# astooke/accel_rl

Measured on AMD Instinct MI355X. Metric: env-steps/sec (whole node), 256-env PPO Atari, higher is better.
Workload: dtype f32; 1 GPU; PPO breakout, 256 envs/GPU, horizon 5, spec-1 CNN (fp32), minibatch 512/GPU x 4 epochs, adam; synthetic fixed-frame emulator; hipGraph rollout; total_envs=256, global_minibatch=512, parallelism=single

## Files before the change

accel_rl_amd/_lib.py:

```python
import collections
import ctypes as C
import os

import torch

_PKG = os.path.dirname(os.path.abspath(__file__))
LIB_PATH = os.path.join(_PKG, "libaccel_rl_hip.so")

ARL_ABI_VERSION = 4
PROMO_NEP50, PROMO_LEGACY, PROMO_ASSOC = 0, 1, 2
PPO_TIE_THEANO, PPO_TIE_MATH, PPO_TIE_BOTH = 0, 1, 2
PPG_POLICY, PPG_AUX = 0, 1
OPT_ADAM, OPT_RMSPROP = 0, 1
VMPO_MAX_ROWS = 65536
RND_MAX_ROWS, RND_MIX_MAX_ENVS, RND_MIX_MAX_ROWS = 1 << 24, 1 << 20, 1 << 22
MAX_ACTIONS = 18
REPLAY_MAX_HORIZON = 16
RAW_H, RAW_W, OBS_H, OBS_W = 210, 160, 104, 80
OPT_PARTIALS = 1024

_vp, _i32, _i64, _f32, _f64 = C.c_void_p, C.c_int32, C.c_int64, C.c_float, C.c_double


class ArlGame(C.Structure):
# ... 100 lines not shown
NOISY_MAX_DRAWS = 16


class ArlNoisyLogitSrc(C.Structure):
    _fields_ = [("w_part", _vp), ("bias_or_null", _vp), ("s_part", _vp), ("b_sigma_or_null", _vp), ("feout", _vp),
                ("w_split_stride", _i64), ("s_split_stride", _i64), ("w_splits", _i32), ("s_splits", _i32)]


class ArlReplay(C.Structure):
    _fields_ = [("n_env", _i64), ("size", _i32), ("n_stack", _i32), ("frame_bytes", _i32),
                ("reward_horizon", _i32), ("frames", _vp), ("n_blanks", _vp), ("acts", _vp),
                ("terminals", _vp), ("rewards", _vp), ("returns", _vp)]


class ArlOptState(C.Structure):
    _fields_ = [("n_params", _i64), ("params", _vp), ("grads", _vp), ("slot0", _vp),
                ("slot1", _vp), ("step_count", _vp), ("lr_mult", _vp), ("partials", _vp),
                ("grad_norm_log", _vp), ("norm_log_len", _i32)]


_SIGNATURES = {
    "arl_abi_version": (_i32, []),
    "arl_last_error": (C.c_char_p, []),
    "arl_gae_scan": (_i32, [_vp, _vp, _vp, _vp, _f64, _f64, _i64, _i32, _i32, _vp, _vp, _vp]),
    "arl_nstep_return": (_i32, [_vp, _vp, _vp, _vp, _f64, _i64, _i32, _i32, _vp, _vp, _vp]),
    "arl_valids_mask": (_i32, [_vp, _i64, _i32, _vp, _vp, _vp, _vp, _vp]),
    "arl_standardize_workspace_bytes": (_i64, []),
    "arl_standardize": (_i32, [_vp, _vp, _i64, _f64, _vp, _vp]),
    "arl_sample_categorical": (_i32, [_vp, _vp, _i64, _i32, _vp, _vp]),
    "arl_env_act_step": (_i32, [C.POINTER(ArlGame), C.POINTER(ArlEnvState), C.POINTER(ArlRollout),
                                _vp, _vp, _vp, _vp, _i32, _i32, _f64, _f64, _vp]),
    "arl_env_frame_step": (_i32, [C.POINTER(ArlGame), C.POINTER(ArlEnvState), C.POINTER(ArlRollout),
                                  _i32, _i32, _vp]),
    "arl_env_step": (_i32, [C.POINTER(ArlGame), C.POINTER(ArlEnvState), C.POINTER(ArlRollout),
                            _vp, _vp, _vp, _vp, _i32, _i32, _f64, _f64, _i32, _i32, _vp]),
    "arl_rollout_begin": (_i32, [C.POINTER(ArlGame), C.POINTER(ArlEnvState), C.POINTER(ArlRollout), _vp]),
    "arl_env_reset": (_i32, [C.POINTER(ArlGame), C.POINTER(ArlEnvState), C.POINTER(ArlRollout),
                             _vp, _i32, _vp]),
    "arl_preprocess_frames": (_i32, [_vp, _vp, _i64, _i32, _vp, _vp]),
    "arl_copy_bytes": (_i32, [_vp, _vp, _i64, _vp]),
    "arl_ring_append": (_i32, [_vp, _i32, _vp, _i32, _vp, _vp]),
    "arl_gather_rows_many": (_i32, [C.POINTER(ArlGatherItem), _i32, _vp, _i64, C.POINTER(ArlRowMap), _vp]),
    "arl_gather_scale_obs": (_i32, [_vp, _vp, _i64, _i64, _f32, _vp, _vp]),
    "arl_gather_scale_obs_nhwc": (_i32, [_vp, _vp, _i64, _i32, _i32, _f32, _vp, _vp]),
    "arl_traj_minibatch": (_i32, [_vp, _i32, _i32, _i64, C.POINTER(_vp), _i32, _i32, _vp, _vp, C.POINTER(_vp), _vp, _vp]),
    "arl_bias_relu": (_i32, [_vp, _vp, _i64, _i32, _vp]),
    "arl_relu_bwd_workspace_bytes": (_i64, []),
    "arl_relu_bwd_bias_grad": (_i32, [_vp, _vp, _i64, _i32, _vp, _vp, _vp]),
    "arl_pg_head_workspace_bytes": (_i64, []),
    "arl_pg_head_infer": (_i32, [_vp, _vp, _vp, _i64, _i32, _i32, _vp, _vp, _vp]),
    "arl_pg_head_loss": (_i32, [_vp] * 11 + [_i64, _i32, _i32, _i32, _i32, _f32, _f32, _f32, _i32] + [_vp] * 7),
    "arl_pg_head_loss_parts": (_i32, [_vp] * 11 + [_i64, _i32, _i32, _i32, _i32, _f32, _f32, _f32, _i32] + [_vp] * 7 +
                               [_vp, _i32, _vp]),
    "arl_conv_workspace_bytes": (_i64, []),
    "arl_conv2d_fwd": (_i32, [_vp, _vp, _vp, _vp, C.POINTER(ArlConvGeom), _i32, _vp, _vp]),
    "arl_conv2d_bwd_data": (_i32, [_vp, _vp, _vp, _vp, _vp, C.POINTER(ArlConvGeom), C.POINTER(ArlCorunJob), C.POINTER(_i32), _vp]),
    "arl_conv2d_dgrad_weights": (_i32, [C.POINTER(ArlDgradWt), _i32, _vp]),
    "arl_conv2d_bwd_weight": (_i32, [_vp, _vp, _vp, C.POINTER(ArlConvGeom), _vp, _vp]),
    "arl_conv2d_bwd_weight_parts": (_i32, [_vp, _vp, _vp, C.POINTER(ArlConvGeom), _vp, _i64, C.POINTER(ArlFoldItem),
                                           _vp, C.POINTER(ArlFoldItem), _vp]),
    "arl_fold_many": (_i32, [C.POINTER(ArlFoldItem), _i32, _vp]),
    "arl_conv2d_fwd_parts": (_i32, [_vp, _vp, _vp, _vp, C.POINTER(ArlConvGeom), _i32, _vp, C.POINTER(ArlFoldItem), _vp]),
    "arl_conv2d_fwd_plan": (_i32, [C.POINTER(ArlConvGeom), C.POINTER(_i32), C.POINTER(_i32)]),
    "arl_serve_conv1_supported": (_i32, [C.POINTER(ArlGame), C.POINTER(ArlConvGeom)]),
    "arl_rollout_begin_conv1": (_i32, [C.POINTER(ArlGame), C.POINTER(ArlEnvState), C.POINTER(ArlRollout),
                                       C.POINTER(ArlServeConv1), _vp]),
    "arl_env_step_served": (_i32, [C.POINTER(ArlGame), C.POINTER(ArlEnvState), C.POINTER(ArlRollout),
                                   C.POINTER(ArlServeHead), C.POINTER(ArlServeConv1), _vp, _i32, _f64, _f64, _i32, _vp]),
    "arl_conv2d_u8_fwd": (_i32, [_vp, _i64, _vp, _f32, _vp, _vp, _vp, C.POINTER(ArlConvGeom), _i32, _vp]),
    "arl_conv2d_u8_bwd_weight_parts": (_i32, [_vp, _vp, _i64, _vp, _f32, _vp, C.POINTER(ArlConvGeom), _vp, _i64,
                                              C.POINTER(ArlFoldItem), _vp, C.POINTER(ArlFoldItem), _vp]),
    "arl_conv2d_bwd_pair": (_i32, [_vp, _vp, _vp, _vp, _vp, _vp, _vp, C.POINTER(ArlConvGeom), _vp, _i64,
                                   C.POINTER(ArlFoldItem), _vp, C.POINTER(ArlFoldItem), C.POINTER(ArlCorunJob),
                                   C.POINTER(_i32), _vp]),
    "arl_conv2d_bwd_weight_plan": (_i32, [_vp, _vp, _vp, C.POINTER(ArlConvGeom), _vp, _i64, C.POINTER(ArlFoldItem),
                                          _vp, C.POINTER(ArlFoldItem), C.POINTER(ArlWgradPlan)]),
    "arl_conv2d_u8_bwd_weight_plan": (_i32, [_vp, _vp, _i64, _vp, _f32, _vp, C.POINTER(ArlConvGeom), _vp, _i64,
                                             C.POINTER(ArlFoldItem), _vp, C.POINTER(ArlFoldItem),
                                             C.POINTER(ArlWgradPlan)]),
    "arl_conv2d_bwd_pair_plan": (_i32, [_vp, _vp, _vp, _vp, _vp, _vp, _vp, C.POINTER(ArlConvGeom), _vp, _i64,
                                        C.POINTER(ArlFoldItem), _vp, C.POINTER(ArlFoldItem), C.POINTER(ArlCorunJob),
                                        C.POINTER(_i32), C.POINTER(ArlWgradPlan), _vp]),
    "arl_conv2d_bwd_weight_group": (_i32, [C.POINTER(ArlWgradPlan), _i32, _vp]),
    "arl_relu_bwd_bias_parts": (_i32, [_vp, _vp, _i64, _i32, _vp, _vp, C.POINTER(ArlFoldItem), _vp]),
    "arl_replay_append": (_i32, [C.POINTER(ArlReplay), _vp, _vp, _vp, _vp, _i32, _i32, _f64, _i32, _vp]),
    "arl_replay_extract": (_i32, [C.POINTER(ArlReplay), _vp, _vp, _i64, _vp, _vp, _vp, _vp, _vp, _vp]),
    "arl_replay_extract_shift": (_i32, [C.POINTER(ArlReplay), _vp, _vp, _i64, _i32, _i32, _i32, _i32, _i32, _i64, _i64,
                                        _vp, _vp, _vp, _vp, _vp, _vp]),
    "arl_sumtree_find": (_i32, [_vp, _i32, _vp, _i64, _vp, _vp]),
    "arl_sumtree_add": (_i32, [_vp, _i32, _vp, _vp, _i64, _vp]),
    "arl_sumtree_gather": (_i32, [_vp, _vp, _i64, _f64, _vp, _vp]),
    "arl_sumtree_sample": (_i32, [_vp, _i32, _vp, _i32, _i32, _i32, _vp, _vp, _vp, _vp, _vp, _vp]),
    "arl_sumtree_sample_batch": (_i32, [_vp, _i32, _vp, _i32, _i32, _i32, _vp, _vp, _vp, _vp, _vp, _f64, _vp, _vp, _i32, _vp]),
    "arl_sumtree_update_pow": (_i32, [_vp, _i32, _vp, _vp, _vp, _f64, _i64, _vp]),
    "arl_is_weights": (_i32, [_vp, _i64, _f64, _vp, _vp]),
    "arl_priority_diffs": (_i32, [_vp, _vp, _i64, _f64, _vp, _vp]),
    "arl_catdqn_act": (_i32, [_vp, _vp, _vp, _i64, _i32, _i32, _i32, _i32, _vp, _vp, _vp]),
    "arl_catdqn_loss": (_i32, [_vp] * 8 + [_i64, _i32, _i32, _i32, _i32, _f32, _f32, _f32, _vp, _vp, _vp, _vp]),
    "arl_catdqn_loss_parts": (_i32, [_vp] * 8 + [_i64, _i32, _i32, _i32, _i32, _f32, _f32, _f32, _vp, _vp, _vp, _vp, _i32,
                               _vp]),
    "arl_qrdqn_act": (_i32, [_vp, _vp, _i64, _i32, _i32, _i32, _i32, _vp, _vp, _vp]),
    "arl_qrdqn_loss": (_i32, [_vp] * 7 + [_i64, _i32, _i32, _i32, _i32, _f32, _f32, _vp, _vp, _vp, _vp]),
    "arl_iqn_embed": (_i32, [_vp, _vp, _i64, _i64, _i64, _i32, _vp, _vp, _vp]),
    "arl_iqn_merge_fwd": (_i32, [_vp, _vp, _i64, _i32, _i32, _vp, _vp]),
    "arl_iqn_merge_bwd": (_i32, [_vp, _vp, _vp, _i64, _i32, _i32, _vp, _vp, _vp]),
    "arl_iqn_act": (_i32, [_vp, _vp, _i64, _i32, _i32, _i32, _vp, _vp, _vp, _i64, _vp]),
    "arl_iqn_loss": (_i32, [_vp] * 8 + [_i64, _i32, _i32, _i32, _i32, _f32, _f32, _vp, _vp, _vp, _vp, _i64, _vp]),
    "arl_miqn_loss": (_i32, [_vp] * 8 + [_i64, _i32, _i32, _i32, _i32, _f32, _f32, _f32, _f32, _f32, _vp, _vp, _vp, _vp,
                             _i64, _vp]),
    "arl_fqf_fractions": (_i32, [_vp, _i64, _i32, _i32, _vp, _vp, _vp, _vp, _vp, _vp, _vp]),
    "arl_fqf_act": (_i32, [_vp, _vp, _vp, _i64, _i32, _i32, _i32, _vp, _vp, _vp]),
    "arl_fqf_loss": (_i32, [_vp] * 13 + [_i64, _i32, _i32, _i32, _i32, _f32, _f32, _f32, _vp, _vp, _vp, _vp, _vp, _vp]),
    "arl_dqn_act": (_i32, [_vp, _vp, _i64, _i32, _i32, _i32, _vp, _vp, _vp]),
    "arl_dqn_loss": (_i32, [_vp] * 7 + [_i64, _i32, _i32, _i32, _f32, _f32, _vp, _vp, _vp, _vp]),
    "arl_drq_loss": (_i32, [_vp] * 7 + [_i64, _i32, _i32, _i32, _i32, _i32, _f32, _f32, _vp, _vp, _vp, _vp]),
    "arl_q_regress_loss": (_i32, [_vp] * 4 + [_i64, _i32, _i32, _f32, _vp, _vp, _vp, _vp]),
    "arl_qlambda_scan": (_i32, [_vp] * 4 + [_f64, _f64, _i64, _i32, _i32, _i32, _vp, _vp]),
    "arl_ppg_head_loss_parts": (_i32, [_vp] * 10 + [_i64, _i32, _i32, _i32, _i32, _f32, _f32, _f32, _f32, _i32] +
                                [_vp] * 8),
    "arl_vmpo_weights": (_i32, [_vp, _vp, _i64, _vp, _f64, _vp, _vp, _vp]),
    "arl_vmpo_head_loss_parts": (_i32, [_vp] * 10 + [_i64, _i32, _i32, _f32, _i32] + [_vp] * 8),
    "arl_vmpo_dual_step": (_i32, [_vp] * 7 + [_f32, _i32, _f32, _f32, _f32, _f32, _vp]),
    "arl_vtrace_scan": (_i32, [_vp] * 7 + [_f64] * 5 + [_i64, _i32, _i32, _vp, _vp, _vp, _vp]),
    "arl_seq_store": (_i32, [C.POINTER(_vp), _i32, _i32, _vp, _i32, _i32, _i32, _i32, _i32, C.POINTER(_vp), _vp, _vp]),
    "arl_seq_prepare": (_i32, [_vp, _vp, _i32, _i32, _i32, _i32, C.POINTER(_vp), _i32, _i32, _vp, _vp, _vp, C.POINTER(_vp),
                               _vp, _vp]),
    "arl_r2d2_loss": (_i32, [_vp] * 6 + [_i32] * 7 + [_f64] * 3 + [_vp] * 5),
    "arl_ln_bwd_workspace_bytes": (_i64, []),
    "arl_ln_relu_fwd": (_i32, [_vp, _vp, _vp, _i64, _i32, _f32, _vp, _vp, _vp]),
    "arl_ln_relu_bwd": (_i32, [_vp] * 5 + [_i64, _i32, _i32, _vp, _vp, _vp, _vp, C.POINTER(ArlFoldItem), _vp]),
    "arl_maxpool3s2_fwd": (_i32, [_vp, _i64, _i32, _i32, _i32, _vp, _vp, _vp, _vp]),
    "arl_maxpool3s2_bwd": (_i32, [_vp, _vp, _i64, _i32, _i32, _i32, _vp, _vp]),
    "arl_add_relu": (_i32, [_vp, _vp, _i64, _vp, _vp, _vp]),
    "arl_gather_scale_obs_nhwc_any": (_i32, [_vp, _vp, _i64, _i32, _i32, _f32, _vp, _vp]),
    "arl_mdqn_loss": (_i32, [_vp] * 7 + [_i64, _i32, _i32, _i32, _f32, _f32, _f32, _f32, _f32, _vp, _vp, _vp, _vp]),
    "arl_sacd_act": (_i32, [_vp, _vp, _i64, _i32, _i32, _i32, _vp, _vp, _vp]),
    "arl_sacd_loss": (_i32, [_vp] * 11 + [_i64, _i32, _i32, _f32, _f32, _vp, _vp, _vp, _vp, _vp]),
    "arl_sacd_alpha_grad": (_i32, [_vp, _i64, _vp, _f32, _vp, _vp]),
    "arl_lstm_cell_fwd": (_i32, [_vp, _i64, _vp, _vp, _i64, _i64, _i32, _vp, _i64, _vp, _i64, _vp, _i64, _vp]),
    "arl_lstm_cell_bwd": (_i32, [_vp, _i64, _vp, _vp, _vp, _i64, _vp, _i64, _vp, _i64, _i64, _i32, _vp, _i64, _vp, _vp]),
    "arl_gru_cell_fwd": (_i32, [_vp, _i64, _vp, _vp, _i64, _i64, _i32, _vp, _i64, _vp, _i64, _vp]),
    "arl_gru_cell_bwd": (_i32, [_vp, _i64, _vp, _vp, _vp, _i64, _vp, _i64, _i64, _i32, _vp, _i64, _vp, _i64, _vp, _vp]),
    "arl_rnn_cell_fwd": (_i32, [_vp, _i64, _vp, _i64, _i32, _vp, _i64, _vp]),
    "arl_rnn_cell_bwd": (_i32, [_vp, _i64, _vp, _vp, _i64, _i64, _i32, _vp, _i64, _vp]),
    "arl_seq_handover": (_i32, [_vp, _i64, _vp, _i64, _vp, _vp, _i64, _i64, _i64, _i32, _vp, _vp, _i64, _vp, _i64, _vp]),
    "arl_lstm_cell_bwd_reset": (_i32, [_vp, _i64, _vp, _vp, _vp, _i64, _vp, _i64, _vp, _i64, _i64, _i32, _vp, _i64, _vp,
                                       _vp, _vp, _i64, _i64, _vp]),
    "arl_gru_cell_bwd_reset": (_i32, [_vp, _i64, _vp, _vp, _vp, _i64, _vp, _i64, _i64, _i32, _vp, _i64, _vp, _i64, _vp,
                                      _vp, _vp, _i64, _i64, _vp]),
    "arl_rnn_cell_bwd_reset": (_i32, [_vp, _i64, _vp, _vp, _i64, _i64, _i32, _vp, _i64, _vp, _vp, _i64, _i64, _vp]),
    "arl_rnd_obs_stats_workspace_bytes": (_i64, [_i32, _i32]),
    "arl_rnd_obs_stats": (_i32, [_vp, _vp, _i64, _i32, _i32, _i32, _i32, _vp, _vp, _vp, _vp, _vp]),
    "arl_rnd_obs_prepare": (_i32, [_vp, _vp, _vp, _i64, _i64, _i32, _i32, _i32, _i32, _vp, _vp, _vp, _vp, _vp]),
    "arl_rnd_error": (_i32, [_vp, _vp, _i64, _i32, _i32, _vp, _vp, _vp, _vp]),
    "arl_rnd_reward_mix": (_i32, [_vp, _vp, _i64, _i32, _vp, _vp, _f64, _f64, _f64, _vp, _vp, _vp, _vp]),
    "arl_acer_retrace_scan": (_i32, [_vp] * 4 + [_i32, _vp, _vp, _vp, _vp, _f64, _f64, _i64, _i32, _i32, _vp, _vp, _vp, _vp]),
    "arl_acer_loss": (_i32, [_vp] * 6 + [_i64, _i32, _i32, _f64, _f64, _f64, _f64, _vp, _vp, _vp]),
    "arl_acer_avg_step": (_i32, [_vp, _vp, _i64, _f32, _vp]),
    "arl_gather_segments": (_i32, [_vp, _vp, _i64, _i64, _i64, _vp, _vp]),
    "arl_opt_step": (_i32, [C.POINTER(ArlOptState), _i32, _f32, _f32, _f32, _f32, _f32, _f32, _vp]),
    "arl_opt_step_noclip": (_i32, [C.POINTER(ArlOptState), _i32, _f32, _f32, _f32, _f32, _f32, _i32, _vp, _vp, _vp]),
    "arl_opt_finish": (_i32, [C.POINTER(ArlOptState), _i32, _f32, _vp, _vp, _vp]),
    "arl_opt_step_noclip_split": (_i32, [C.POINTER(ArlOptState), _i32, _f32, _f32, _f32, _f32, _f32, _i32, _vp, _vp,
                                         _i64, _i64, _i32, _vp]),
    "arl_opt_finish_split": (_i32, [C.POINTER(ArlOptState), _i32, _f32, _vp, _vp, _i64, _vp]),
    "arl_corun_job_init": (_i32, [C.POINTER(ArlCorunJob), C.POINTER(ArlOptState), _i32, _f32, _f32, _f32, _f32, _f32,
                                  _i32, _vp, _vp, _i64, _i64]),
    "arl_corun_job_run": (_i32, [C.POINTER(ArlCorunJob), _vp]),
    "arl_noisy_normals": (_i32, [_i64, _i64, _i32, _i32, _i64, _i32, _i32, _vp, _vp, _vp, _vp]),
    "arl_noisy_noise": (_i32, [_vp, C.POINTER(ArlNoisyLayer), _i32, _i64, _i32, _vp]),
    "arl_noisy_dense_combine": (_i32, [C.POINTER(ArlFoldItem), _vp, C.POINTER(ArlFoldItem), _vp, _vp, _i64, _i32, _i32,
                                       _vp, _vp, _vp, _vp, _vp]),
    "arl_noisy_dense_bwd_prep": (_i32, [_vp, _vp, _i64, _i32, _vp, _vp, _vp, _vp]),
    "arl_noisy_dense_bwd_dx": (_i32, [_vp, _vp, _vp, _i64, _i32, _vp, _vp]),
    "arl_noisy_draws": (_i32, [_vp, C.POINTER(ArlNoisyDraw), _i32, _i64, _i32, _vp]),
    "arl_noisy_duel_combine": (_i32, [C.POINTER(ArlFoldItem), _vp, C.POINTER(ArlFoldItem), C.POINTER(ArlFoldItem), _vp,
                                      _vp, _i64, _i32, _i32, _i32, _vp, _vp, _vp, _vp, _vp]),
    "arl_noisy_duel_bwd_prep": (_i32, [_vp, _vp, _i64, _i32, _i32, _vp, _vp, _vp, _vp, _vp]),
    "arl_noisy_duel_bwd_dx": (_i32, [_vp, _vp, _vp, _vp, _vp, _i64, _i32, _vp, _vp]),
    "arl_noisy_catdqn_loss_limits": (_i32, [C.POINTER(_i32), C.POINTER(_i32), C.POINTER(_i32)]),
    "arl_noisy_catdqn_loss_parts": (_i32, [C.POINTER(ArlNoisyLogitSrc), C.POINTER(ArlNoisyLogitSrc),
                                           C.POINTER(ArlNoisyLogitSrc), _vp, _vp, _vp, _vp, _vp, _i64, _i32, _i32, _i32,
                                           _i32, _f32, _f32, _f32, _vp, _vp, _vp, C.POINTER(ArlDgradWt), _i32, _vp]),
}

class ArlDevLaunch(C.Structure):
    _fields_ = [(n, _i32) for n in ("family", "wgm", "wgn", "tm", "tn", "bk", "minw", "flags", "split_mode", "splits")] + \
               [(n, C.c_uint32) for n in ("grid_x", "grid_y", "grid_z", "lds_bytes")]


_DEV_SIGNATURES = {
    "arl_dev_conv_trace_buffer": (None, [_vp]),
    "arl_dev_conv_force_generic": (None, [_i32]),
    "arl_dev_conv_variant": (None, [_i32]),
    "arl_dev_fwd_tile": (None, [_i32]),
    "arl_dev_dgrad_wt": (None, [_i32]),
    "arl_dev_conv_launch_log": (_i32, [C.POINTER(ArlDevLaunch), _i32]),
    "arl_dev_fold_wide_from": (None, [_i32]),
    "arl_dev_scan_force_wave": (None, [_i32]),
    "arl_dev_scan_wave_groups": (None, [_i32]),
    "arl_dev_env_variant": (None, [_i32]),
}

EXPORTED_SYMBOLS = tuple(_SIGNATURES)
DEV_SYMBOLS = tuple(_DEV_SIGNATURES)

ROUTE_SPLIT9, ROUTE_FP32, ROUTE_SPLIT6, ROUTE_BF16 = 0, 1, 6, 2
_PRECISION_TO_ROUTE = {9: ROUTE_SPLIT9, 0: ROUTE_FP32, 6: ROUTE_SPLIT6, 1: ROUTE_BF16}
default_route = _PRECISION_TO_ROUTE[int(os.environ.get("ARL_CONV_PRECISION", "9"))]


def set_conv_precision(mode):
    global default_route
    if mode not in _PRECISION_TO_ROUTE:
        raise ValueError("conv precision: 0 (fp32 MFMA), 6 or 9 (bf16-split products) or 1 (bf16 operands)")
    default_route = _PRECISION_TO_ROUTE[mode]


def conv_precision():
    return {v: k for k, v in _PRECISION_TO_ROUTE.items()}[default_route]

_lib = None


def load():
    global _lib
    if _lib is not None:
        return _lib
    if not os.path.exists(LIB_PATH):
        raise RuntimeError(
            "libaccel_rl_hip.so is not built (%s).  Run `python -c 'import __graft_entry__ as g; "
            "g.build()'` or `python accel_rl_amd/_build.py`.  There is no CPU fallback." % LIB_PATH)
    lib = C.CDLL(LIB_PATH)
    for name, (res, args) in list(_SIGNATURES.items()) + list(_DEV_SIGNATURES.items()):
        fn = getattr(lib, name)
        fn.restype = res
        fn.argtypes = args
    if lib.arl_abi_version() != ARL_ABI_VERSION:
        raise RuntimeError("libaccel_rl_hip.so ABI %d != binding %d" % (lib.arl_abi_version(), ARL_ABI_VERSION))
    _lib = lib
    return lib


def _check(rc, what):
    if rc != 0:
        msg = load().arl_last_error().decode(errors="replace")
        raise RuntimeError("%s failed (code %d): %s" % (what, rc, msg))


def ptr(t):
# ... 153 lines not shown
           "arl_env_act_step")


def env_step(game, state, rollout, prob, value, uniforms, step, mid_batch_reset, max_path_length, discount,
             max_start_noops, active=None, single_write=False, stream=None):
    _check(load().arl_env_step(C.byref(game), C.byref(state), C.byref(rollout), ptr(prob), ptr(value),
                               ptr(uniforms), ptr(active), step, int(bool(mid_batch_reset)),
                               float(max_path_length), float(discount), int(max_start_noops),
                               int(bool(single_write)), stream_ptr(stream)), "arl_env_step")


def serve_conv1_supported(game, geom):
    return bool(load().arl_serve_conv1_supported(C.byref(game), C.byref(geom)))


def rollout_begin_conv1(game, state, rollout, conv1, stream=None):
    _check(load().arl_rollout_begin_conv1(C.byref(game), C.byref(state), C.byref(rollout), C.byref(conv1),
                                          stream_ptr(stream)), "arl_rollout_begin_conv1")


def env_step_served(game, state, rollout, head, conv1, uniforms, step, max_path_length, discount, max_start_noops,
                    stream=None):
    _want(uniforms, torch.float64, "uniforms")
    _check(load().arl_env_step_served(C.byref(game), C.byref(state), C.byref(rollout), C.byref(head),
                                      None if conv1 is None else C.byref(conv1), ptr(uniforms), int(step),
                                      float(max_path_length), float(discount), int(max_start_noops),
                                      stream_ptr(stream)), "arl_env_step_served")


def env_frame_step(game, state, rollout, step, max_start_noops, stream=None):
    _check(load().arl_env_frame_step(C.byref(game), C.byref(state), C.byref(rollout), step,
                                     int(max_start_noops), stream_ptr(stream)), "arl_env_frame_step")


def rollout_begin(game, state, rollout, stream=None):
    _check(load().arl_rollout_begin(C.byref(game), C.byref(state), C.byref(rollout), stream_ptr(stream)),
           "arl_rollout_begin")


def env_reset(game, state, rollout, flags, max_start_noops, stream=None):
    _check(load().arl_env_reset(C.byref(game), C.byref(state), C.byref(rollout), ptr(flags),
                                int(max_start_noops), stream_ptr(stream)), "arl_env_reset")


def opt_step(opt, method, learning_rate, avg_factor, clip, beta1_or_rho, beta2, epsilon, stream=None):
    _check(load().arl_opt_step(C.byref(opt), method, learning_rate, avg_factor,
                               0.0 if clip is None else clip, beta1_or_rho, beta2, epsilon,
                               stream_ptr(stream)), "arl_opt_step")


OPT_NORM_SLOTS, OPT_NORM_BLOCKS = 64, 2048


def opt_step_noclip(opt, method, learning_rate, avg_factor, beta1_or_rho, beta2, epsilon, k, step_pp, norm_parts,
                    stream=None):
    _check(load().arl_opt_step_noclip(C.byref(opt), method, learning_rate, avg_factor, beta1_or_rho, beta2, epsilon,
                                      int(k), ptr(step_pp), ptr(norm_parts), stream_ptr(stream)), "arl_opt_step_noclip")


def opt_finish(opt, n_updates, avg_factor, step_pp, norm_parts, stream=None, hole_count=0):
    _check(load().arl_opt_finish_split(C.byref(opt), int(n_updates), avg_factor, ptr(step_pp), ptr(norm_parts),
                                       int(hole_count), stream_ptr(stream)), "arl_opt_finish_split")


def opt_step_noclip_split(opt, method, learning_rate, avg_factor, beta1_or_rho, beta2, epsilon, k, step_pp,
                          norm_parts, hole_first, hole_count, part, stream=None):
    _check(load().arl_opt_step_noclip_split(C.byref(opt), method, learning_rate, avg_factor, beta1_or_rho, beta2,
                                            epsilon, int(k), ptr(step_pp), ptr(norm_parts), int(hole_first),
                                            int(hole_count), int(part), stream_ptr(stream)),
           "arl_opt_step_noclip_split")


def corun_job(opt, method, learning_rate, avg_factor, beta1_or_rho, beta2, epsilon, k, step_pp, norm_parts,
              hole_first, hole_count):
    job = ArlCorunJob()
    _check(load().arl_corun_job_init(C.byref(job), C.byref(opt), method, learning_rate, avg_factor, beta1_or_rho, beta2,
                                     epsilon, int(k), ptr(step_pp), ptr(norm_parts), int(hole_first), int(hole_count)),
           "arl_corun_job_init")
    return job


def corun_job_run(job, stream=None):
    _check(load().arl_corun_job_run(C.byref(job), stream_ptr(stream)), "arl_corun_job_run")



def gather_scale_obs_nhwc(obs, idx, out, scale, stream=None):
    _want(obs, torch.uint8, "obs")
    _want(out, torch.float32, "out")
    if idx is not None:
        _want(idx, torch.int32, "idx")
    batch = out.shape[0]
    channels, plane = obs.shape[1], obs.shape[2] * obs.shape[3]
    assert out.numel() == batch * channels * plane
    _check(load().arl_gather_scale_obs_nhwc(ptr(obs), ptr(idx), batch, channels, plane, float(scale),
                                            out.data_ptr(), stream_ptr(stream)),
           "arl_gather_scale_obs_nhwc")


def traj_minibatch(seg, horizon, state_in, valids, idx, state_out, inv_count=None, stream=None):
    _want(seg, torch.int32, "seg")
    _want(idx, torch.int32, "idx")
    n_seg, n_state = seg.numel(), len(state_in)
    if len(state_out) != n_state:
        raise ValueError("traj_minibatch: %d states in, %d out" % (n_state, len(state_out)))
    if idx.numel() != n_seg * horizon:
        raise ValueError("traj_minibatch: idx holds %d rows, not %d segments x %d" % (idx.numel(), n_seg, horizon))
    hidden, total = 0, None
    for a, b in zip(state_in, state_out):
        _want(a, torch.float32, "state_in")
        _want(b, torch.float32, "state_out")
        hidden = a.shape[-1]
        if b.numel() != n_seg * hidden or a.numel() % (hidden * horizon) or total not in (None, a.numel() // hidden):
            raise ValueError("traj_minibatch: state shapes %s -> %s" % (tuple(a.shape), tuple(b.shape)))
        total = a.numel() // hidden
    if valids is not None:
        _want(valids, torch.int8, "valids")
        if valids.numel() % horizon or total not in (None, valids.numel()):
            raise ValueError("traj_minibatch: valids holds %d rows" % valids.numel())
        total = valids.numel()
    if inv_count is not None:
        _want(inv_count, torch.float32, "inv_count")
    n_traj = (total // horizon) if total is not None else 2 ** 31 // max(horizon, 1) - 1
    arr = C.c_void_p * max(n_state, 1)
    sin, sout = arr(*[ptr(a) for a in state_in]), arr(*[ptr(b) for b in state_out])
    _check(load().arl_traj_minibatch(ptr(seg), n_seg, horizon, n_traj, sin, n_state, hidden, ptr(valids), ptr(idx), sout,
                                     ptr(inv_count), stream_ptr(stream)), "arl_traj_minibatch")


def bias_relu(x, bias, rows, channels, stream=None):
    _check(load().arl_bias_relu(x.data_ptr(), bias.data_ptr(), rows, channels, stream_ptr(stream)),
           "arl_bias_relu")


def relu_bwd_workspace(device):
    return torch.empty(load().arl_relu_bwd_workspace_bytes() // 4, dtype=torch.float32, device=device)


def relu_bwd_bias_grad(dy, y, rows, channels, dbias, workspace, stream=None):
    _check(load().arl_relu_bwd_bias_grad(dy.data_ptr(), y.data_ptr(), rows, channels,
                                         dbias.data_ptr(), ptr(workspace), stream_ptr(stream)),
           "arl_relu_bwd_bias_grad")


def pg_head_workspace(device):
    return torch.zeros(load().arl_pg_head_workspace_bytes() // 4, dtype=torch.float32, device=device)


def pg_head_infer(h, w_head, b_head, prob, value, stream=None):
    batch, hid = h.shape
    n_act = prob.shape[1]
    _check(load().arl_pg_head_infer(ptr(h), w_head.data_ptr(), b_head.data_ptr(), batch, hid, n_act,
                                    ptr(prob), ptr(value), stream_ptr(stream)), "arl_pg_head_infer")


def pg_head_loss(h, w_head, b_head, actions, advantages, returns, old_prob, valids, idx, lr_mult,
                 inv_count, n_actions, kind, clip_param, v_loss_coeff, ent_loss_coeff,
                 dout, dh, dw_head, db_head, loss4, workspace, stream=None, relu_mask_dh=False,
                 tie_rule=PPO_TIE_THEANO):
    batch, hid = h.shape
    _check(load().arl_pg_head_loss(
        ptr(h), w_head.data_ptr(), b_head.data_ptr(), ptr(actions), ptr(advantages), ptr(returns),
        ptr(old_prob), ptr(valids), ptr(idx), ptr(lr_mult), ptr(inv_count), batch, hid, n_actions,
        kind, int(tie_rule), float(clip_param), float(v_loss_coeff), float(ent_loss_coeff), int(bool(relu_mask_dh)), ptr(dout), ptr(dh),
        dw_head.data_ptr(), db_head.data_ptr(), ptr(loss4), ptr(workspace), stream_ptr(stream)),
        "arl_pg_head_loss")
# ... 84 lines not shown
    if idx is not None:
        _want(idx, torch.int32, "idx")
        assert idx.numel() == geom.batch, "idx length"
    else:
        assert obs.shape[0] == geom.batch, "obs rows"


def conv2d_u8_fwd(obs, idx, scale, w, bias, y, geom, relu, stream=None):
    _u8_rows(obs, idx, geom)
    ho, wo = conv_out_hw(geom)
    assert w.numel() == geom.out_c * geom.kh * geom.kw * geom.in_c, "w size"
    assert y.numel() == geom.batch * ho * wo * geom.out_c, "y size"
    _check(load().arl_conv2d_u8_fwd(obs.data_ptr(), obs.shape[0], ptr(idx), float(scale), w.data_ptr(), ptr(bias),
                                    y.data_ptr(), C.byref(geom), int(bool(relu)), stream_ptr(stream)),
           "arl_conv2d_u8_fwd")


def conv2d_dgrad_weights(layers, stream=None):
    assert 0 < len(layers) <= DGRAD_WT_MAX
    items = (ArlDgradWt * len(layers))()
    for it, (w, wt, geom) in zip(items, layers):
        _want(w, torch.float32, "w")
        _want(wt, torch.float32, "wt")
        assert w.numel() == wt.numel() == geom.out_c * geom.kh * geom.kw * geom.in_c, "w / wt size"
        it.w, it.wt, it.geom = ptr(w), ptr(wt), C.pointer(geom)
    _check(load().arl_conv2d_dgrad_weights(items, len(layers), stream_ptr(stream)), "arl_conv2d_dgrad_weights")


def conv2d_bwd_data(dy, w, mask, dx, geom, stream=None, corun=None, wt=None):
    ho, wo = conv_out_hw(geom)
    assert dy.numel() == geom.batch * ho * wo * geom.out_c, "dy size"
    assert dx.numel() == geom.batch * geom.in_h * geom.in_w * geom.in_c, "dx size"
    assert mask is None or mask.numel() == dx.numel()
    taken = _i32(0)
    _check(load().arl_conv2d_bwd_data(dy.data_ptr(), w.data_ptr(), ptr(wt), None if mask is None else mask.data_ptr(),
                                      dx.data_ptr(), C.byref(geom), None if corun is None else C.byref(corun),
                                      C.byref(taken), stream_ptr(stream)), "arl_conv2d_bwd_data")
    return bool(taken.value)


def conv2d_bwd_weight(dy, x, dw, geom, workspace, stream=None):
    ho, wo = conv_out_hw(geom)
    assert dy.numel() == geom.batch * ho * wo * geom.out_c, "dy size"
    assert x.numel() == geom.batch * geom.in_h * geom.in_w * geom.in_c, "x size"
    assert dw.numel() == geom.out_c * geom.kh * geom.kw * geom.in_c, "dw size"
    _check(load().arl_conv2d_bwd_weight(dy.data_ptr(), x.data_ptr(), dw.data_ptr(), C.byref(geom),
                                        ptr(workspace), stream_ptr(stream)), "arl_conv2d_bwd_weight")


class FoldList(object):

    def __init__(self):
        self._items = (ArlFoldItem * FOLD_MAX_ITEMS)()
        self._n = 0
        self._plans = (ArlWgradPlan * WGRAD_GROUP_MAX)()
        self._n_plans = 0
        self.last_dw_in_place = False
        self.corun_taken = False

    def _next(self):
        assert self._n < FOLD_MAX_ITEMS, "too many pending folds"
        self._n += 1
        return C.byref(self._items[self._n - 1])

    def _bias_slot(self, dbias):
        if dbias is None:
            return None, None
        return dbias.data_ptr(), self._next()

    def _bias_done(self, dbias):
        if dbias is None:
            return True
        if self._items[self._n - 1].splits < 0:
            self._n -= 1
            return False
        return True

    def _next_plan(self, stream):
        if self._n_plans == WGRAD_GROUP_MAX:
            self.run_wgrads(stream)
        self._n_plans += 1
        return C.byref(self._plans[self._n_plans - 1])

    def run_wgrads(self, stream=None):
        n, self._n_plans = self._n_plans, 0
        if n:
            _check(load().arl_conv2d_bwd_weight_group(self._plans, n, stream_ptr(stream)), "arl_conv2d_bwd_weight_group")

    def conv2d_bwd_weight(self, dy, x, dw, geom, workspace, dbias=None, stream=None, defer=False):
        ho, wo = conv_out_hw(geom)
        assert dy.numel() == geom.batch * ho * wo * geom.out_c, "dy size"
        assert x.numel() == geom.batch * geom.in_h * geom.in_w * geom.in_c, "x size"
        assert dw.numel() == geom.out_c * geom.kh * geom.kw * geom.in_c, "dw size"
        item = self._next()
        pb, ib = self._bias_slot(dbias)
        if defer:
            _check(load().arl_conv2d_bwd_weight_plan(dy.data_ptr(), x.data_ptr(), dw.data_ptr(), C.byref(geom),
                                                     ptr(workspace), workspace.numel() * workspace.element_size(),
                                                     item, pb, ib, self._next_plan(stream)), "arl_conv2d_bwd_weight_plan")
            return self._bias_done(dbias)
        _check(load().arl_conv2d_bwd_weight_parts(dy.data_ptr(), x.data_ptr(), dw.data_ptr(), C.byref(geom),
                                                  ptr(workspace), workspace.numel() * workspace.element_size(),
                                                  item, pb, ib, stream_ptr(stream)), "arl_conv2d_bwd_weight_parts")
        return self._bias_done(dbias)

    def conv2d_u8_bwd_weight(self, dy, obs, idx, scale, dw, geom, workspace, dbias=None, stream=None, defer=False):
        _u8_rows(obs, idx, geom)
        ho, wo = conv_out_hw(geom)
        assert dy.numel() == geom.batch * ho * wo * geom.out_c, "dy size"
        assert dw.numel() == geom.out_c * geom.kh * geom.kw * geom.in_c, "dw size"
        item = self._next()
        pb, ib = self._bias_slot(dbias)
        if defer:
            _check(load().arl_conv2d_u8_bwd_weight_plan(dy.data_ptr(), obs.data_ptr(), obs.shape[0], ptr(idx),
                                                        float(scale), dw.data_ptr(), C.byref(geom), ptr(workspace),
                                                        workspace.numel() * workspace.element_size(), item, pb, ib,
                                                        self._next_plan(stream)), "arl_conv2d_u8_bwd_weight_plan")
            return self._bias_done(dbias)
        _check(load().arl_conv2d_u8_bwd_weight_parts(dy.data_ptr(), obs.data_ptr(), obs.shape[0], ptr(idx),
                                                     float(scale), dw.data_ptr(), C.byref(geom), ptr(workspace),
                                                     workspace.numel() * workspace.element_size(), item, pb, ib,
                                                     stream_ptr(stream)), "arl_conv2d_u8_bwd_weight_parts")
        return self._bias_done(dbias)

    def conv2d_bwd_pair(self, dy, w, mask, dx, x, dw, geom, workspace, dbias=None, stream=None, corun=None, wt=None,
                        defer=False):
        ho, wo = conv_out_hw(geom)
        assert dy.numel() == geom.batch * ho * wo * geom.out_c, "dy size"
        assert x.numel() == dx.numel() == geom.batch * geom.in_h * geom.in_w * geom.in_c, "x / dx size"
        assert dw.numel() == w.numel() == geom.out_c * geom.kh * geom.kw * geom.in_c, "w / dw size"
        item = self._next()
        slot = self._n - 1
        pb, ib = self._bias_slot(dbias)
        taken = _i32(0)
        if defer:
            _check(load().arl_conv2d_bwd_pair_plan(dy.data_ptr(), w.data_ptr(), ptr(wt), ptr(mask), dx.data_ptr(),
                                                   x.data_ptr(), dw.data_ptr(), C.byref(geom), ptr(workspace),
                                                   workspace.numel() * workspace.element_size(), item, pb, ib,
                                                   None if corun is None else C.byref(corun), C.byref(taken),
                                                   self._next_plan(stream), stream_ptr(stream)),
                   "arl_conv2d_bwd_pair_plan")
        else:
            _check(load().arl_conv2d_bwd_pair(dy.data_ptr(), w.data_ptr(), ptr(wt), ptr(mask), dx.data_ptr(), x.data_ptr(),
                                              dw.data_ptr(), C.byref(geom), ptr(workspace),
                                              workspace.numel() * workspace.element_size(), item, pb, ib,
                                              None if corun is None else C.byref(corun), C.byref(taken),
                                              stream_ptr(stream)), "arl_conv2d_bwd_pair")
        self.corun_taken = bool(taken.value)
        self.last_dw_in_place = self._items[slot].splits == 0
        return self._bias_done(dbias)

    def relu_bwd_bias_grad(self, dy, y, rows, channels, dbias, workspace, stream=None):
        _check(load().arl_relu_bwd_bias_parts(dy.data_ptr(), y.data_ptr(), rows, channels, dbias.data_ptr(),
                                              ptr(workspace), self._next(), stream_ptr(stream)),
               "arl_relu_bwd_bias_parts")

    def pg_head_loss(self, h, w_head, b_head, actions, advantages, returns, old_prob, valids, idx, lr_mult,
                     inv_count, n_actions, kind, clip_param, v_loss_coeff, ent_loss_coeff,
                     dout, dh, dw_head, db_head, loss4, workspace, stream=None, relu_mask_dh=False,
                 tie_rule=PPO_TIE_THEANO, dgrad_weights=None):
        batch, hid = h.shape
        assert self._n + 3 <= FOLD_MAX_ITEMS, "too many pending folds"
        first = C.byref(self._items[self._n])
        self._n += 3
        wt_items, n_wt = None, 0
        if dgrad_weights:
            n_wt = len(dgrad_weights)
            assert n_wt <= DGRAD_WT_MAX
            wt_items = (ArlDgradWt * n_wt)()
            for it, (w, wt, geom) in zip(wt_items, dgrad_weights):
# ... 959 lines not shown
```

accel_rl_amd/csrc/arl_optim_dev.h:

```cpp
#pragma once

#include "arl_common.h"

namespace arl {

__device__ __forceinline__ double wave_sum_d(double x) {
#pragma unroll
    for (int off = 32; off > 0; off >>= 1) x += __shfl_down(x, off, 64);
    return x;
}

__device__ __forceinline__ double block_sum_d(double x, double* lds) {
    x = wave_sum_d(x);
    const int lane = threadIdx.x & 63, w = threadIdx.x >> 6, nw = blockDim.x >> 6;
    if (lane == 0) lds[w] = x;
    __syncthreads();
    if (threadIdx.x == 0) {
        double s = 0;
        for (int i = 0; i < nw; ++i) s += lds[i];
        lds[0] = s;
    }
    __syncthreads();
    const double r = lds[0];
    __syncthreads();
    return r;
}

template <int METHOD>
__device__ __forceinline__ void update_one(float& p, float g, float& s0, float& s1, float avg,
                                           float cscale, float lr, float a_t, float b1, float b2,
                                           float eps) {
    const float gg = (g * avg) * cscale;
    if (METHOD == ARL_OPT_ADAM) {
        const float m = b1 * s0 + (1.f - b1) * gg;
        const float v = b2 * s1 + (1.f - b2) * (gg * gg);
        const float step = a_t * m / (sqrtf(v) + eps);
        s0 = m; s1 = v;
        p = p - step;
    } else {
        const float acc = b1 * s0 + (1.f - b1) * (gg * gg);
        const float step = lr * gg / sqrtf(acc + eps);
        s0 = acc;
        p = p - step;
    }
}

template <int METHOD>
__device__ __forceinline__ float opt_step_size(float lr, float b1, float b2, float t) {
    float a_t = 0.f;
    if (METHOD == ARL_OPT_ADAM)
        a_t = lr * sqrtf(1.f - powf(b2, t)) / (1.f - powf(b1, t));
    return a_t;
}

struct OptSeg {
    arl_opt_state o;
    int method, k;
    float lr_base, avg, b1, b2, eps;
    float* step_pp;
    double* norm_parts;
    long long a0, an, b0, bn;
    int block0, finish;
    int slots;
    int co_blocks;
};

template <int METHOD>
__device__ __forceinline__ void opt_update_block(const OptSeg& c, int block, int nblocks, double* lds) {
    const arl_opt_state& o = c.o;
    const float t = c.step_pp[c.k & 1] + 1.0f;
    const float lr = c.lr_base * o.lr_mult[0];
    const float a_t = opt_step_size<METHOD>(lr, c.b1, c.b2, t);
    float4* p4 = reinterpret_cast<float4*>(o.params);
    const float4* g4 = reinterpret_cast<const float4*>(o.grads);
    float4* m4 = reinterpret_cast<float4*>(o.slot0);
    float4* v4 = reinterpret_cast<float4*>(o.slot1);
    typedef float f32x4_t __attribute__((ext_vector_type(4)));
    auto ld_nt = [](const float4* q) {
        const f32x4_t x = __builtin_nontemporal_load(reinterpret_cast<const f32x4_t*>(q));
        return make_float4(x.x, x.y, x.z, x.w);
    };
    auto st_nt = [](float4* q, const float4& x) {
        f32x4_t y = {x.x, x.y, x.z, x.w};
        __builtin_nontemporal_store(y, reinterpret_cast<f32x4_t*>(q));
    };
    double s = 0;
    const long long total = c.an + c.bn, stride = (long long)nblocks * blockDim.x;
    for (long long j = (long long)block * blockDim.x + threadIdx.x; j < total; j += stride) {
        const long long i = j < c.an ? c.a0 + j : c.b0 + (j - c.an);
        float4 p = p4[i];
        const float4 g = ld_nt(g4 + i);
        float4 m = ld_nt(m4 + i);
        float4 v = (METHOD == ARL_OPT_ADAM) ? ld_nt(v4 + i) : make_float4(0, 0, 0, 0);
        s += (double)g.x * g.x + (double)g.y * g.y + (double)g.z * g.z + (double)g.w * g.w;
        update_one<METHOD>(p.x, g.x, m.x, v.x, c.avg, 1.f, lr, a_t, c.b1, c.b2, c.eps);
        update_one<METHOD>(p.y, g.y, m.y, v.y, c.avg, 1.f, lr, a_t, c.b1, c.b2, c.eps);
        update_one<METHOD>(p.z, g.z, m.z, v.z, c.avg, 1.f, lr, a_t, c.b1, c.b2, c.eps);
        update_one<METHOD>(p.w, g.w, m.w, v.w, c.avg, 1.f, lr, a_t, c.b1, c.b2, c.eps);
        p4[i] = p;
        st_nt(m4 + i, m);
        if (METHOD == ARL_OPT_ADAM) st_nt(v4 + i, v);
    }
    const long long n = o.n_params;
    if (c.finish && block == 0 && threadIdx.x < (n & 3)) {
        const long long i = ((n >> 2) << 2) + threadIdx.x;
        const float g = o.grads[i];
        float p = o.params[i], m = o.slot0[i], v = (METHOD == ARL_OPT_ADAM) ? o.slot1[i] : 0.f;
        s += (double)g * g;
        update_one<METHOD>(p, g, m, v, c.avg, 1.f, lr, a_t, c.b1, c.b2, c.eps);
        o.params[i] = p;
        o.slot0[i] = m;
        if (METHOD == ARL_OPT_ADAM) o.slot1[i] = v;
    }
    s = block_sum_d(s, lds);
    if (threadIdx.x == 0) {
        c.norm_parts[(long long)c.k * ARL_OPT_NORM_BLOCKS + c.block0 + block] = s;
        if (c.finish && block == 0) { c.step_pp[(c.k + 1) & 1] = t; o.step_count[0] = t; }
    }
    if (block == 0)
        for (int i = nblocks + threadIdx.x; i < c.slots; i += blockDim.x)
            c.norm_parts[(long long)c.k * ARL_OPT_NORM_BLOCKS + c.block0 + i] = 0.0;
}

inline void opt_split_plan(long long n_params, long long hole_count, int* rest, int* hole) {
    const long long n4 = n_params >> 2, h4 = hole_count >> 2;
    *rest = (int)stream_grid(n4 - h4, 256);
    if (h4 > 0 && *rest > ARL_OPT_NORM_BLOCKS / 2) *rest = ARL_OPT_NORM_BLOCKS / 2;
    long long hb = (h4 + 511) / 512;
    if (hb > ARL_OPT_NORM_BLOCKS - *rest) hb = ARL_OPT_NORM_BLOCKS - *rest;
    *hole = h4 > 0 ? (int)(hb < 1 ? 1 : hb) : 0;
}

int make_opt_seg(OptSeg* c, const arl_opt_state* opt, int32_t method, float learning_rate, float avg_factor,
                 float beta1_or_rho, float beta2, float epsilon, int32_t k, float* step_pp, double* norm_parts,
                 int64_t hole_first, int64_t hole_count, int part, int* blocks);
int launch_opt_seg(const OptSeg& c, int blocks, hipStream_t s);

}
```

accel_rl_amd/csrc/mfma_conv.hip:

```cpp
#include "mfma_conv_impl.h"
#include "dgrad_wt_dev.h"

using namespace arlc;

namespace arlc {
thread_local CallCtx t_ctx = {9, nullptr, false};
thread_local LaunchLog t_launch_log = {};
thread_local int t_launch_split = 9;
unsigned long long* g_trace = nullptr;
bool g_force_generic = false;
int g_fwd_tile = -1;
}

namespace {
constexpr int FOLD_WIDE = 128, FOLD_THREADS = 1024;
int g_fold_wide = FOLD_WIDE;
bool g_dgrad_wt = true;

struct FoldSlot { int64_t i; int zg, zgn, row0, o; };
__device__ __forceinline__ FoldSlot fold_slot(int splits, int local_block, int wide_from) {
    FoldSlot f;
    const int tid = threadIdx.x;
    f.o = tid & 15;
    if (splits >= wide_from) { f.zg = tid >> 4; f.zgn = 64; f.row0 = 0; f.i = (int64_t)local_block * 16 + f.o; }
// ... 41 lines not shown
        if (relu) { s.x = fmaxf(s.x, 0.f); s.y = fmaxf(s.y, 0.f); s.z = fmaxf(s.z, 0.f); s.w = fmaxf(s.w, 0.f); }
        if (mask) {
            const float4 m = mask[i];
            if (!(m.x > 0.f)) s.x = 0.f;
            if (!(m.y > 0.f)) s.y = 0.f;
            if (!(m.z > 0.f)) s.z = 0.f;
            if (!(m.w > 0.f)) s.w = 0.f;
        }
        out[i] = s;
    }
}

struct FoldManyArgs {
    arl_fold_item items[ARL_FOLD_MAX_ITEMS];
    int block_start[ARL_FOLD_MAX_ITEMS + 1];
    int n, wide_from;
};

__global__ __launch_bounds__(FOLD_THREADS) void fold_many_kernel(const FoldManyArgs a) {
    __shared__ float4 lds[64][16];
    int it = 0;
    while (it + 1 < a.n && (int)blockIdx.x >= a.block_start[it + 1]) ++it;
    const float4* part = reinterpret_cast<const float4*>(a.items[it].part);
    float4* out = reinterpret_cast<float4*>(a.items[it].out);
    const int64_t total4 = a.items[it].total >> 2;
    const int splits = a.items[it].splits;
    const FoldSlot f = fold_slot(splits, (int)blockIdx.x - a.block_start[it], a.wide_from);
    const float4 s = fold_sum(part, splits, total4, f, lds);
    const int64_t i = f.i;
    if (f.zg == 0 && i < total4) {
        const int64_t valid = a.items[it].valid;
        if (valid <= 0 || 4 * i + 3 < valid) {
            out[i] = s;
        } else {
            float* o1 = reinterpret_cast<float*>(out + i);
            if (4 * i < valid) o1[0] = s.x;
            if (4 * i + 1 < valid) o1[1] = s.y;
            if (4 * i + 2 < valid) o1[2] = s.z;
        }
    }
}

int launch_fold(const float* part, int splits, int64_t total, const float* bias, int n_bias, int relu,
                float* out, hipStream_t s, const float* mask = nullptr) {
    const int64_t total4 = total >> 2;
    hipLaunchKernelGGL(fold_splits_kernel, dim3((unsigned)fold_blocks(splits, total4)), dim3(FOLD_THREADS), 0, s,
                       (const float4*)part, splits, total4, (const float4*)bias, n_bias >> 2, relu,
                       (const float4*)mask, (float4*)out, g_fold_wide);
    log_launch(ARL_DEV_K_FOLD, {splits >= g_fold_wide ? 64 : 16, 0, 0, 0, 0, 0}, 0, splits,
               dim3((unsigned)fold_blocks(splits, total4)), 0);
    return arl::check_launch("fold_splits_kernel");
}

}

extern "C" int64_t arl_conv_workspace_bytes(void) { return (int64_t)64 << 20; }

extern "C" void arl_dev_conv_trace_buffer(void* device_u64_or_null) { g_trace = (unsigned long long*)device_u64_or_null; }

extern "C" void arl_dev_conv_force_generic(int32_t on) { g_force_generic = on != 0; }

extern "C" void arl_dev_fold_wide_from(int32_t splits) { g_fold_wide = splits > 0 ? splits : FOLD_WIDE; }

extern "C" void arl_dev_fwd_tile(int32_t v) { g_fwd_tile = ((v >= 0 && v <= 2) || v == 6 || v == 7) ? v : -1; }

extern "C" void arl_dev_dgrad_wt(int32_t on) { g_dgrad_wt = on != 0; }

extern "C" int32_t arl_dev_conv_launch_log(arl_dev_launch* out, int32_t max) {
    const LaunchLog& l = t_launch_log;
    for (int i = 0; out && i < l.n && i < max && i < ARL_DEV_LAUNCH_LOG_MAX; ++i) out[i] = l.rec[i];
    return l.n;
}

extern "C" int arl_corun_job_init(arl_corun_job* job, const arl_opt_state* opt, int32_t method, float learning_rate,
                                  float avg_factor, float beta1_or_rho, float beta2, float epsilon, int32_t k,
                                  float* step_pp, double* norm_parts, int64_t hole_first, int64_t hole_count) {
    ARL_REQUIRE(job, ARL_E_ARG, "null pointer");
    CorunJob* j = reinterpret_cast<CorunJob*>(job);
    int rc = arl::make_opt_seg(&j->seg, opt, method, learning_rate, avg_factor, beta1_or_rho, beta2, epsilon, k,
                               step_pp, norm_parts, hole_first, hole_count, 1, &j->blocks);
    if (rc) return rc;
    j->host_blocks = 256;
    if (const char* e = getenv("ARL_CORUN_BLOCKS")) j->host_blocks = atoi(e) > 0 ? atoi(e) : 256;
    return 0;
}

extern "C" int arl_corun_job_run(const arl_corun_job* job, void* stream) {
    ARL_REQUIRE(job, ARL_E_ARG, "null pointer");
    const CorunJob* j = reinterpret_cast<const CorunJob*>(job);
    return arl::launch_opt_seg(j->seg, j->blocks, (hipStream_t)stream);
}

namespace {
bool fwd_plan(int M, int N, int K, int* splits, int* per) {
    *splits = 1; *per = round_up(K, BKT);
    const bool small = N >= 128 && (int64_t)M * N <= (int64_t)1 << 20;
    const bool small32 = small && !g_split;
    if (small) plan_split(((M + (small32 ? 31 : 63)) / (small32 ? 32 : 64)) * ((N + 63) / 64), K, splits, per, 3 * TARGET_WGS);
    const int tiles128 = ((M + 127) / 128) * ((N + 127) / 128);
    if (!small && N >= 128 && tiles128 * 4 <= TARGET_WGS * 3) plan_split(tiles128, K, splits, per, TARGET_WGS);
    return small;
}

int fwd_impl(const float* x, const float* w, const float* bias_or_null, float* y, const arl_conv_geom* geom, int32_t relu,
             void* workspace, void* stream, arl_fold_item* parts = nullptr) {
    Geom g;
    int rc = check_geom(geom, &g);
    if (rc) return rc;
    ARL_REQUIRE(x && w && y && workspace, ARL_E_ARG, "null pointer");
    ARL_REQUIRE(arl::aligned16(x) && arl::aligned16(w) && arl::aligned16(y) && arl::aligned16(workspace) &&
                    (!bias_or_null || arl::aligned16(bias_or_null)), ARL_E_ALIGN, "16-byte alignment");
    hipStream_t s = (hipStream_t)stream;
    GemmArgs a = {};
    a.g.src = x; a.g.Hs = g.H; a.g.Ws = g.W; a.g.Cs = g.C; a.g.out_h = g.Ho; a.g.out_w = g.Wo;
    a.g.mul = g.stride; a.g.add_y = -g.pad_h; a.g.add_x = -g.pad_w; a.g.taps_x = g.kw; a.g.step = 1;
    a.M = (int)(g.batch * g.Ho * g.Wo); a.N = g.K; a.K = g.kh * g.kw * g.C;
    a.g.src_bytes = (unsigned)(g.batch * g.H * g.W * g.C * 4);
    a.b.w = w; a.b.ld = a.K; a.b.w_bytes = (unsigned)((int64_t)a.N * a.K * 4);
    a.o.dense = 1; a.trace = g_trace; a.xcd = 1;
    int splits, per;
    const bool small = fwd_plan(a.M, a.N, a.K, &splits, &per);
    const bool small32 = small && !g_split;
    const int tiles128 = ((a.M + 127) / 128) * ((a.N + 127) / 128);
    auto cu_fill = [](int t) { return (double)t / (double)(((t + TARGET_WGS - 1) / TARGET_WGS) * TARGET_WGS); };
    const int tiles64 = ((a.M + 63) / 64) * ((a.N + 63) / 64);
    const bool fill64 = !small && a.N >= 128 && splits == 1 && g_split && g_fwd_tile != 7 &&
                        (g_fwd_tile == 6 || 0.85 * cu_fill(tiles64) > cu_fill(tiles128));
    a.k_per_split = per;
    if (splits > 1) {
        ARL_REQUIRE((int64_t)splits * a.M * a.N * 4 <= arl_conv_workspace_bytes(), ARL_E_RANGE, "workspace too small");
        a.o.out = (float*)workspace; a.split_stride = (int64_t)a.M * a.N;
    } else {
        a.o.out = y; a.o.bias = bias_or_null; a.o.relu = relu;
    }
    constexpr int FBK = 32;
    const bool single_tap = g.C % FBK == 0;
    const bool multi_tap = !single_tap && FBK % g.C == 0 && g.kw % (FBK / g.C) == 0;
    const bool has_pad = g.pad_h > 0 || g.pad_w > 0;
    const bool fast = !g_force_generic && a.K % FBK == 0 && per % FBK == 0 && (single_tap || multi_tap) &&
                      (!has_pad || g.kh * g.kw <= 32) && a.N % 4 == 0;
    if (fast) {
        a.o.out_bytes = (unsigned)((int64_t)a.M * a.N * 4);
        a.g.mg_w = div_magic((int64_t)a.M + 256, a.g.out_w); a.g.mg_h = div_magic((int64_t)a.M + 256, a.g.out_h);
        a.g.taps_y = g.kh; a.g.dmin = 0;
        a.g.rmin = (a.g.add_y * g.W + a.g.add_x) * g.C;
        a.g.origin = a.g.rmin + a.g.dmin;
        a.g.src_bytes = (unsigned)(g.batch * g.H * g.W * g.C * 4 - (int64_t)a.g.origin * 4);
        if (a.N <= 16 && a.K % 16 == 0 && per % 16 == 0 && (g.C % 16 == 0 || (16 % g.C == 0 && g.kw % (16 / g.C) == 0)))
            rc = launch_igemm<4, 1, 2, 1, 16, true, true>(a, splits, multi_tap, has_pad, s);
        else if (g_split && a.N <= 32) rc = launch_igemm_split<4, 1, 1, 1, FBK, true, false, 2>(a, multi_tap, has_pad, s, splits);
        else if (g_split && a.N <= 64) {
            const int v = (g_fwd_tile >= 0 && g_fwd_tile <= 2) ? g_fwd_tile : (2 * ((a.M + 127) / 128) <= TARGET_WGS ? 1 : 0);
            if (v == 1) rc = launch_igemm_split<4, 1, 1, 1, FBK, true, false, 2>(a, multi_tap, has_pad, s, splits);
            else if (v == 2) rc = launch_igemm_split<2, 2, 1, 1, FBK, true, false, 3>(a, multi_tap, has_pad, s, splits);
            else rc = launch_igemm_split<4, 1, 1, 2, FBK, true, false, 2>(a, multi_tap, has_pad, s, splits);
        }
        else if (g_split && (small || fill64)) rc = launch_igemm_split<2, 2, 1, 1, FBK, true, false, 3>(a, multi_tap, has_pad, s, splits);
        else if (g_split) rc = launch_igemm_split<2, 2, 2, 2, FBK, true, false, 1>(a, multi_tap, has_pad, s, splits);
        else if (a.N <= 32 && a.K % 16 == 0 && per % 16 == 0 && (g.C % 16 == 0 || (16 % g.C == 0 && g.kw % (16 / g.C) == 0)))
            rc = launch_igemm<4, 1, 1, 1, 16, true>(a, splits, multi_tap, has_pad, s);
        else if (a.N <= 32) rc = launch_igemm<4, 1, 1, 1, FBK, true>(a, splits, multi_tap, has_pad, s);
        else if (a.N <= 64 && splits == 1) rc = launch_n64<true>(a, multi_tap, has_pad, s);
        else if (a.N <= 64) rc = launch_igemm<2, 2, 1, 1, FBK, true>(a, splits, multi_tap, has_pad, s);
        else if (small32) rc = launch_igemm_occ<1, 4, 2, 1, 32, true, true, 5>(a, multi_tap, has_pad, s, splits);
        else if (small) rc = launch_igemm<2, 2, 1, 1, FBK, true>(a, splits, multi_tap, has_pad, s);
        else rc = launch_igemm<2, 2, 2, 2, FBK, true>(a, splits, multi_tap, has_pad, s);
    } else {
        if (a.N <= 32) rc = launch_rowgather<4, 1, 2, 1, 16, true>(a, splits, s);
        else if (a.N <= 64) rc = launch_rowgather<2, 2, 2, 1, 16, true>(a, splits, s);
        else if (small) rc = launch_rowgather<2, 2, 1, 1, 16, true>(a, splits, s);
        else rc = launch_rowgather<2, 2, 2, 2, 16, true>(a, splits, s);
    }
    if (parts) {
// ... 176 lines not shown
        if (K <= 16) return launch_wgrad_fast<1, 4, 1, 1, FBK, true>(a, splits, p.has_pad, s);
        if (g_split && K <= 32) return launch_wgrad_split<1, 4, 1, 1, FBK, false, 2>(a, splits, p.has_pad, s);
        if (g_split && K <= 64) return launch_wgrad_split<2, 2, 1, 1, FBK, false, 2>(a, splits, p.has_pad, s);
        if (g_split) return launch_wgrad_split<2, 2, 2, 2, FBK, false, 1>(a, splits, p.has_pad, s);
        if (K <= 32) return launch_wgrad_fast<1, 4, 1, 1, FBK>(a, splits, p.has_pad, s);
        if (K <= 64) return launch_wgrad_fast<2, 2, 1, 1, FBK>(a, splits, p.has_pad, s);
        return launch_wgrad_fast<2, 2, 2, 2, FBK>(a, splits, p.has_pad, s);
    }
    if (K <= 32) return launch_wgrad<1, 4, 1, 1, 16>(a, splits, s);
    if (K <= 64) return launch_wgrad<2, 2, 1, 1, 16>(a, splits, s);
    return launch_wgrad<2, 2, 2, 2, 16>(a, splits, s);
}

int group_blocks(const WgradPlan& p) {
    const int bm = p.kind == WPLAN_U8 ? 32 : 64, bn = p.kind == WPLAN_U8 ? (p.cfg == 1 ? 256 : 128) : 64;
    return ((p.a.N + bn - 1) / bn) * ((p.a.K_out + bm - 1) / bm) * p.splits;
}

int wgrad_impl(const float* dy, const float* x, float* dw, const arl_conv_geom* geom, void* workspace,
               int64_t workspace_bytes, int* splits_out, int64_t* total_out, float** bias_part_out,
               WgradPlan* plan_only, void* stream) {
    ARL_REQUIRE(dy && x && dw && workspace, ARL_E_ARG, "null pointer");
    Geom g;
    int rc = check_geom(geom, &g);
    if (rc) return rc;
    ARL_REQUIRE(arl::aligned16(dy) && arl::aligned16(x) && arl::aligned16(dw) && arl::aligned16(workspace),
                ARL_E_ALIGN, "16-byte alignment");
    hipStream_t s = (hipStream_t)stream;
    WgradArgs a = {};
    a.dy = dy;
    a.g.src = x; a.g.Hs = g.H; a.g.Ws = g.W; a.g.Cs = g.C; a.g.out_h = g.Ho; a.g.out_w = g.Wo;
    a.g.mul = g.stride; a.g.add_y = -g.pad_h; a.g.add_x = -g.pad_w; a.g.taps_x = g.kw; a.g.step = 1;
    a.K_out = g.K; a.N = g.kh * g.kw * g.C; a.Mred = (int)(g.batch * g.Ho * g.Wo);
    a.g.src_bytes = (unsigned)(g.batch * g.H * g.W * g.C * 4);
    a.dy_bytes = (unsigned)((int64_t)a.Mred * g.K * 4);
    a.trace = g_trace; a.xcd = 1;
    int bm, bn;
    if (g.K <= 16) { bm = 16; bn = 128; }
    else if (g.K <= 32) { bm = 32; bn = 128; }
    else if (g.K <= 64) { bm = 64; bn = 64; }
    else { bm = 128; bn = 128; }
    const int tiles = ((a.K_out + bm - 1) / bm) * ((a.N + bn - 1) / bn);
    int splits, per;
    plan_split(tiles, a.Mred, &splits, &per, g.K <= 32 ? 2 * TARGET_WGS : g.K <= 64 ? 3 * TARGET_WGS : TARGET_WGS);
    a.m_per_split = per;
    const int64_t total = (int64_t)a.K_out * a.N;
    if (splits > 1) {
        ARL_REQUIRE((int64_t)splits * total * 4 <= workspace_bytes, ARL_E_RANGE, "workspace too small");
        a.part = (float*)workspace;
    } else {
        a.part = dw;
    }
    constexpr int FBK = 32;
    const bool has_pad = g.pad_h > 0 || g.pad_w > 0;
    const bool fast = !g_force_generic && a.Mred % FBK == 0 && per % FBK == 0 && (!has_pad || g.kh * g.kw <= 32);
    if (bias_part_out) *bias_part_out = nullptr;
    if (fast && bias_part_out) {
        const int64_t used = splits > 1 ? (int64_t)splits * total : 0;
        ARL_REQUIRE((used + (int64_t)splits * a.K_out) * 4 <= workspace_bytes, ARL_E_RANGE, "workspace too small");
        a.bias_part = (float*)workspace + used;
        *bias_part_out = a.bias_part;
    }
    if (fast) {
        a.g.taps_y = g.kh; a.g.dmin = 0;
        a.g.rmin = (a.g.add_y * g.W + a.g.add_x) * g.C;
        a.g.origin = a.g.rmin;
        a.g.src_bytes = (unsigned)(g.batch * g.H * g.W * g.C * 4 - (int64_t)a.g.origin * 4);
        const int img = g.Ho * g.Wo;
        a.adv_b = WG_ROWS / img;
        a.adv_y = (WG_ROWS % img) / g.Wo;
        a.adv_x = (WG_ROWS % img) % g.Wo;
    }
    WgradPlan p = {};
    p.a = a; p.fast = fast; p.has_pad = has_pad; p.cfg = g.K <= 32 ? 0 : g.K <= 64 ? 1 : 2;
    p.splits = splits; p.total = total; p.kind = WPLAN_F32; p.route = g_split;
    *splits_out = splits;
    *total_out = total;
    if (plan_only) { *plan_only = p; return 0; }
    return launch_wgrad_plan(p, s);
}
}

extern "C" int arl_conv2d_bwd_data(const float* dy, const float* w, const float* wt_or_null, const float* mask_or_null,
                                   float* dx, const arl_conv_geom* geom, const arl_corun_job* job_or_null,
                                   int32_t* job_taken_or_null, void* stream) {
    ARL_ROUTE_SCOPE(geom, job_or_null);
    const int rc = dgrad_impl(dy, w, mask_or_null, dx, geom, nullptr, stream, nullptr, 0, wt_or_null);
    if (job_taken_or_null) *job_taken_or_null = t_ctx.corun_taken ? 1 : 0;
    return rc;
}

extern "C" int arl_conv2d_bwd_weight(const float* dy, const float* x, float* dw, const arl_conv_geom* geom,
                                     void* workspace, void* stream) {
    ARL_ROUTE_SCOPE(geom, nullptr);
    int splits = 1;
    int64_t total = 0;
    int rc = wgrad_impl(dy, x, dw, geom, workspace, arl_conv_workspace_bytes(), &splits, &total, nullptr, nullptr, stream);
    if (rc || splits == 1) return rc;
    return launch_fold((const float*)workspace, splits, total, nullptr, 4, 0, dw, (hipStream_t)stream);
}

namespace {
void bias_item(arl_fold_item* item, const float* bias_part, float* dbias, int splits, int channels) {
    item->part = bias_part; item->out = dbias; item->total = channels;
    item->splits = bias_part ? splits : -1;
    item->valid = 0;
}
int wgrad_parts_impl(const float* dy, const float* x, float* dw, const arl_conv_geom* geom,
                     void* workspace, int64_t workspace_bytes, arl_fold_item* item,
                     float* dbias_or_null, arl_fold_item* bias_item_or_null, void* stream,
                     WgradPlan* plan_only = nullptr) {
    ARL_REQUIRE(item && (!dbias_or_null || bias_item_or_null), ARL_E_ARG, "null pointer");
    ARL_REQUIRE(!dbias_or_null || arl::aligned16(dbias_or_null), ARL_E_ALIGN, "16-byte alignment");
    int splits = 1;
    int64_t total = 0;
    float* bias_part = nullptr;
    int rc = wgrad_impl(dy, x, dw, geom, workspace, workspace_bytes, &splits, &total,
                        dbias_or_null ? &bias_part : nullptr, plan_only, stream);
    item->part = (const float*)workspace; item->out = dw; item->total = total;
    item->splits = splits > 1 ? splits : 0;
    item->valid = 0;
    if (dbias_or_null) bias_item(bias_item_or_null, bias_part, dbias_or_null, splits, geom->out_c);
    return rc;
}
}

extern "C" int arl_conv2d_bwd_weight_parts(const float* dy, const float* x, float* dw, const arl_conv_geom* geom,
                                           void* workspace, int64_t workspace_bytes, arl_fold_item* item,
                                           float* dbias_or_null, arl_fold_item* bias_item_or_null, void* stream) {
    ARL_ROUTE_SCOPE(geom, nullptr);
    return wgrad_parts_impl(dy, x, dw, geom, workspace, workspace_bytes, item, dbias_or_null, bias_item_or_null, stream);
}

static_assert(sizeof(WgradPlan) <= sizeof(arl_wgrad_plan), "arl_wgrad_plan too small");

extern "C" int arl_conv2d_bwd_weight_plan(const float* dy, const float* x, float* dw, const arl_conv_geom* geom,
                                          void* workspace, int64_t workspace_bytes, arl_fold_item* item,
                                          float* dbias_or_null, arl_fold_item* bias_item_or_null, arl_wgrad_plan* plan) {
    ARL_REQUIRE(plan, ARL_E_ARG, "null pointer");
    *plan = arl_wgrad_plan{};
    ARL_ROUTE_SCOPE(geom, nullptr);
    return wgrad_parts_impl(dy, x, dw, geom, workspace, workspace_bytes, item, dbias_or_null, bias_item_or_null, nullptr,
                            reinterpret_cast<WgradPlan*>(plan));
}

namespace {
struct U8Geom { int H, W, C, K, kh, kw, stride, Ho, Wo; int64_t batch; };

int check_u8(const uint8_t* obs, int64_t obs_rows, const arl_conv_geom* g, U8Geom* o) {
    ARL_REQUIRE(obs && g && obs_rows > 0, ARL_E_ARG, "null pointer");
    ARL_REQUIRE(g->batch > 0 && g->in_h > 0 && g->in_w > 0 && g->in_c > 0 && g->out_c > 0 && g->kh > 0 && g->kw > 0 &&
                    g->stride > 0, ARL_E_ARG, "conv: bad geometry");
    const int cpr = g->kw / 4;
    ARL_REQUIRE(g->pad_h == 0 && g->pad_w == 0 && g->stride % 4 == 0 && g->in_w % 4 == 0 &&
                    (g->in_h * g->in_w) % 4 == 0 && (g->kw == 4 || g->kw == 8 || g->kw == 16) && g->kh % (4 / cpr) == 0 &&
                    g->out_c % 4 == 0 && g->out_c <= 32 && ((uintptr_t)obs & 3) == 0,
                ARL_E_RANGE, "u8 conv: needs pad 0, stride % 4 == 0, width % 4 == 0, kw in {4, 8, 16}, <= 32 filters");
    o->H = g->in_h; o->W = g->in_w; o->C = g->in_c; o->K = g->out_c; o->kh = g->kh; o->kw = g->kw; o->stride = g->stride;
    o->Ho = (g->in_h - g->kh) / g->stride + 1; o->Wo = (g->in_w - g->kw) / g->stride + 1; o->batch = g->batch;
    const int64_t lim = (int64_t)OOB / 4;
    ARL_REQUIRE(o->Ho > 0 && o->Wo > 0 && g->batch * (int64_t)o->Ho * o->Wo * g->out_c < lim &&
                    obs_rows * (int64_t)g->in_c * g->in_h * g->in_w < (int64_t)OOB,
                ARL_E_RANGE, "conv: tensor larger than the 32-bit buffer offsets address");
    return 0;
}

void fill_u8(GatherDesc* d, const uint8_t* obs, int64_t obs_rows, const int32_t* idx, float scale, const U8Geom& g) {
// ... 43 lines not shown
        const dim3 pgrid((a.M + PBM - 1) / PBM, 1, 1);
        const arl::OptSeg none = {};
        const size_t lds = (size_t)2 * (PBM * (PBK + 4) + 32 * (PBK + 4)) * sizeof(float);
        hipLaunchKernelGGL((igemm_occ_kernel<2, 2, 2, 1, PBK, true, false, false, true, 5, false, true>), pgrid, dim3(256),
                           lds, (hipStream_t)stream, a, none);
        log_launch(ARL_DEV_K_IGEMM_OCC, {2, 2, 2, 1, PBK, 5}, launch_flags(true, true, true, false, false), 1, pgrid, lds);
        return arl::check_launch("igemm_occ_kernel (u8)");
    } else {
        const size_t lds = (size_t)2 * (BM * (BK + 4) + 32 * (BK + 4)) * sizeof(float);
        hipLaunchKernelGGL((igemm_u8_kernel<4, 1, 1, 1, BK, false>), grid, dim3(256), lds, (hipStream_t)stream, a);
        log_launch(ARL_DEV_K_IGEMM_U8, {4, 1, 1, 1, BK, 0}, launch_flags(true, false, true, false, false), 1, grid, lds);
    }
    return arl::check_launch("igemm_u8_kernel");
}

namespace {
int wgrad_u8_impl(const float* dy, const uint8_t* obs, int64_t obs_rows, const int32_t* idx_or_null, float scale, float* dw,
                  const arl_conv_geom* geom, void* workspace, int64_t workspace_bytes, arl_fold_item* item,
                  float* dbias_or_null, arl_fold_item* bias_item_or_null, WgradPlan* plan_only, void* stream) {
    launch_log_clear();
    ARL_REQUIRE(dy && dw && workspace && item && (!dbias_or_null || bias_item_or_null), ARL_E_ARG, "null pointer");
    U8Geom g;
    int rc = check_u8(obs, obs_rows, geom, &g);
    if (rc) return rc;
    ARL_ROUTE_SCOPE(geom, nullptr);
    ARL_REQUIRE(arl::aligned16(dy) && arl::aligned16(dw) && arl::aligned16(workspace) &&
                    (!dbias_or_null || arl::aligned16(dbias_or_null)), ARL_E_ALIGN, "16-byte alignment");
    WgradArgs a = {};
    a.dy = dy;
    fill_u8(&a.g, obs, obs_rows, idx_or_null, scale, g);
    a.K_out = g.K; a.N = g.C * g.kh * g.kw; a.Mred = (int)(g.batch * g.Ho * g.Wo);
    a.dy_bytes = (unsigned)((int64_t)a.Mred * g.K * 4);
    a.trace = g_trace; a.xcd = 1;
    const bool wide = g.K > 16 && g_split && g.kw % 8 == 0 && a.N % 256 == 0;
    const int bm = g.K <= 16 ? 16 : 32, bn = wide ? 256 : 128;
    const int tiles = ((a.K_out + bm - 1) / bm) * ((a.N + bn - 1) / bn);
    int splits, per;
    plan_split(tiles, a.Mred, &splits, &per, (g.K <= 16 ? 4 : 2) * TARGET_WGS);
    a.m_per_split = per;
    const int64_t total = (int64_t)a.K_out * a.N;
    const int64_t used = splits > 1 ? (int64_t)splits * total : 0;
    ARL_REQUIRE((used + (int64_t)splits * a.K_out) * 4 <= workspace_bytes, ARL_E_RANGE, "workspace too small");
    a.part = splits > 1 ? (float*)workspace : dw;
    if (dbias_or_null) a.bias_part = (float*)workspace + used;
    const int img = g.Ho * g.Wo;
    a.adv_b = WG_ROWS / img; a.adv_y = (WG_ROWS % img) / g.Wo; a.adv_x = (WG_ROWS % img) % g.Wo;
    WgradPlan p = {};
    p.a = a; p.splits = splits; p.total = total; p.kind = WPLAN_U8; p.route = g_split;
    p.cfg = g.K > 16 && g_split && g.kw % 8 == 0 ? (wide ? 1 : 2) : g.K <= 16 ? 0 : 3;
    p.fast = p.cfg == 1 || p.cfg == 2;
    item->part = (const float*)workspace; item->out = dw; item->total = total;
    item->splits = splits > 1 ? splits : 0;
    item->valid = 0;
    if (dbias_or_null) bias_item(bias_item_or_null, a.bias_part, dbias_or_null, splits, g.K);
    if (plan_only) { *plan_only = p; return 0; }
    return launch_wgrad_plan(p, (hipStream_t)stream);
}
}

extern "C" int arl_conv2d_u8_bwd_weight_parts(const float* dy, const uint8_t* obs, int64_t obs_rows,
                                              const int32_t* idx_or_null, float scale, float* dw,
                                              const arl_conv_geom* geom, void* workspace, int64_t workspace_bytes,
                                              arl_fold_item* item, float* dbias_or_null,
                                              arl_fold_item* bias_item_or_null, void* stream) {
    return wgrad_u8_impl(dy, obs, obs_rows, idx_or_null, scale, dw, geom, workspace, workspace_bytes, item, dbias_or_null,
                         bias_item_or_null, nullptr, stream);
}

extern "C" int arl_conv2d_u8_bwd_weight_plan(const float* dy, const uint8_t* obs, int64_t obs_rows,
                                             const int32_t* idx_or_null, float scale, float* dw,
                                             const arl_conv_geom* geom, void* workspace, int64_t workspace_bytes,
                                             arl_fold_item* item, float* dbias_or_null,
                                             arl_fold_item* bias_item_or_null, arl_wgrad_plan* plan) {
    ARL_REQUIRE(plan, ARL_E_ARG, "null pointer");
    *plan = arl_wgrad_plan{};
    return wgrad_u8_impl(dy, obs, obs_rows, idx_or_null, scale, dw, geom, workspace, workspace_bytes, item, dbias_or_null,
                         bias_item_or_null, reinterpret_cast<WgradPlan*>(plan), nullptr);
}


namespace {
int pair_impl(const float* dy, const float* w, const float* wt_or_null, const float* mask_or_null, float* dx, const float* x,
              float* dw, const arl_conv_geom* geom, void* workspace, int64_t workspace_bytes, arl_fold_item* item,
              float* dbias_or_null, arl_fold_item* bias_item_or_null, const arl_corun_job* job_or_null,
              int32_t* job_taken_or_null, WgradPlan* defer, void* stream) {
    ARL_REQUIRE(item && geom && (!dbias_or_null || bias_item_or_null), ARL_E_ARG, "null pointer");
    if (job_taken_or_null) *job_taken_or_null = 0;
    ARL_ROUTE_SCOPE(geom, job_or_null);
    ARL_REQUIRE(!dbias_or_null || arl::aligned16(dbias_or_null), ARL_E_ALIGN, "16-byte alignment");
    DgradPlan dp = {};
    WgradPlan wp = {};
    int splits = 1;
    int64_t total = 0;
    float* bias_part = nullptr;
    int rc = dgrad_impl(dy, w, mask_or_null, dx, geom, &dp, stream);
    if (rc) return rc;
    rc = wgrad_impl(dy, x, dw, geom, workspace, workspace_bytes, &splits, &total,
                    dbias_or_null ? &bias_part : nullptr, &wp, stream);
    if (rc) return rc;
    const bool has_pad = dp.has_pad || wp.has_pad;
    const int64_t dgrad_tiles = (int64_t)((dp.a.M + 127) / 128) * ((dp.a.N + 127) / 128) * (dp.a.n_par ? dp.a.n_par : 1);
    const bool paired = dp.fast && wp.fast && dp.cfg == 2 && wp.cfg == 2 && dgrad_tiles <= 2 * TARGET_WGS &&
                        (!has_pad || geom->kh * geom->kw <= 32) && !g_trace;
    if (!paired) {
        const int64_t half = (workspace_bytes / 2) & ~(int64_t)15;
        rc = dgrad_impl(dy, w, mask_or_null, dx, geom, nullptr, stream, (char*)workspace + half, workspace_bytes - half,
                        wt_or_null);
        if (job_taken_or_null) *job_taken_or_null = t_ctx.corun_taken ? 1 : 0;
        if (rc) return rc;
        return wgrad_parts_impl(dy, x, dw, geom, workspace, half, item, dbias_or_null, bias_item_or_null, stream, defer);
    }
    hipStream_t s = (hipStream_t)stream;
    if (g_split) rc = launch_pair<2, 2, 2, 2, 2, 2, 2, 2, 16>(dp, wp, has_pad, s);
    else rc = launch_pair<2, 2, 2, 2, 2, 2, 2, 2>(dp, wp, has_pad, s);
    item->part = (const float*)workspace; item->out = dw; item->total = wp.total;
    item->splits = wp.splits > 1 ? wp.splits : 0;
    item->valid = 0;
    if (dbias_or_null) bias_item(bias_item_or_null, bias_part, dbias_or_null, wp.splits, geom->out_c);
    return rc;
}
}

extern "C" int arl_conv2d_bwd_pair(const float* dy, const float* w, const float* wt_or_null, const float* mask_or_null,
                                   float* dx, const float* x, float* dw, const arl_conv_geom* geom, void* workspace,
                                   int64_t workspace_bytes, arl_fold_item* item, float* dbias_or_null,
                                   arl_fold_item* bias_item_or_null, const arl_corun_job* job_or_null,
                                   int32_t* job_taken_or_null, void* stream) {
    return pair_impl(dy, w, wt_or_null, mask_or_null, dx, x, dw, geom, workspace, workspace_bytes, item, dbias_or_null,
                     bias_item_or_null, job_or_null, job_taken_or_null, nullptr, stream);
}

extern "C" int arl_conv2d_bwd_pair_plan(const float* dy, const float* w, const float* wt_or_null, const float* mask_or_null,
                                        float* dx, const float* x, float* dw, const arl_conv_geom* geom, void* workspace,
                                        int64_t workspace_bytes, arl_fold_item* item, float* dbias_or_null,
                                        arl_fold_item* bias_item_or_null, const arl_corun_job* job_or_null,
                                        int32_t* job_taken_or_null, arl_wgrad_plan* plan, void* stream) {
    ARL_REQUIRE(plan, ARL_E_ARG, "null pointer");
    *plan = arl_wgrad_plan{};
    return pair_impl(dy, w, wt_or_null, mask_or_null, dx, x, dw, geom, workspace, workspace_bytes, item, dbias_or_null,
                     bias_item_or_null, job_or_null, job_taken_or_null, reinterpret_cast<WgradPlan*>(plan), stream);
}

extern "C" int arl_conv2d_bwd_weight_group(const arl_wgrad_plan* plans, int32_t n, void* stream) {
    launch_log_clear();
    ARL_REQUIRE(plans || n == 0, ARL_E_ARG, "null pointer");
    ARL_REQUIRE(n >= 0 && n <= ARL_WGRAD_GROUP_MAX, ARL_E_RANGE, "0 .. ARL_WGRAD_GROUP_MAX plans");
    hipStream_t s = (hipStream_t)stream;
    const WgradPlan* pl[ARL_WGRAD_GROUP_MAX];
    for (int i = 0; i < n; ++i) pl[i] = reinterpret_cast<const WgradPlan*>(&plans[i]);
    auto body_of = [](const WgradPlan& p) {
        if (!p.route || g_trace) return -1;
        if (p.kind == WPLAN_U8) return p.cfg == 1 ? 2 : p.cfg == 2 ? 3 : -1;
        return p.kind == WPLAN_F32 && p.fast && p.cfg == 1 ? (p.has_pad ? 1 : 0) : -1;
    };
    int route = 0, n_el = 0, el[ARL_WGRAD_GROUP_MAX];
    for (int i = 0; i < n; ++i) {
        if (pl[i]->kind != WPLAN_F32 && pl[i]->kind != WPLAN_U8) continue;
        if (body_of(*pl[i]) >= 0 && !route) route = pl[i]->route;
        if (body_of(*pl[i]) >= 0 && pl[i]->route == route) el[n_el++] = i;
    }
    for (int i = 0; i < n; ++i) {
        if (pl[i]->kind != WPLAN_F32 && pl[i]->kind != WPLAN_U8) continue;
        bool grouped = false;
        for (int k = 0; k < n_el; ++k) grouped = grouped || el[k] == i;
        if (grouped && n_el > 1) continue;
        const CallScope scope(pl[i]->route, nullptr, true);
        const int rc = launch_wgrad_plan(*pl[i], s);
        if (rc) return rc;
    }
    if (n_el < 2) return 0;
    for (int i = 1; i < n_el; ++i)
        for (int k = i; k > 0 && group_blocks(*pl[el[k]]) > group_blocks(*pl[el[k - 1]]); --k) std::swap(el[k], el[k - 1]);
    WgradGroupArgs g = {};
    size_t lds = 0;
    int groups = 0;
    for (int k = 0; k < n_el; ++k) {
        const WgradPlan& p = *pl[el[k]];
        const int body = body_of(p);
        const int bm = body < 2 ? 64 : 32, bn = body < 2 ? 64 : body == 2 ? 256 : 128;
        const int npl = planes_of(route);
        const size_t l = (size_t)2 * (npl * bm + (body < 2 ? npl : 1) * bn) * 32 * 2;
        if (l > lds) lds = l;
        g.a[k] = p.a; g.body[k] = body;
        g.gx[k] = (p.a.N + bn - 1) / bn; g.gy[k] = (p.a.K_out + bm - 1) / bm;
        g.blocks[k] = group_blocks(p);
        g.group_start[k] = groups;
        groups += (g.blocks[k] + 7) / 8;
    }
    g.group_start[n_el] = groups; g.n = n_el;
    const CallScope scope(route, nullptr, true);
    return launch_wgrad_group(g, groups, lds, s);
}

namespace {
__global__ __launch_bounds__(256) void dgrad_weights_kernel(const arlw::DgradWtArgs a) {
    arlw::dgrad_wt_block(a, (int)blockIdx.x, (int)threadIdx.x);
}
}

namespace arlw {
int dgrad_wt_plan(const arl_dgrad_wt* items, int32_t n, DgradWtArgs* out, int* blocks_out) {
    ARL_REQUIRE(items && n > 0 && n <= ARL_DGRAD_WT_MAX, ARL_E_ARG, "1 .. ARL_DGRAD_WT_MAX items");
    DgradWtArgs& a = *out;
    a = DgradWtArgs{};
    int blocks = 0;
    for (int i = 0; i < n; ++i) {
        arlc::Geom g;
        int rc = arlc::check_geom(items[i].geom, &g);
        if (rc) return rc;
        ARL_REQUIRE(items[i].w && items[i].wt && items[i].w != items[i].wt, ARL_E_ARG, "null / aliased pointer");
        ARL_REQUIRE(arl::aligned16(items[i].w) && arl::aligned16(items[i].wt), ARL_E_ALIGN, "16-byte alignment");
        const int st = g.stride;
        ARL_REQUIRE(g.kh % st == 0 && g.kw % st == 0 && st * st <= 4 && g.H >= st && g.W >= st, ARL_E_RANGE,
                    "kernel size divisible by the stride, stride <= 2");
        DgradWtItem& q = a.it[i];
        q.w = items[i].w; q.wt = items[i].wt; q.K = g.K; q.kh = g.kh; q.kw = g.kw; q.C = g.C; q.st = st;
        q.taps_x = g.kw / st; q.kred = (g.kh / st) * (g.kw / st) * g.K; q.total = g.K * g.kh * g.kw * g.C;
        for (int ph = 0; ph < st; ++ph)
            for (int pw = 0; pw < st; ++pw) {
                q.i0[ph * st + pw] = (ph + g.pad_h) % st;
                q.j0[ph * st + pw] = (pw + g.pad_w) % st;
            }
        a.block_start[i] = blocks;
        blocks += (q.total + 255) / 256;
    }
    a.block_start[n] = blocks; a.n = n;
    *blocks_out = blocks;
    return 0;
}
}

extern "C" int arl_conv2d_dgrad_weights(const arl_dgrad_wt* items, int32_t n, void* stream) {
    launch_log_clear();
    arlw::DgradWtArgs a;
    int blocks = 0;
    int rc = arlw::dgrad_wt_plan(items, n, &a, &blocks);
    if (rc) return rc;
    hipLaunchKernelGGL(dgrad_weights_kernel, dim3((unsigned)blocks), dim3(256), 0, (hipStream_t)stream, a);
    log_launch(ARL_DEV_K_DGRAD_WEIGHTS, {0, 0, 0, 0, 0, 0}, 0, n, dim3((unsigned)blocks), 0);
    return arl::check_launch("dgrad_weights_kernel");
}

extern "C" int arl_fold_many(const arl_fold_item* items, int32_t n, void* stream) {
    launch_log_clear();
    ARL_REQUIRE(items || n == 0, ARL_E_ARG, "null pointer");
    ARL_REQUIRE(n >= 0 && n <= ARL_FOLD_MAX_ITEMS, ARL_E_RANGE, "too many fold items");
    FoldManyArgs a = {};
    int blocks = 0;
    for (int i = 0; i < n; ++i) {
        if (items[i].splits <= 0) continue;
        ARL_REQUIRE(items[i].part && items[i].out && items[i].total > 0 && (items[i].total & 3) == 0, ARL_E_ARG,
                    "fold item: null pointer or length not a multiple of 4");
        ARL_REQUIRE(arl::aligned16(items[i].part) && arl::aligned16(items[i].out), ARL_E_ALIGN, "16-byte alignment");
        a.items[a.n] = items[i];
        a.block_start[a.n++] = blocks;
        blocks += fold_blocks(items[i].splits, items[i].total >> 2);
    }
    if (a.n == 0) return 0;
    a.block_start[a.n] = blocks;
    a.wide_from = g_fold_wide;
    hipLaunchKernelGGL(fold_many_kernel, dim3((unsigned)blocks), dim3(FOLD_THREADS), 0, (hipStream_t)stream, a);
    log_launch(ARL_DEV_K_FOLD_MANY, {0, 0, 0, 0, 0, 0}, 0, a.n, dim3((unsigned)blocks), 0);
    return arl::check_launch("fold_many_kernel");
}
```

accel_rl_amd/csrc/mfma_dispatch.h:

```cpp
#pragma once
#include "mfma_generic.h"
#include "mfma_igemm.h"
#include "mfma_wgrad.h"
#include "mfma_pair.h"

namespace arlc {

struct LaunchLog { int n; arl_dev_launch rec[ARL_DEV_LAUNCH_LOG_MAX]; };
extern thread_local LaunchLog t_launch_log;
extern thread_local int t_launch_split;
inline void launch_log_clear() { t_launch_log.n = 0; }
struct Tile { int wgm, wgn, tm, tn, bk, minw; };
inline void log_launch(int family, Tile t, int flags, int splits, dim3 grid, size_t lds) {
    LaunchLog& l = t_launch_log;
    if (l.n < ARL_DEV_LAUNCH_LOG_MAX)
        l.rec[l.n] = arl_dev_launch{family, t.wgm, t.wgn, t.tm, t.tn, t.bk, t.minw, flags, t_launch_split, splits,
                                    grid.x, grid.y, grid.z, (uint32_t)lds};
    ++l.n;
}

template <int WGM, int WGN, int TM, int TN, int BK, bool B_KC, bool TAP_UNIFORM = false>
int launch_rowgather(const GemmArgs& a, int splits, hipStream_t s) {
    constexpr int BM = WGM * TM * 32, BN = WGN * TN * 32;
    constexpr int A_SZ = BM * (BK + 4), B_SZ = B_KC ? BN * (BK + 4) : BK * BN;
    const size_t lds = (size_t)2 * (A_SZ + B_SZ) * sizeof(float);
    dim3 grid((a.M + BM - 1) / BM, (a.N + BN - 1) / BN, splits);
    hipLaunchKernelGGL((rowgather_gemm_kernel<WGM, WGN, TM, TN, BK, B_KC, TAP_UNIFORM>), grid, dim3(256), lds, s, a);
    log_launch(ARL_DEV_K_ROWGATHER, {WGM, WGN, TM, TN, BK, 0},
               (B_KC ? ARL_DEV_F_B_KC : 0) | (TAP_UNIFORM ? ARL_DEV_F_TAP_UNIFORM : 0), splits, grid, lds);
    return arl::check_launch("rowgather_gemm_kernel");
}

template <int WGM, int WGN, int TM, int TN, int BK>
int launch_wgrad(const WgradArgs& a, int splits, hipStream_t s) {
    constexpr int BM = WGM * TM * 32, BN = WGN * TN * 32;
    const size_t lds = (size_t)2 * BK * (BM + BN) * sizeof(float);
    dim3 grid((a.N + BN - 1) / BN, (a.K_out + BM - 1) / BM, splits);
    hipLaunchKernelGGL((wgrad_kernel<WGM, WGN, TM, TN, BK>), grid, dim3(256), lds, s, a);
    log_launch(ARL_DEV_K_WGRAD, {WGM, WGN, TM, TN, BK, 0}, 0, splits, grid, lds);
    return arl::check_launch("wgrad_kernel");
}

inline int launch_flags(bool b_kc, bool n16, bool u8, bool multi_tap, bool has_pad, bool direct = false, bool corun = false) {
    return (b_kc ? ARL_DEV_F_B_KC : 0) | (n16 ? ARL_DEV_F_N16 : 0) | (u8 ? ARL_DEV_F_U8 : 0) |
           (multi_tap ? ARL_DEV_F_MULTI_TAP : 0) | (has_pad ? ARL_DEV_F_HAS_PAD : 0) | (direct ? ARL_DEV_F_DIRECT : 0) |
           (corun ? ARL_DEV_F_CORUN : 0);
}

constexpr bool lds_fits(int floats) { return floats * 4 <= 65536; }

template <typename K>
int allow_big_lds(K kernel, size_t lds) {
    if (lds <= 65536) return 0;
    hipError_t e = hipFuncSetAttribute(reinterpret_cast<const void*>(kernel),
                                       hipFuncAttributeMaxDynamicSharedMemorySize, (int)lds);
    if (e != hipSuccess) { arl::set_error("hipFuncSetAttribute(LDS %zu): %s", lds, hipGetErrorString(e)); return (int)e; }
    return 0;
}

template <int WGM, int WGN, int TM, int TN, int BK, bool B_KC, bool N16 = false>
int launch_igemm(const GemmArgs& a, int splits, bool multi_tap, bool has_pad, hipStream_t s) {
    constexpr int BM = WGM * TM * (N16 ? 16 : 32), BN = N16 ? WGN * 16 : WGN * TN * 32;
    constexpr int A_SZ = BM * (BK + 4), B_SZ = B_KC ? BN * (BK + 4) : BK * (N16 ? BN + 4 : BN);
    const size_t lds = (size_t)2 * (A_SZ + B_SZ) * sizeof(float);
    dim3 grid((a.M + BM - 1) / BM, (a.N + BN - 1) / BN, a.n_par ? a.n_par : splits);
    int rc = 0;
#define ARL_IGEMM(MT, HP)                                                                                  \
    do {                                                                                                   \
        auto k = igemm_kernel<WGM, WGN, TM, TN, BK, B_KC, MT, HP, N16>;                                    \
        rc = allow_big_lds(k, lds);                                                                        \
        if (!rc) hipLaunchKernelGGL(k, grid, dim3(256), lds, s, a);                                        \
    } while (0)
    if (multi_tap && has_pad) ARL_IGEMM(true, true);
    else if (multi_tap) ARL_IGEMM(true, false);
    else if (has_pad) ARL_IGEMM(false, true);
    else ARL_IGEMM(false, false);
#undef ARL_IGEMM
    if (!rc) log_launch(ARL_DEV_K_IGEMM, {WGM, WGN, TM, TN, BK, 0}, launch_flags(B_KC, N16, false, multi_tap, has_pad), splits, grid, lds);
    return rc ? rc : arl::check_launch("igemm_kernel");
}

struct CorunJob { arl::OptSeg seg; int blocks, host_blocks; };
static_assert(sizeof(CorunJob) <= sizeof(arl_corun_job), "arl_corun_job too small");
struct CallCtx { int split; const CorunJob* corun; bool corun_taken; };
extern thread_local CallCtx t_ctx;
#define g_split (t_ctx.split)
struct CallScope {
    explicit CallScope(int split, const arl_corun_job* job = nullptr, bool keep_log = false) {
        t_ctx.split = split; t_ctx.corun = reinterpret_cast<const CorunJob*>(job); t_ctx.corun_taken = false;
        t_launch_split = split;
        if (!keep_log) launch_log_clear();
    }
    ~CallScope() { t_ctx.corun = nullptr; }
};
inline int split_of(const arl_conv_geom* g) {
    if (!g) return 9;
    return g->route == ARL_CONV_ROUTE_SPLIT9 ? 9 : g->route == ARL_CONV_ROUTE_FP32 ? 0 : g->route == ARL_CONV_ROUTE_SPLIT6 ? 6
         : g->route == ARL_CONV_ROUTE_BF16 ? 1 : -1;
}
#define ARL_ROUTE_SCOPE(geom, job)                                                                         \
    ARL_REQUIRE(split_of(geom) >= 0, ARL_E_ARG, "conv route: ARL_CONV_ROUTE_SPLIT9, _FP32, _SPLIT6 or _BF16");    \
    const CallScope call_scope_(split_of(geom), job)
inline bool corun_take(arl::OptSeg* c, dim3* grid) {
    if (!t_ctx.corun || t_ctx.corun_taken) return false;
    *c = t_ctx.corun->seg;
    c->co_blocks = t_ctx.corun->blocks < t_ctx.corun->host_blocks ? t_ctx.corun->blocks : t_ctx.corun->host_blocks;
    grid->x += (unsigned)c->co_blocks;
    t_ctx.corun_taken = true;
    return true;
}

template <int WGM, int WGN, int TM, int TN, int BK, bool B_KC, bool N16, int MINW>
int launch_igemm_occ(const GemmArgs& a, bool multi_tap, bool has_pad, hipStream_t s, int splits = 1) {
    constexpr int BM = WGM * TM * (N16 ? 16 : 32), BN = N16 ? WGN * 16 : WGN * TN * 32;
    constexpr int A_SZ = BM * (BK + 4), B_SZ = B_KC ? BN * (BK + 4) : BK * (N16 ? BN + 4 : BN);
    const size_t lds = (size_t)2 * (A_SZ + B_SZ) * sizeof(float);
    static_assert(lds_fits(2 * (A_SZ + B_SZ)), "<= 64 KiB of LDS");
    dim3 grid((a.M + BM - 1) / BM, (a.N + BN - 1) / BN, a.n_par ? a.n_par : splits);
    arl::OptSeg c = {};
    if constexpr (!B_KC) {
        if (!multi_tap && corun_take(&c, &grid)) {
            if (has_pad) hipLaunchKernelGGL((igemm_occ_kernel<WGM, WGN, TM, TN, BK, B_KC, false, true, N16, MINW, true>), grid, dim3(256), lds, s, a, c);
            else hipLaunchKernelGGL((igemm_occ_kernel<WGM, WGN, TM, TN, BK, B_KC, false, false, N16, MINW, true>), grid, dim3(256), lds, s, a, c);
            log_launch(ARL_DEV_K_IGEMM_OCC, {WGM, WGN, TM, TN, BK, MINW}, launch_flags(B_KC, N16, false, false, has_pad, false, true), splits, grid, lds);
            return arl::check_launch("igemm_occ_kernel (co-run)");
        }
    }
#define ARL_IGEMM_OCC(MT, HP) \
    hipLaunchKernelGGL((igemm_occ_kernel<WGM, WGN, TM, TN, BK, B_KC, MT, HP, N16, MINW>), grid, dim3(256), lds, s, a, c)
    if (multi_tap && has_pad) ARL_IGEMM_OCC(true, true);
    else if (multi_tap) ARL_IGEMM_OCC(true, false);
    else if (has_pad) ARL_IGEMM_OCC(false, true);
    else ARL_IGEMM_OCC(false, false);
#undef ARL_IGEMM_OCC
    log_launch(ARL_DEV_K_IGEMM_OCC, {WGM, WGN, TM, TN, BK, MINW}, launch_flags(B_KC, N16, false, multi_tap, has_pad), splits, grid, lds);
    return arl::check_launch("igemm_occ_kernel");
}

#ifdef ARL_NO_SPLIT6
#define ARL_BY_MODE(X1, X6, X9) do { X9; } while (0)
#else
#define ARL_BY_MODE(X1, X6, X9) do { if (g_split == 1) { X1; } else if (g_split == 6) { X6; } else { X9; } } while (0)
#endif

template <int WGM, int WGN, int TM, int TN, int BK, bool B_KC, bool U8, int MINW>
int launch_igemm_split(const GemmArgs& a, bool multi_tap, bool has_pad, hipStream_t s, int splits = 1) {
    constexpr int BM = WGM * TM * 32, BN = WGN * TN * 32;
    const int npl = planes_of(g_split);
    const size_t lds = (size_t)2 * ((U8 ? 1 : npl) * BM + npl * BN) * BK * 2;
    const size_t lds_dir = (size_t)2 * npl * BN * BK * 2;
    (void)lds_dir;
    dim3 grid((a.M + BM - 1) / BM, (a.N + BN - 1) / BN, a.n_par ? a.n_par : splits);
    arl::OptSeg c = {};
    int rc = 0;
    auto note = [&](bool mt, bool hp, bool co) {
        const bool ad = WGN == 1 && (U8 || !mt);
        if (!rc) log_launch(ARL_DEV_K_IGEMM_SPLIT, {WGM, WGN, TM, TN, BK, MINW}, launch_flags(B_KC, false, U8, mt, hp, ad, co), splits, grid, ad ? lds_dir : lds);
    };
#define ARL_SPLIT_K(MT, HP, SPL, CO, AD)                                                                   \
    do {                                                                                                   \
        auto k = igemm_split_kernel<WGM, WGN, TM, TN, BK, B_KC, MT, HP, U8, SPL, MINW, CO, AD>;            \
        const size_t lds_k = (AD) ? lds_dir : lds;                                                         \
        rc = allow_big_lds(k, lds_k + (CO ? 64 : 0));                                                      \
        if (!rc) hipLaunchKernelGGL(k, grid, dim3(256), lds_k, s, a, c);                                   \
    } while (0)
#define ARL_SPLIT_PIN(MT, HP, SPL, CO)                                                                     \
    do {                                                                                                   \
        constexpr bool AD = WGN == 1 && (U8 || !(MT));                                                     \
        ARL_SPLIT_K(MT, HP, SPL, CO, AD);                                                                  \
    } while (0)
#define ARL_SPLIT_MODE(MT, HP, CO)                                                                         \
    do {                                                                                                   \
        ARL_BY_MODE(ARL_SPLIT_PIN(MT, HP, 1, CO), ARL_SPLIT_PIN(MT, HP, 6, CO), ARL_SPLIT_PIN(MT, HP, 9, CO));                           \
    } while (0)
    if constexpr (U8) {
        ARL_SPLIT_MODE(false, false, false);
        note(false, false, false);
    } else {
        if constexpr (!B_KC || (WGM == 4 && WGN == 1 && TM == 1)) {
            if (!multi_tap && corun_take(&c, &grid)) {
                if (has_pad) ARL_SPLIT_MODE(false, true, true); else ARL_SPLIT_MODE(false, false, true);
                note(false, has_pad, true);
                return rc ? rc : arl::check_launch("igemm_split_kernel (co-run)");
            }
        }
        if (multi_tap && has_pad) ARL_SPLIT_MODE(true, true, false);
        else if (multi_tap) ARL_SPLIT_MODE(true, false, false);
        else if (has_pad) ARL_SPLIT_MODE(false, true, false);
        else ARL_SPLIT_MODE(false, false, false);
        note(multi_tap, has_pad, false);
    }
// ... 116 lines not shown
    const size_t lds = lds_d > lds_w ? lds_d : lds_w;
    const int dgx = (d.a.M + DBM - 1) / DBM, dgy = (d.a.N + DBN - 1) / DBN, dgz = d.a.n_par ? d.a.n_par : 1;
    const int wgx = (w.a.N + WBN - 1) / WBN, wgy = (w.a.K_out + WBM - 1) / WBM, wgz = w.splits;
    const int n_ig = dgx * dgy * dgz, n_wg = wgx * wgy * wgz;
    int rc;
    size_t lds_used = lds;
    if (g_split) {
        const size_t lds_s = (size_t)2 * planes_of(g_split) * ((DBM + DBN) > (WBM + WBN) ? (DBM + DBN) : (WBM + WBN)) * BK * 2;
#define ARL_PSPLIT(HP, SPL)                                                                                \
    do {                                                                                                   \
        auto k = bwd_pair_kernel<DWGM, DWGN, DTM, DTN, WWGM, WWGN, WTM, WTN, BK, HP, SPL>;                 \
        rc = allow_big_lds(k, lds_s + 4096);                                                               \
        if (!rc) hipLaunchKernelGGL(k, dim3(n_ig + n_wg), dim3(256), lds_s, s, d.a, w.a, dgx, dgy, n_ig, wgx, wgy); \
    } while (0)
        if (has_pad) ARL_BY_MODE(ARL_PSPLIT(true, 1), ARL_PSPLIT(true, 6), ARL_PSPLIT(true, 9));
        else ARL_BY_MODE(ARL_PSPLIT(false, 1), ARL_PSPLIT(false, 6), ARL_PSPLIT(false, 9));
#undef ARL_PSPLIT
        lds_used = lds_s;
    } else if (has_pad) {
        auto k = bwd_pair_kernel<DWGM, DWGN, DTM, DTN, WWGM, WWGN, WTM, WTN, BK, true>;
        rc = allow_big_lds(k, lds + 4096);
        if (!rc) hipLaunchKernelGGL(k, dim3(n_ig + n_wg), dim3(256), lds, s, d.a, w.a, dgx, dgy, n_ig, wgx, wgy);
    } else {
        auto k = bwd_pair_kernel<DWGM, DWGN, DTM, DTN, WWGM, WWGN, WTM, WTN, BK, false>;
        rc = allow_big_lds(k, lds + 4096);
        if (!rc) hipLaunchKernelGGL(k, dim3(n_ig + n_wg), dim3(256), lds, s, d.a, w.a, dgx, dgy, n_ig, wgx, wgy);
    }
    if (!rc) log_launch(ARL_DEV_K_BWD_PAIR, {DWGM, DWGN, DTM, DTN, BK, 0}, launch_flags(false, false, false, false, has_pad), wgz, dim3(n_ig + n_wg), lds_used);
    return rc ? rc : arl::check_launch("bwd_pair_kernel");
}


int launch_conv1_img(const unsigned char* obs, int64_t obs_rows, const int32_t* idx, float scale, const float* w, const float* bias, float* y,
                     int64_t batch, int C, int H, int W, int K, int kh, int kw, int stride, int Ho, int Wo, int relu,
                     hipStream_t s, unsigned char* copy_out = nullptr, long long copy_stride = 0, int* zero_word = nullptr);

#define ARL_GA const GemmArgs&, bool, bool, hipStream_t, int
#define ARL_P1(T) \
    T int launch_igemm_split<4, 1, 2, 1, 32, true, true, 2>(ARL_GA); \
    T int launch_igemm_split<4, 1, 1, 2, 32, true, false, 2>(ARL_GA); \
    T int launch_igemm_split<4, 1, 1, 1, 32, true, false, 2>(ARL_GA);
#define ARL_P2(T) \
    T int launch_igemm_split<2, 2, 2, 2, 32, true, false, 1>(ARL_GA); \
    T int launch_igemm_split<2, 2, 1, 1, 32, true, false, 3>(ARL_GA); \
    T int launch_igemm_split<2, 2, 1, 1, 32, false, false, 3>(ARL_GA);
#define ARL_P3(T) \
    T int launch_igemm_split<4, 1, 1, 2, 32, false, false, 2>(ARL_GA); \
    T int launch_igemm_split<4, 1, 1, 1, 32, false, false, 2>(ARL_GA); \
    T int launch_igemm_split<2, 2, 2, 2, 32, false, false, 1>(ARL_GA);
#define ARL_P4(T) \
    T int launch_wgrad_split<2, 2, 2, 2, 32, false, 1>(const WgradArgs&, int, bool, hipStream_t); \
    T int launch_wgrad_split<2, 2, 1, 1, 32, false, 2>(const WgradArgs&, int, bool, hipStream_t); \
    T int launch_wgrad_split<1, 4, 1, 1, 32, false, 2>(const WgradArgs&, int, bool, hipStream_t); \
    T int launch_wgrad_split<1, 4, 1, 1, 32, true, 2>(const WgradArgs&, int, bool, hipStream_t); \
    T int launch_wgrad_split<1, 4, 1, 2, 32, true, 2>(const WgradArgs&, int, bool, hipStream_t);
#define ARL_P5(T) \
    T int launch_pair<2, 2, 2, 2, 2, 2, 2, 2, 32>(const DgradPlan&, const WgradPlan&, bool, hipStream_t); \
    T int launch_pair<2, 2, 2, 2, 2, 2, 2, 2, 16>(const DgradPlan&, const WgradPlan&, bool, hipStream_t);
#define ARL_P6(T) \
    T int launch_igemm<2, 2, 1, 1, 32, true, false>(const GemmArgs&, int, bool, bool, hipStream_t); \
    T int launch_igemm<2, 2, 1, 1, 32, false, false>(const GemmArgs&, int, bool, bool, hipStream_t); \
    T int launch_igemm<2, 2, 2, 2, 32, true, false>(const GemmArgs&, int, bool, bool, hipStream_t); \
    T int launch_igemm<2, 2, 2, 2, 32, false, false>(const GemmArgs&, int, bool, bool, hipStream_t); \
    T int launch_igemm<4, 1, 2, 1, 16, true, true>(const GemmArgs&, int, bool, bool, hipStream_t); \
    T int launch_igemm<4, 1, 2, 1, 16, false, true>(const GemmArgs&, int, bool, bool, hipStream_t); \
    T int launch_igemm<4, 1, 1, 1, 32, true, false>(const GemmArgs&, int, bool, bool, hipStream_t); \
    T int launch_igemm<4, 1, 1, 1, 16, true, false>(const GemmArgs&, int, bool, bool, hipStream_t); \
    T int launch_igemm<4, 1, 1, 1, 16, false, false>(const GemmArgs&, int, bool, bool, hipStream_t);
#define ARL_P7(T) \
    T int launch_igemm_occ<2, 2, 2, 1, 32, false, true, 5>(ARL_GA); \
    T int launch_igemm_occ<1, 4, 2, 1, 32, true, true, 5>(ARL_GA); \
    T int launch_igemm_occ<1, 4, 2, 1, 32, false, true, 5>(ARL_GA); \
    T int launch_wgrad_fast<2, 2, 2, 2, 32, false>(const WgradArgs&, int, bool, hipStream_t); \
    T int launch_wgrad_fast<2, 2, 1, 1, 32, false>(const WgradArgs&, int, bool, hipStream_t); \
    T int launch_wgrad_fast<1, 4, 1, 1, 32, false>(const WgradArgs&, int, bool, hipStream_t); \
    T int launch_wgrad_fast<1, 4, 1, 1, 32, true>(const WgradArgs&, int, bool, hipStream_t);
#ifndef ARL_CONV_PART
#define ARL_CONV_PART 0
#endif
int launch_wgrad_group(const WgradGroupArgs& g, int groups, size_t lds, hipStream_t s);
#if ARL_CONV_PART == 8
int launch_wgrad_group(const WgradGroupArgs& g, int groups, size_t lds, hipStream_t s) {
    int rc = 0;
#define ARL_WGROUP(SPL)                                                                                    \
    do {                                                                                                   \
        auto k = wgrad_group_kernel<SPL>;                                                                  \
        rc = allow_big_lds(k, lds + 4096);                                                                 \
        if (!rc) hipLaunchKernelGGL(k, dim3((unsigned)groups * 8), dim3(256), lds, s, g);                  \
    } while (0)
    ARL_BY_MODE(ARL_WGROUP(1), ARL_WGROUP(6), ARL_WGROUP(9));
#undef ARL_WGROUP
    if (!rc) log_launch(ARL_DEV_K_WGRAD_GROUP, {0, 0, 0, 0, 32, 0}, 0, g.n, dim3((unsigned)groups * 8), lds);
    return rc ? rc : arl::check_launch("wgrad_group_kernel");
}
#endif
#define ARL_T_DEF template
#define ARL_T_EXT extern template
#if ARL_CONV_PART == 1
ARL_P1(ARL_T_DEF)
#else
ARL_P1(ARL_T_EXT)
#endif
#if ARL_CONV_PART == 2
ARL_P2(ARL_T_DEF)
#else
ARL_P2(ARL_T_EXT)
#endif
#if ARL_CONV_PART == 3
ARL_P3(ARL_T_DEF)
#else
ARL_P3(ARL_T_EXT)
#endif
#if ARL_CONV_PART == 4
ARL_P4(ARL_T_DEF)
#else
ARL_P4(ARL_T_EXT)
#endif
#if ARL_CONV_PART == 5
ARL_P5(ARL_T_DEF)
#else
ARL_P5(ARL_T_EXT)
#endif
#if ARL_CONV_PART == 6
ARL_P6(ARL_T_DEF)
#else
ARL_P6(ARL_T_EXT)
#endif
#if ARL_CONV_PART == 7
ARL_P7(ARL_T_DEF)
#else
ARL_P7(ARL_T_EXT)
#endif

}
```

accel_rl_amd/csrc/mfma_igemm.h:

```cpp
#pragma once
#include "mfma_common.h"

namespace arlc {

template <int WGM, int WGN, int TM, int TN, int BK, bool B_KC, bool MULTI_TAP, bool HAS_PAD, bool N16 = false,
          bool U8 = false, int SPLIT = 0, bool ADIR = false>
__device__ __forceinline__ void igemm_body(const GemmArgs& a, const int bx, const int by, const int bz, float* smem) {
    constexpr bool SP = SPLIT != 0;
    static_assert(!ADIR || (SP && WGN == 1 && !MULTI_TAP), "direct operand: split kernels, one wave per row tile");
    constexpr int MT = N16 ? 16 : 32;
    constexpr int BM = WGM * TM * MT, BN = N16 ? WGN * 16 : WGN * TN * 32, CH = BK / 4;
    constexpr int LDA = BK + 4;
    constexpr int LDB = B_KC ? BK + 4 : (N16 ? BN + 4 : BN);
    static_assert(!N16 || (TN == 1 && BK % 16 == 0), "16-wide tiles: one column tile per wave");
    static_assert(!SP || (!N16 && BK % 16 == 0), "split products: 32-wide tiles, two LDS stages");
    constexpr int ROWS_PER_PASS = 256 / CH;
    constexpr int RA = (BM + ROWS_PER_PASS - 1) / ROWS_PER_PASS;
    constexpr int A_SZ = BM * LDA, B_SZ = B_KC ? BN * LDB : BK * LDB;
    constexpr int NST = 2;
    constexpr int NB4 = B_KC ? BN * CH : BK * BN / 4;
    constexpr int NPAIR = (BK / 2) * (BN / 4);
    constexpr int RB = (SP && !B_KC) ? 2 * ((NPAIR + 255) / 256) : (NB4 + 255) / 256;
    static_assert(WGM * WGN == 4 && BK % 8 == 0, "tile shape");
    float* sA = smem;
// ... 541 lines not shown
            issue_mask_loads();
        }
        __builtin_amdgcn_sched_barrier(0);
        mfma_steps(buf_c, C0{}, CS_{});
        __builtin_amdgcn_sched_barrier(0);
        if (kt + 1 < nk) {
            store_tiles(buf ^ 1);
            __syncthreads();
        }
    };
    {
        int kt = 0;
        if (nk & 1) { k_tile(C1{}, 0); kt = 1; }
        for (; kt < nk; kt += 2) {
            k_tile(C0{}, kt);
            k_tile(C1{}, kt + 1);
        }
    }
    }

    if (a.trace) tr2 = __builtin_readcyclecounter();
    float* out = a.o.out + (a.n_par ? 0 : (int64_t)bz * a.split_stride);
    {
        const __amdgpu_buffer_rsrc_t rsO = make_rsrc(out, a.o.out_bytes);
        if (!PRE_MASK) decode_out_rows();
        if constexpr (N16) {
            const int n = n0 + wn * 16 + 4 * quad;
            const float4 bq = bias_q[0][0];
#pragma unroll
            for (int i = 0; i < TM; ++i) {
                const bool ok = row_off[i] >= 0 && n < a.N;
                float4 val = U8 ? make_float4(acc16[i][0] * g.scale + bq.x, acc16[i][1] * g.scale + bq.y,
                                              acc16[i][2] * g.scale + bq.z, acc16[i][3] * g.scale + bq.w)
                                : make_float4(acc16[i][0] + bq.x, acc16[i][1] + bq.y, acc16[i][2] + bq.z, acc16[i][3] + bq.w);
                if (a.o.relu) { val.x = fmaxf(val.x, 0.f); val.y = fmaxf(val.y, 0.f); val.z = fmaxf(val.z, 0.f); val.w = fmaxf(val.w, 0.f); }
                if (a.o.mask) {
                    float4 mk = make_float4(1.f, 1.f, 1.f, 1.f);
                    if (PRE_MASK) mk = mk_pre[0][i < TM ? i : 0];
                    else if (ok) mk = *reinterpret_cast<const float4*>(a.o.mask + row_off[i] + n);
                    if (!(mk.x > 0.f)) val.x = 0.f;
                    if (!(mk.y > 0.f)) val.y = 0.f;
                    if (!(mk.z > 0.f)) val.z = 0.f;
                    if (!(mk.w > 0.f)) val.w = 0.f;
                }
                u32x4 raw = {__float_as_uint(val.x), __float_as_uint(val.y), __float_as_uint(val.z), __float_as_uint(val.w)};
                __builtin_amdgcn_raw_buffer_store_b128(raw, rsO, ok ? (unsigned)((row_off[i] + n) << 2) : OOB, 0, 0);
            }
        } else {
            store_tiles_quads<TM, TN, U8>(acc, rsO, row_off, a.N, n0 + wn * TN * 32, lane, bias_q, a.o.mask, a.o.relu,
                                          PRE_MASK ? mk_pre : nullptr, g.scale);
        }
    }
    if (a.trace && tid == 0) {
        unsigned long long* t = a.trace + ((size_t)(bz * gridDim.y + by) * gridDim.x + bx) * 8;
        t[0] = tr0; t[1] = tr1; t[2] = tr2; t[3] = __builtin_readcyclecounter();
        t[4] = rt0; t[5] = __builtin_amdgcn_s_memrealtime();
#ifdef ARL_PROLOGUE_STAMPS
        if constexpr (SP) { t[6] = st_a; t[7] = st_b; }
        else
#endif
        {
        t[6] = __builtin_amdgcn_s_getreg((31 << 11) | 4);
        t[7] = __builtin_amdgcn_s_getreg((31 << 11) | 20);
        }
    }
}

template <int WGM, int WGN, int TM, int TN, int BK, bool B_KC, bool MULTI_TAP, bool HAS_PAD, bool N16 = false>
__global__ __launch_bounds__(256) void igemm_kernel(const GemmArgs a) {
    extern __shared__ __attribute__((aligned(16))) float smem[];
    igemm_body<WGM, WGN, TM, TN, BK, B_KC, MULTI_TAP, HAS_PAD, N16>(a, blockIdx.x, blockIdx.y, blockIdx.z, smem);
}

template <int WGM, int WGN, int TM, int TN, int BK, bool B_KC, bool MULTI_TAP, bool HAS_PAD, bool U8, int SPLIT, int MINW,
          bool CORUN = false, bool ADIR = false>
__global__ __launch_bounds__(256, MINW) void igemm_split_kernel(const GemmArgs a, const arl::OptSeg c) {
    extern __shared__ __attribute__((aligned(16))) float smem[];
    pin_gemm_args(a);
    int bx = blockIdx.x;
    if constexpr (CORUN) {
        if (bx < c.co_blocks) {
            __shared__ double lds[8];
            if (blockIdx.y || blockIdx.z) return;
            if (c.method == ARL_OPT_ADAM) arl::opt_update_block<ARL_OPT_ADAM>(c, bx, c.co_blocks, lds);
            else arl::opt_update_block<ARL_OPT_RMSPROP>(c, bx, c.co_blocks, lds);
            return;
        }
        bx -= c.co_blocks;
    }
    int by = blockIdx.y, bz = blockIdx.z;
    if (!CORUN && a.xcd) {
        const int gx = gridDim.x, gy = gridDim.y;
        const int t = xcd_chunk((bz * gy + by) * gx + bx, gx * gy * (int)gridDim.z);
        bx = t % gx;
        const int u = t / gx;
        by = u % gy; bz = u / gy;
    }
    igemm_body<WGM, WGN, TM, TN, BK, B_KC, MULTI_TAP, HAS_PAD, false, U8, SPLIT, ADIR>(a, bx, by, bz, smem);
}

template <int WGM, int WGN, int TM, int TN, int BK, bool B_KC, bool MULTI_TAP, bool HAS_PAD, bool N16, int MINW, bool CORUN = false,
          bool U8 = false>
__global__ __launch_bounds__(256, MINW) void igemm_occ_kernel(const GemmArgs a, const arl::OptSeg c) {
    extern __shared__ __attribute__((aligned(16))) float smem[];
    if constexpr (CORUN) {
        if ((int)blockIdx.x < c.co_blocks) {
            __shared__ double lds[8];
            if (blockIdx.y || blockIdx.z) return;
            if (c.method == ARL_OPT_ADAM) arl::opt_update_block<ARL_OPT_ADAM>(c, (int)blockIdx.x, c.co_blocks, lds);
            else arl::opt_update_block<ARL_OPT_RMSPROP>(c, (int)blockIdx.x, c.co_blocks, lds);
            return;
        }
        igemm_body<WGM, WGN, TM, TN, BK, B_KC, MULTI_TAP, HAS_PAD, N16, U8>(a, blockIdx.x - c.co_blocks, blockIdx.y, blockIdx.z, smem);
        return;
    }
    igemm_body<WGM, WGN, TM, TN, BK, B_KC, MULTI_TAP, HAS_PAD, N16, U8>(a, blockIdx.x, blockIdx.y, blockIdx.z, smem);
}

template <int WGM, int WGN, int TM, int TN, int BK, bool N16>
__global__ __launch_bounds__(256) void igemm_u8_kernel(const GemmArgs a) {
    extern __shared__ __attribute__((aligned(16))) float smem[];
    igemm_body<WGM, WGN, TM, TN, BK, true, false, false, N16, true>(a, blockIdx.x, blockIdx.y, blockIdx.z, smem);
}

}
```

accel_rl_amd/csrc/mfma_wgrad.h:

```cpp
#pragma once
#include "mfma_common.h"

namespace arlc {

constexpr int WG_ROWS = 256;

__device__ __forceinline__ uint2 (*wgrad_row_table())[WG_ROWS] {
    __shared__ uint2 table[2][WG_ROWS];
    return table;
}

template <int WGM, int WGN, int TM, int TN, int BK, bool HAS_PAD, bool M16 = false, bool U8 = false, int SPLIT = 0>
__device__ __forceinline__ void wgrad_fast_body(const WgradArgs& a, const int bx, const int by, const int bz, float* smem) {
    constexpr bool SP = SPLIT != 0;
    constexpr int BM = M16 ? 16 : WGM * TM * 32, BN = WGN * TN * 32;
    static_assert(!M16 || (WGM == 1 && TM == 1 && BK % 16 == 0), "16-row tiles: one row tile");
    static_assert(!SP || (!M16 && BK % 16 == 0), "split products: 32-row tiles");
    constexpr int A_SZ = BK * BM, B_SZ = BK * BN;
    constexpr int MC4 = BM / 4, NPA = (BK / 2) * MC4;
    constexpr int NA4 = BK * BM / 4, RA = SP ? 2 * ((NPA + 255) / 256) : (NA4 + 255) / 256;
    constexpr bool W8 = U8 && SP;
    constexpr int CW = W8 ? 8 : 4;
    constexpr int NC4 = BN / CW, KROWS = 256 / NC4, RB = BK / KROWS;
    static_assert(!SP || RB % 2 == 0, "split products: an even number of gather passes (row pairs)");
// ... 407 lines not shown
                if (NPA % 256 == 0 || t < NPA) red[a_row_of(p) * MC4 + t % MC4] = bsum[p];
                continue;
            }
            const int idx = tid + p * 256;
            if (NA4 % 256 == 0 || idx < NA4) red[idx] = bsum[p];
        }
        __syncthreads();
        if (tid < MC4) {
            float4 t = red[tid];
            for (int kl = 1; kl < BK; ++kl) {
                const float4 v = red[kl * MC4 + tid];
                t.x += v.x; t.y += v.y; t.z += v.z; t.w += v.w;
            }
            const int ko = i0 + tid * 4;
            if (ko < a.K_out) *reinterpret_cast<float4*>(a.bias_part + (int64_t)bz * a.K_out + ko) = t;
        }
    }

    float* out = a.part + (int64_t)bz * a.K_out * a.N;
    if constexpr (M16) {
#pragma unroll
        for (int gq = 0; gq < G16; ++gq) {
            const int col = n0 + wn * TN * 32 + gq * 16 + l15;
#pragma unroll
            for (int v = 0; v < 4; ++v) {
                const int row = i0 + 4 * quad + v;
                if (row < a.K_out && col < a.N) out[(int64_t)row * a.N + col] = U8 ? acc16[gq][v] * a.g.scale : acc16[gq][v];
            }
        }
    } else {
        if constexpr (U8) {
#pragma unroll
            for (int i = 0; i < TM; ++i)
#pragma unroll
                for (int j = 0; j < TN; ++j)
#pragma unroll
                    for (int v = 0; v < 16; ++v) acc[i][j][v] *= a.g.scale;
        }
        store_tiles_rowmajor<TM, TN>(acc, out, a.K_out, a.N, i0 + wm * TM * 32, n0 + wn * TN * 32, lane, nullptr, 0);
    }
    if (a.trace && tid == 0) {
        unsigned long long* t = a.trace + ((size_t)(bz * gridDim.y + by) * gridDim.x + bx) * 8;
        t[0] = tr0; t[1] = tr1; t[2] = tr2; t[3] = __builtin_readcyclecounter();
        t[4] = rt0; t[5] = __builtin_amdgcn_s_memrealtime();
        t[6] = __builtin_amdgcn_s_getreg((31 << 11) | 4);
        t[7] = __builtin_amdgcn_s_getreg((31 << 11) | 20);
    }
}

template <int WGM, int WGN, int TM, int TN, int BK, bool HAS_PAD, bool M16 = false>
__global__ __launch_bounds__(256, (TM * TN > 1 ? 2 : 4)) void wgrad_fast_kernel(const WgradArgs a) {
    extern __shared__ __attribute__((aligned(16))) float smem[];
    wgrad_fast_body<WGM, WGN, TM, TN, BK, HAS_PAD, M16>(a, blockIdx.x, blockIdx.y, blockIdx.z, smem);
}

template <int WGM, int WGN, int TM, int TN, int BK, bool M16>
__global__ __launch_bounds__(256, 4) void wgrad_u8_kernel(const WgradArgs a) {
    extern __shared__ __attribute__((aligned(16))) float smem[];
    wgrad_fast_body<WGM, WGN, TM, TN, BK, false, M16, true>(a, blockIdx.x, blockIdx.y, blockIdx.z, smem);
}

template <int WGM, int WGN, int TM, int TN, int BK, bool HAS_PAD, bool U8, int SPLIT, int MINW>
__global__ __launch_bounds__(256, MINW) void wgrad_split_kernel(const WgradArgs a) {
    extern __shared__ __attribute__((aligned(16))) float smem[];
    int bx = blockIdx.x, by = blockIdx.y, bz = blockIdx.z;
    if (a.xcd) {
        const int gx = gridDim.x, gy = gridDim.y;
        const int t = xcd_chunk((bz * gy + by) * gx + bx, gx * gy * (int)gridDim.z);
        bx = t % gx;
        const int u = t / gx;
        by = u % gy; bz = u / gy;
    }
    wgrad_fast_body<WGM, WGN, TM, TN, BK, HAS_PAD, false, U8, SPLIT>(a, bx, by, bz, smem);
}

struct WgradGroupArgs {
    WgradArgs a[ARL_WGRAD_GROUP_MAX];
    int gx[ARL_WGRAD_GROUP_MAX], gy[ARL_WGRAD_GROUP_MAX], blocks[ARL_WGRAD_GROUP_MAX], body[ARL_WGRAD_GROUP_MAX];
    int group_start[ARL_WGRAD_GROUP_MAX + 1];
    int n;
};

template <int SPLIT>
__global__ __launch_bounds__(256, 2) void wgrad_group_kernel(const WgradGroupArgs g) {
    extern __shared__ __attribute__((aligned(16))) float smem[];
    const int grp = (int)blockIdx.x >> 3;
    int it = 0;
    while (it + 1 < g.n && grp >= g.group_start[it + 1]) ++it;
    const int id = ((grp - g.group_start[it]) << 3) | ((int)blockIdx.x & 7);
    const int blocks = g.blocks[it];
    if (id >= blocks) return;
    const int gx = g.gx[it], gy = g.gy[it];
    const int t = g.a[it].xcd ? xcd_chunk(id, blocks) : id;
    const int bx = t % gx, u = t / gx;
    const int by = u % gy, bz = u / gy;
    switch (g.body[it]) {
    case 0: wgrad_fast_body<2, 2, 1, 1, 32, false, false, false, SPLIT>(g.a[it], bx, by, bz, smem); break;
    case 1: wgrad_fast_body<2, 2, 1, 1, 32, true, false, false, SPLIT>(g.a[it], bx, by, bz, smem); break;
    case 2: wgrad_fast_body<1, 4, 1, 2, 32, false, false, true, SPLIT>(g.a[it], bx, by, bz, smem); break;
    default: wgrad_fast_body<1, 4, 1, 1, 32, false, false, true, SPLIT>(g.a[it], bx, by, bz, smem); break;
    }
}

}
```

accel_rl_amd/csrc/optim.hip:

```cpp

#include "arl_optim_dev.h"

namespace {

using arl::block_sum_d;
using arl::update_one;

__global__ __launch_bounds__(256) void sumsq_kernel(const float* __restrict__ g, int64_t n,
                                                    double* __restrict__ partials,
                                                    float* __restrict__ step_count) {
    __shared__ double lds[8];
    double s = 0;
    const int64_t n4 = n >> 2;
    const int64_t stride = (int64_t)gridDim.x * blockDim.x;
    const float4* g4 = reinterpret_cast<const float4*>(g);
    for (int64_t i = (int64_t)blockIdx.x * blockDim.x + threadIdx.x; i < n4; i += stride) {
        const float4 v = g4[i];
        s += (double)v.x * v.x + (double)v.y * v.y + (double)v.z * v.z + (double)v.w * v.w;
    }
    if (blockIdx.x == 0 && threadIdx.x < (n & 3)) {
        const float v = g[(n4 << 2) + threadIdx.x];
        s += (double)v * v;
    }
    s = block_sum_d(s, lds);
    if (threadIdx.x == 0) {
        partials[blockIdx.x] = s;
        if (blockIdx.x == 0) step_count[0] += 1.0f;
    }
}

template <int METHOD>
__global__ __launch_bounds__(256) void update_kernel(arl_opt_state o, int n_partials, float lr_base,
                                                     float avg, float clip, float b1, float b2,
                                                     float eps) {
    __shared__ double lds[8];
    double s = 0;
    for (int i = threadIdx.x; i < n_partials; i += blockDim.x) s += o.partials[i];
    s = block_sum_d(s, lds);
    const float norm = avg * (float)sqrt(s);
    float cscale = 1.f;
    if (clip > 0.f) {
        const float target = fminf(fmaxf(norm, 0.f), clip);
        cscale = target / (1e-7f + norm);
    }
    const float t = o.step_count[0];
    const float lr = lr_base * o.lr_mult[0];
    float a_t = 0.f;
    if (METHOD == ARL_OPT_ADAM)
        a_t = lr * sqrtf(1.f - powf(b2, t)) / (1.f - powf(b1, t));
    if (blockIdx.x == 0 && threadIdx.x == 0 && o.grad_norm_log) {
        const int k = ((int)t - 1) % o.norm_log_len;
        o.grad_norm_log[k < 0 ? 0 : k] = norm;
    }
    const int64_t n = o.n_params, n4 = n >> 2;
    const int64_t stride = (int64_t)gridDim.x * blockDim.x;
    float4* p4 = reinterpret_cast<float4*>(o.params);
    const float4* g4 = reinterpret_cast<const float4*>(o.grads);
    float4* m4 = reinterpret_cast<float4*>(o.slot0);
    float4* v4 = reinterpret_cast<float4*>(o.slot1);
    for (int64_t i = (int64_t)blockIdx.x * blockDim.x + threadIdx.x; i < n4; i += stride) {
        float4 p = p4[i];
        const float4 g = g4[i];
        float4 m = m4[i];
        float4 v = (METHOD == ARL_OPT_ADAM) ? v4[i] : make_float4(0, 0, 0, 0);
        update_one<METHOD>(p.x, g.x, m.x, v.x, avg, cscale, lr, a_t, b1, b2, eps);
        update_one<METHOD>(p.y, g.y, m.y, v.y, avg, cscale, lr, a_t, b1, b2, eps);
        update_one<METHOD>(p.z, g.z, m.z, v.z, avg, cscale, lr, a_t, b1, b2, eps);
        update_one<METHOD>(p.w, g.w, m.w, v.w, avg, cscale, lr, a_t, b1, b2, eps);
        p4[i] = p;
        m4[i] = m;
        if (METHOD == ARL_OPT_ADAM) v4[i] = v;
    }
    if (blockIdx.x == 0 && threadIdx.x < (n & 3)) {
        const int64_t i = (n4 << 2) + threadIdx.x;
        float p = o.params[i], m = o.slot0[i], v = (METHOD == ARL_OPT_ADAM) ? o.slot1[i] : 0.f;
        update_one<METHOD>(p, o.grads[i], m, v, avg, cscale, lr, a_t, b1, b2, eps);
        o.params[i] = p;
        o.slot0[i] = m;
        if (METHOD == ARL_OPT_ADAM) o.slot1[i] = v;
    }
}

template <int METHOD>
__global__ __launch_bounds__(256) void update_noclip_kernel(const arl::OptSeg c) {
    __shared__ double lds[8];
    arl::opt_update_block<METHOD>(c, (int)blockIdx.x, (int)gridDim.x, lds);
}

__global__ __launch_bounds__(256) void opt_finish_kernel(arl_opt_state o, int n_updates, int n_blocks, float avg,
                                                         float* step_pp, const double* __restrict__ norm_parts) {
    __shared__ double lds[8];
    const int k = blockIdx.x;
    double s = 0;
    for (int i = threadIdx.x; i < n_blocks; i += blockDim.x) s += norm_parts[(int64_t)k * ARL_OPT_NORM_BLOCKS + i];
    s = block_sum_d(s, lds);
    if (threadIdx.x == 0) {
        if (o.grad_norm_log) o.grad_norm_log[k % o.norm_log_len] = avg * (float)sqrt(s);
        if (k == 0) { const float t = step_pp[n_updates & 1]; step_pp[0] = t; step_pp[1] = t; o.step_count[0] = t; }
    }
}

int check_opt(const arl_opt_state* opt, int32_t method, float learning_rate, float beta1_or_rho, float beta2,
              float epsilon) {
    ARL_REQUIRE(opt, ARL_E_ARG, "null state");
    ARL_REQUIRE(opt->params && opt->grads && opt->slot0 && opt->step_count && opt->lr_mult, ARL_E_ARG,
                "null pointer in state");
    ARL_REQUIRE(method == ARL_OPT_ADAM || method == ARL_OPT_RMSPROP, ARL_E_ARG, "unknown method");
    ARL_REQUIRE(method != ARL_OPT_ADAM || opt->slot1, ARL_E_ARG, "adam needs slot1");
    ARL_REQUIRE(opt->n_params > 0, ARL_E_ARG, "n_params <= 0");
    ARL_REQUIRE(!opt->grad_norm_log || opt->norm_log_len > 0, ARL_E_ARG, "norm_log_len <= 0");
    ARL_REQUIRE(arl::aligned16(opt->params) && arl::aligned16(opt->grads) && arl::aligned16(opt->slot0) &&
                    (!opt->slot1 || arl::aligned16(opt->slot1)), ARL_E_ALIGN, "flat buffers must be 16-byte aligned");
    if (method == ARL_OPT_ADAM)
        ARL_REQUIRE(beta1_or_rho >= 0.f && beta1_or_rho < 1.f && beta2 >= 0.f && beta2 < 1.f, ARL_E_RANGE,
                    "adam: beta1 and beta2 in [0, 1)");
    else
        ARL_REQUIRE(beta1_or_rho >= 0.f && beta1_or_rho <= 1.f, ARL_E_RANGE, "rmsprop: rho in [0, 1]");
    ARL_REQUIRE(epsilon >= 0.f, ARL_E_RANGE, "epsilon negative or NaN");
    ARL_REQUIRE(learning_rate >= 0.f, ARL_E_RANGE, "learning_rate negative or NaN");
    return 0;
}

}

namespace {
int check_noclip(const arl_opt_state* opt, int32_t method, float learning_rate, float beta1_or_rho, float beta2,
                 float epsilon, int32_t k, const float* step_pp, const double* norm_parts) {
    int rc = check_opt(opt, method, learning_rate, beta1_or_rho, beta2, epsilon);
    if (rc) return rc;
    ARL_REQUIRE(step_pp && norm_parts, ARL_E_ARG, "null pointer");
    ARL_REQUIRE(k >= 0 && k < ARL_OPT_NORM_SLOTS, ARL_E_RANGE, "update index outside the call's slots");
    return 0;
}

}

namespace arl {
int launch_opt_seg(const OptSeg& c, int blocks, hipStream_t s) {
    if (c.method == ARL_OPT_ADAM)
        hipLaunchKernelGGL((update_noclip_kernel<ARL_OPT_ADAM>), dim3((unsigned)blocks), dim3(256), 0, s, c);
    else
        hipLaunchKernelGGL((update_noclip_kernel<ARL_OPT_RMSPROP>), dim3((unsigned)blocks), dim3(256), 0, s, c);
    return check_launch("update_noclip_kernel");
}


int make_opt_seg(OptSeg* c, const arl_opt_state* opt, int32_t method, float learning_rate, float avg_factor,
                 float beta1_or_rho, float beta2, float epsilon, int32_t k, float* step_pp, double* norm_parts,
                 int64_t hole_first, int64_t hole_count, int part, int* blocks) {
    int rc = check_noclip(opt, method, learning_rate, beta1_or_rho, beta2, epsilon, k, step_pp, norm_parts);
    if (rc) return rc;
    ARL_REQUIRE(hole_first >= 0 && hole_count >= 0 && hole_first + hole_count <= opt->n_params &&
                    (hole_first & 3) == 0 && (hole_count & 3) == 0, ARL_E_ARG,
                "hole: a float4-aligned range inside the bucket");
    ARL_REQUIRE(part == 0 || hole_count > 0, ARL_E_ARG, "part 1 needs a hole");
    int rest, hole;
    opt_split_plan(opt->n_params, hole_count, &rest, &hole);
    *c = OptSeg{};
    c->o = *opt; c->method = method; c->k = k;
    c->lr_base = learning_rate; c->avg = avg_factor; c->b1 = beta1_or_rho; c->b2 = beta2; c->eps = epsilon;
    c->step_pp = step_pp; c->norm_parts = norm_parts;
    const long long n4 = opt->n_params >> 2, h0 = hole_first >> 2, hn = hole_count >> 2;
    if (part == 0) {
        c->a0 = 0; c->an = h0; c->b0 = h0 + hn; c->bn = n4 - (h0 + hn);
        c->block0 = 0; c->finish = 1; c->slots = rest; *blocks = rest;
    } else {
        c->a0 = h0; c->an = hn; c->b0 = 0; c->bn = 0;
        c->block0 = rest; c->finish = 0; c->slots = hole; *blocks = hole;
    }
// ... 67 lines not shown
```

accel_rl_amd/policies/atari_cnn_policy.py:

```python
import ctypes as C
import os

import numpy as np
import torch

from accel_rl_amd import _lib
from accel_rl_amd.distributions import Categorical
from accel_rl_amd.spaces import Discrete
from accel_rl_amd.util.misc import struct
from accel_rl_amd.util.seed import layer_rng

KIND_A2C, KIND_PPO = 0, 1
KIND_VMPO = 4


def _glorot_uniform(shape):
    receptive = int(np.prod(shape[2:]))
    fan_in, fan_out = shape[1] * receptive, shape[0] * receptive
    a = np.sqrt(6. / (fan_in + fan_out))
    return layer_rng().uniform(low=-a, high=a, size=shape).astype(np.float32)


def _norm_c(shape, std):
    out = np.random.randn(*shape).astype(np.float32)
# ... 458 lines not shown
            finally:
                self._wt_fresh = False
            return loss4

    max_rows_per_pass = None
    CACHE_BYTES = 256 << 20

    def rows_per_pass(self):
        if not isinstance(self.max_rows_per_pass, str):
            return self.max_rows_per_pass
        per_row = int(np.prod(self._obs_shape)) + 8 * sum(nf * ho * wo for nf, ci, sz, st, pad, ho, wo in self._conv_geom)
        return max(256, (self.CACHE_BYTES // per_row + 128) // 256 * 256)

    def _loss_and_grads_in_passes(self, mb, rows, limit, kind, clip_param, v_loss_coeff, ent_loss_coeff, lr_mult,
                                  inv_count, tie_rule=_lib.PPO_TIE_THEANO, beta_clone=1.0, duals=None):
        idx = mb.get("idx")
        if idx is None:
            idx = self._buffer(("all_rows", rows), (rows,), dtype=torch.int32)
            idx.copy_(torch.arange(rows, dtype=torch.int32, device=self.device))
        if inv_count is None:
            inv_count = self._buffer(("inv_rows", rows), (1,))
            inv_count.fill_(1.0 / rows)
        if not getattr(self, "_passes_logged", False):
            self._passes_logged = True
            from accel_rl_amd.util import logger
            logger.log("AtariCnnPolicy: minibatches of %d rows are walked in passes of %d (gradients accumulated in a fixed "
                       "order; max_rows_per_pass = None keeps one pass)" % (rows, limit))
        acc = self._buffer(("grad_acc",), tuple(self.flat_grads.shape))
        loss_acc = self._buffer(("loss_acc",), (4,))
        one = dict((k, v) for k, v in mb.items() if k not in ("split_hook", "dense_w_hook", "stored_acts"))
        saved, self.max_rows_per_pass = self.max_rows_per_pass, None
        try:
            for k, lo in enumerate(range(0, rows, limit)):
                one["idx"] = idx[lo:min(lo + limit, rows)]
                loss4 = self.loss_and_grads(one, kind, clip_param, v_loss_coeff, ent_loss_coeff, lr_mult, inv_count,
                                            tie_rule, beta_clone, duals)
                if k == 0:
                    acc.copy_(self.flat_grads)
                    loss_acc.copy_(loss4)
                else:
                    acc.add_(self.flat_grads)
                    loss_acc.add_(loss4)
        finally:
            self.max_rows_per_pass = saved
        self.flat_grads.copy_(acc)
        hook = mb.get("split_hook")
        if hook is not None:
            hook()
        return loss_acc

    def _backward_trunk(self, x, acts, hids, dh, masked=False, split_hook=None, dense_w_hook=None):
        b = x.shape[0]
        conv_g, dense_g = self._layer_geoms(b)
        d_cur, job = dh, None
        for j in range(self._n_hid - 1, -1, -1):
            k = 2 * (self._n_conv + j)
            hs, fan_in = self._hid_geom[j]
            inp = hids[j - 1] if j > 0 else acts[-1]
            d_prev = self._buffer(("dx_hid", j, b), (b, fan_in))
            d_cur, masked = self._through_activation(self._n_conv + j, d_cur, masked, hids[j])
            self._layer_grads(d_cur, masked, hids[j], b, hs, k, dense_g[j], inp, d_prev)
            if j == 0 and dense_w_hook is not None and self._folds.last_dw_in_place:
                job = dense_w_hook(self._offsets[k], (self._g[k].numel() + 3) // 4 * 4)
            d_cur, masked = d_prev, True
        if split_hook is not None and self._n_hid:
            self._folds.run()
            split_hook()
        self._backward_convs(x, acts, d_cur, masked, corun=job)

    def _dgrad_weight_items(self, b):
        if not self._wt or _lib.default_route == _lib.ROUTE_FP32:
            return []
        conv_g, _ = self._layer_geoms(b)
        return [(self._w[2 * i], wt, conv_g[i]) for i, wt in sorted(self._wt.items())]

    def _backward_convs(self, x, acts, d_act, masked=False, corun=None):
        b = x.shape[0]
        conv_g, _ = self._layer_geoms(b)
        if not getattr(self, "_wt_fresh", False):
            items = self._dgrad_weight_items(b)
            if items:
                _lib.conv2d_dgrad_weights(items)
        group = os.environ.get("ARL_WGRAD_GROUP", "1") != "0"
        for i in range(self._n_conv - 1, -1, -1):
            nf, ci, sz, st, pad, ho, wo = self._conv_geom[i]
            d_in = self._buffer(("dx_conv", i, b), tuple(acts[i - 1].shape)) if i > 0 else None
            d_act, masked = self._through_activation(i, d_act, masked, acts[i])
            self._layer_grads(d_act, masked, acts[i], b * ho * wo, nf, 2 * i, conv_g[i], acts[i - 1] if i > 0 else x, d_in,
                              corun=corun if i > 0 else None,
                              wt=self._wt.get(i) if _lib.default_route != _lib.ROUTE_FP32 else None, defer=group)
            if corun is not None and i > 0 and self._folds.corun_taken:
                corun = None
            d_act, masked = d_in, True
        self._folds.run_wgrads()
        if corun is not None:
            _lib.corun_job_run(corun)
        self._folds.run()

    def _layer_grads(self, d, masked, y, rows, channels, k, geom, inp, d_in, corun=None, wt=None, defer=False):
        folds, g = self._folds, self.grads
        if not masked:
            folds.relu_bwd_bias_grad(d, y, rows, channels, g[k + 1], self._fold_ws(("db", k)))
        dbias = g[k + 1] if masked else None
        if isinstance(inp, ObsRows):
            done = folds.conv2d_u8_bwd_weight(d, inp.obs, inp.idx, self._scale, self._g[k], geom,
                                              self._fold_ws(("dw", k)), dbias=dbias, defer=defer)
        elif d_in is not None:
            done = folds.conv2d_bwd_pair(d, self._w[k], inp, d_in, inp, self._g[k], geom, self._fold_ws(("dw", k)),
                                         dbias=dbias, corun=corun, wt=wt, defer=defer)
        else:
            done = folds.conv2d_bwd_weight(d, inp, self._g[k], geom, self._fold_ws(("dw", k)), dbias=dbias, defer=defer)
        if not done:
            self._bias_grad_left(d, y, rows, channels, k)

    def _bias_grad_left(self, d, y, rows, channels, k):
        self._folds.relu_bwd_bias_grad(d, y, rows, channels, self.grads[k + 1], self._fold_ws(("db", k)))

    def _ones_geom(self, b, width):
        key = ("ones", b, width)
        if key not in self._geoms:
            self._geoms[key] = _lib.dense_geom(b, 4, width)
        return self._geoms[key]

    def _bias_grad_by_ones(self, dout, rows, k):
        ones = self._buffer(("ones4", rows), (rows, 4))
        ones.fill_(1.)
        db4 = self._buffer(("db4", rows, dout.shape[1]), (dout.shape[1], 4))
        _lib.conv2d_bwd_weight(dout, ones, db4, self._ones_geom(rows, dout.shape[1]), self._conv_ws)
        self.grads[k + 1].copy_(db4[:, 0])

    def _through_activation(self, layer, d, masked, y):
        return d, masked

    def _fold_ws(self, key):
        ws = self._fold_workspaces.get(key)
        if ws is None:
            ws = self._fold_workspaces[key] = (_lib.relu_bwd_workspace(self.device) if key[0] == "db"
                                               else _lib.conv_workspace(self.device))
        return ws

    def dist_info(self, observations, state_infos=None):
        return dict(prob=self.prob_value(observations)[0])

    def value(self, observations, state_infos=None):
        return self.prob_value(observations)[1]

    def dist_info_value(self, observations, state_infos=None):
        prob, value = self.prob_value(observations)
        return dict(prob=prob, value=value)

    def _sample(self, prob):
        b = prob.shape[0]
        u = torch.from_numpy(np.random.rand(b)).to(self.device)
        acts = torch.empty(b, dtype=torch.uint8, device=self.device)
        _lib.sample_categorical(prob.contiguous(), u, acts)
        return acts

    def get_actions(self, observations):
        prob, value = self.prob_value(observations)
        return self._sample(prob), dict(prob=prob, value=value)

    def get_action(self, observation, deterministic=False):
        prob, value = self.prob_value(observation[None])
        action = torch.argmax(prob[0]) if deterministic else self._sample(prob)[0]
        return action, dict(prob=prob[0], value=value[0])

    def reset(self, n_batch=None):
        pass

    def reset_one(self, idx):
        pass

    def get_params(self, trainable=True):
        return list(self.params)

    def _internal_arrays(self, flat=None):
        host = (self.flat_params if flat is None else flat).detach().cpu().numpy()
        return [host[o:o + int(np.prod(s))].reshape(s) for o, s in zip(self._offsets, self._shapes)]

    def get_param_values(self, trainable=True):
# ... 48 lines not shown
```

include/accel_rl_hip.h:

```cpp
#ifndef ACCEL_RL_HIP_H
#define ACCEL_RL_HIP_H

#include <stdint.h>

#ifdef __cplusplus
extern "C" {
#endif

#define ARL_ABI_VERSION 4

#define ARL_E_ARG      (-1)
#define ARL_E_RANGE    (-2)
#define ARL_E_ALIGN    (-3)

#define ARL_PROMO_NEP50   0
#define ARL_PROMO_LEGACY  1
#define ARL_PROMO_ASSOC   2

int         arl_abi_version(void);
const char* arl_last_error(void);


int arl_gae_scan(const float* rewards, const float* values, const uint8_t* dones,
                 const float* last_values, double discount, double gae_lambda,
// ... 175 lines not shown
                     const int32_t* idx_or_null, const float* lr_mult,
                     const float* inv_count_or_null, int64_t batch, int32_t hid, int32_t n_actions,
                     int32_t kind, int32_t tie_rule, float clip_param, float v_loss_coeff, float ent_loss_coeff,
                     int32_t relu_mask_dh, float* dout, float* dh, float* dw_head, float* db_head,
                     float* loss4, void* workspace, void* stream);
int arl_pg_head_loss_parts(const float* h, const float* w_head, const float* b_head,
                           const uint8_t* actions, const float* advantages, const float* returns,
                           const float* old_prob, const int8_t* valids_or_null,
                           const int32_t* idx_or_null, const float* lr_mult,
                           const float* inv_count_or_null, int64_t batch, int32_t hid,
                           int32_t n_actions, int32_t kind, int32_t tie_rule, float clip_param,
                           float v_loss_coeff, float ent_loss_coeff, int32_t relu_mask_dh, float* dout, float* dh,
                           float* dw_head, float* db_head, float* loss4, void* workspace,
                           struct arl_fold_item* items3, const struct arl_dgrad_wt* wt_items_or_null, int32_t n_wt,
                           void* stream);

#define ARL_PPG_POLICY 0
#define ARL_PPG_AUX    1
int arl_ppg_head_loss_parts(const float* h, const float* w_head, const float* b_head,
                            const uint8_t* actions, const float* advantages, const float* returns,
                            const float* old_prob, const int32_t* idx_or_null, const float* lr_mult,
                            const float* inv_count_or_null, int64_t batch, int32_t hid, int32_t n_actions,
                            int32_t phase, int32_t tie_rule, float clip_param, float v_loss_coeff,
                            float ent_loss_coeff, float beta_clone, int32_t relu_mask_dh, float* dout, float* dh,
                            float* dw_head, float* db_head, float* loss4, void* workspace,
                            struct arl_fold_item* items3, void* stream);

#define ARL_VMPO_MAX_ROWS 65536
int arl_vmpo_weights(const float* advantages, const int32_t* idx_or_null, int64_t n, const float* duals,
                     double eps_eta, float* psi, float* temp4, void* stream);
int arl_vmpo_head_loss_parts(const float* h, const float* w_head, const float* b_head,
                             const uint8_t* actions, const float* psi, const float* returns,
                             const float* old_prob, const int32_t* idx_or_null, const float* duals,
                             const float* inv_count_or_null, int64_t batch, int32_t hid, int32_t n_actions,
                             float v_loss_coeff, int32_t relu_mask_dh, float* dout, float* dh,
                             float* dw_head, float* db_head, float* loss4, void* workspace,
                             struct arl_fold_item* items3, void* stream);
int arl_vmpo_dual_step(float* duals, float* slot0, float* slot1_or_null, float* step_count,
                       const float* lr_mult, const float* temp4, const float* loss4, float eps_alpha,
                       int32_t method, float learning_rate, float beta1_or_rho, float beta2, float epsilon,
                       void* stream);

#define ARL_RND_MAX_ROWS     16777216
#define ARL_RND_MAX_PIXELS   16777216
#define ARL_RND_MAX_HORIZON  4096
#define ARL_RND_MAX_WIDTH    65536
#define ARL_RND_STATS_SPLITS 32
#define ARL_RND_MIX_MAX_ENVS 1048576
#define ARL_RND_MIX_MAX_ROWS 4194304
int64_t arl_rnd_obs_stats_workspace_bytes(int32_t h, int32_t w);
int arl_rnd_obs_stats(const uint8_t* observations, const uint8_t* extra_observations, int64_t n_env, int32_t horizon,
                      int32_t channels, int32_t h, int32_t w, double* count, double* mean, double* m2, void* workspace,
                      void* stream);
int arl_rnd_obs_prepare(const uint8_t* observations, const uint8_t* extra_observations, const int32_t* idx_or_null,
                        int64_t batch, int64_t n_env, int32_t horizon, int32_t channels, int32_t h, int32_t w,
                        const double* count, const double* mean, const double* m2, float* out, void* stream);
int arl_rnd_error(const float* pred, const float* targ, int64_t batch, int32_t width, int32_t want_grad, float* err,
                  float* dpred, float* loss, void* stream);
int arl_rnd_reward_mix(const float* err, const float* r_ext, int64_t n_env, int32_t horizon, double* rho, double* moments,
                       double gamma_int, double c_ext, double c_int, float* r_mix, float* diag2, void* workspace,
                       void* stream);


typedef struct arl_conv_geom {
    int64_t batch;
    int32_t in_h, in_w, in_c;
    int32_t out_c, kh, kw;
    int32_t stride, pad_h, pad_w;
    int32_t route;
} arl_conv_geom;

#define ARL_CONV_ROUTE_SPLIT9 0
#define ARL_CONV_ROUTE_FP32   1
#define ARL_CONV_ROUTE_SPLIT6 6
#define ARL_CONV_ROUTE_BF16   2

int64_t arl_conv_workspace_bytes(void);

int arl_conv2d_fwd(const float* x, const float* w, const float* bias_or_null, float* y,
                   const arl_conv_geom* geom, int32_t relu, void* workspace, void* stream);

struct arl_corun_job;
int arl_conv2d_bwd_data(const float* dy, const float* w, const float* wt_or_null, const float* mask_or_null, float* dx,
                        const arl_conv_geom* geom, const struct arl_corun_job* job_or_null,
                        int32_t* job_taken_or_null, void* stream);

typedef struct arl_dgrad_wt {
    const float* w;
    float* wt;
    const arl_conv_geom* geom;
} arl_dgrad_wt;
#define ARL_DGRAD_WT_MAX 4
int arl_conv2d_dgrad_weights(const arl_dgrad_wt* items, int32_t n, void* stream);

int arl_conv2d_bwd_weight(const float* dy, const float* x, float* dw, const arl_conv_geom* geom,
                          void* workspace, void* stream);

int arl_conv2d_bwd_weight_parts(const float* dy, const float* x, float* dw, const arl_conv_geom* geom,
                                void* workspace, int64_t workspace_bytes, arl_fold_item* item,
                                float* dbias_or_null, arl_fold_item* bias_item_or_null, void* stream);
int arl_fold_many(const arl_fold_item* items, int32_t n, void* stream);

int arl_conv2d_fwd_parts(const float* x, const float* w, const float* bias_or_null, float* y,
                         const arl_conv_geom* geom, int32_t relu, void* workspace, arl_fold_item* item, void* stream);
int arl_conv2d_fwd_plan(const arl_conv_geom* geom, int32_t* splits, int32_t* k_per_split);


typedef struct arl_serve_head {
    arl_fold_item hidden;
    const float* hidden_bias;
    int32_t hidden_relu;
    int32_t hid;
    const float* w_head;
    const float* b_head;
    float* hidden_out;
} arl_serve_head;

typedef struct arl_serve_conv1 {
    const arl_conv_geom* geom;
    const float* w;
    const float* bias;
    float* y;
    float scale;
    int32_t relu;
} arl_serve_conv1;

int arl_serve_conv1_supported(const arl_game* game, const arl_conv_geom* geom);

int arl_rollout_begin_conv1(const arl_game* game, const arl_env_state* st, const arl_rollout* ro,
                            const arl_serve_conv1* conv1, void* stream);

int arl_env_step_served(const arl_game* game, const arl_env_state* st, const arl_rollout* ro,
                        const arl_serve_head* head, const arl_serve_conv1* conv1_or_null,
                        const double* uniforms, int32_t step, double max_path_length, double discount,
                        int32_t max_start_noops, void* stream);

int arl_conv2d_bwd_pair(const float* dy, const float* w, const float* wt_or_null, const float* mask_or_null, float* dx,
                        const float* x, float* dw, const arl_conv_geom* geom, void* workspace,
                        int64_t workspace_bytes, arl_fold_item* item, float* dbias_or_null,
                        arl_fold_item* bias_item_or_null, const struct arl_corun_job* job_or_null,
                        int32_t* job_taken_or_null, void* stream);

int arl_conv2d_u8_fwd(const uint8_t* obs, int64_t obs_rows, const int32_t* idx_or_null, float scale,
                      const float* w, const float* bias_or_null, float* y, const arl_conv_geom* geom,
                      int32_t relu, void* stream);
int arl_conv2d_u8_bwd_weight_parts(const float* dy, const uint8_t* obs, int64_t obs_rows,
                                   const int32_t* idx_or_null, float scale, float* dw,
                                   const arl_conv_geom* geom, void* workspace, int64_t workspace_bytes,
                                   arl_fold_item* item, float* dbias_or_null,
                                   arl_fold_item* bias_item_or_null, void* stream);

#define ARL_WGRAD_GROUP_MAX 4
typedef struct arl_wgrad_plan { int64_t opaque[32]; } arl_wgrad_plan;
int arl_conv2d_bwd_weight_plan(const float* dy, const float* x, float* dw, const arl_conv_geom* geom,
                               void* workspace, int64_t workspace_bytes, arl_fold_item* item,
                               float* dbias_or_null, arl_fold_item* bias_item_or_null, arl_wgrad_plan* plan);
int arl_conv2d_u8_bwd_weight_plan(const float* dy, const uint8_t* obs, int64_t obs_rows,
                                  const int32_t* idx_or_null, float scale, float* dw,
                                  const arl_conv_geom* geom, void* workspace, int64_t workspace_bytes,
                                  arl_fold_item* item, float* dbias_or_null,
                                  arl_fold_item* bias_item_or_null, arl_wgrad_plan* plan);
int arl_conv2d_bwd_pair_plan(const float* dy, const float* w, const float* wt_or_null, const float* mask_or_null,
                             float* dx, const float* x, float* dw, const arl_conv_geom* geom, void* workspace,
                             int64_t workspace_bytes, arl_fold_item* item, float* dbias_or_null,
                             arl_fold_item* bias_item_or_null, const struct arl_corun_job* job_or_null,
                             int32_t* job_taken_or_null, arl_wgrad_plan* plan, void* stream);
int arl_conv2d_bwd_weight_group(const arl_wgrad_plan* plans, int32_t n, void* stream);


#define ARL_REPLAY_MAX_HORIZON 16

typedef struct arl_replay {
    int64_t  n_env;
    int32_t  size;
    int32_t  n_stack;
    int32_t  frame_bytes;
    int32_t  reward_horizon;
    uint8_t* frames;
    uint8_t* n_blanks;
    uint8_t* acts;
    uint8_t* terminals;
    float*   rewards;
    float*   returns;
} arl_replay;

int arl_replay_append(const arl_replay* rb, const uint8_t* observations, const uint8_t* actions,
                      const float* rewards, const uint8_t* dones, int32_t horizon, int32_t idx,
                      double discount, int32_t promo, void* stream);

int arl_replay_extract(const arl_replay* rb, const int32_t* env_idxs, const int32_t* step_idxs,
                       int64_t batch, uint8_t* obs, uint8_t* next_obs, uint8_t* actions,
                       float* returns, uint8_t* terminals, void* stream);

#define ARL_AUG_PHILOX_STREAM 0xA5D3F1C7u
int arl_replay_extract_shift(const arl_replay* rb, const int32_t* env_idxs, const int32_t* step_idxs, int64_t batch,
                             int32_t frame_h, int32_t frame_w, int32_t pad, int32_t m_obs, int32_t k_next,
                             int64_t seed, int64_t call, uint8_t* obs, uint8_t* next_obs, uint8_t* actions,
                             float* returns, uint8_t* terminals, void* stream);

int arl_sumtree_find(const double* tree, int32_t levels, const double* uniforms, int64_t n,
                     int32_t* tree_idxs, void* stream);
int arl_sumtree_add(double* tree, int32_t levels, const int32_t* tree_idxs, const double* diffs,
                    int64_t n, void* stream);
int arl_sumtree_gather(const double* tree, const int32_t* tree_idxs, int64_t n, double scale,
                       double* out, void* stream);

int arl_sumtree_sample(const double* tree, int32_t levels, const double* uniforms, int32_t m, int32_t n,
                       int32_t part_size, int32_t* tree_idxs, int32_t* env_idxs, int32_t* step_idxs,
                       double* probs, int32_t* n_unique, void* stream);

int arl_sumtree_sample_batch(const double* tree, int32_t levels, const double* uniforms, int32_t m, int32_t n,
                             int32_t part_size, int32_t* tree_idxs, int32_t* env_idxs, int32_t* step_idxs,
                             double* probs, int32_t* n_unique, double beta, float* is_weights_or_null,
                             int64_t* notify_or_null, int32_t ticket, void* stream);

int arl_sumtree_update_pow(double* tree, int32_t levels, const int32_t* tree_idxs, const float* priorities,
                           const double* last_probs, double alpha, int64_t n, void* stream);

int arl_is_weights(const double* probs, int64_t n, double beta, float* out, void* stream);

int arl_priority_diffs(const float* priorities, const double* last_probs, int64_t n, double alpha,
                       double* diffs, void* stream);


int arl_catdqn_act(const float* logits, const float* z, const int32_t* override_or_null, int64_t batch,
                   int32_t n_actions, int32_t n_atoms, int32_t atom_stride, int32_t dueling, float* onehot,
                   uint8_t* greedy_or_null, void* stream);

int arl_catdqn_loss(const float* pred_logits, const float* tgt_next_logits, const float* pol_next_logits_or_null,
                    const float* z, const uint8_t* actions, const float* returns, const uint8_t* terminals,
                    const float* is_weights_or_null, int64_t batch, int32_t n_actions, int32_t n_atoms,
                    int32_t atom_stride, int32_t dueling, float v_min, float v_max, float gamma_n,
                    float* dlogits, float* loss_rows, float* kl, void* stream);

typedef struct arl_logit_src {
    const float* part;
    const float* bias_or_null;
    int64_t split_stride;
    int32_t splits;
    int32_t reserved;
} arl_logit_src;
int arl_catdqn_loss_parts(const arl_logit_src* pred, const arl_logit_src* tgt_next, const arl_logit_src* pol_next_or_null,
                          const float* z, const uint8_t* actions, const float* returns, const uint8_t* terminals,
                          const float* is_weights_or_null, int64_t batch, int32_t n_actions, int32_t n_atoms,
                          int32_t atom_stride, int32_t dueling, float v_min, float v_max, float gamma_n,
                          float* dlogits, float* loss_rows, float* kl, const struct arl_dgrad_wt* wt_items_or_null,
                          int32_t n_wt, void* stream);


int arl_qrdqn_act(const float* theta, const int32_t* override_or_null, int64_t batch, int32_t n_actions,
// ... 140 lines not shown
int arl_lstm_cell_bwd(const float* dh_or_null, int64_t dh_stride, const float* dh_rec_or_null,
                      const float* dc_next_or_null, const float* gates, int64_t gates_stride,
                      const float* c_prev, int64_t cprev_stride, const float* c_out, int64_t c_stride,
                      int64_t batch, int32_t hidden, float* dgates, int64_t dgates_stride, float* dc_prev,
                      void* stream);

int arl_gru_cell_fwd(const float* gx, int64_t gx_stride, const float* gh, const float* h_prev,
                     int64_t hprev_stride, int64_t batch, int32_t hidden, float* h_out, int64_t h_stride,
                     float* saved_or_null, int64_t saved_stride, void* stream);

int arl_gru_cell_bwd(const float* dh_or_null, int64_t dh_stride, const float* dh_rec_or_null,
                     const float* dh_dir_or_null, const float* saved, int64_t saved_stride,
                     const float* h_prev, int64_t hprev_stride, int64_t batch, int32_t hidden,
                     float* dgx, int64_t dgx_stride, float* dgh, int64_t dgh_stride, float* dh_prev,
                     void* stream);

int arl_rnn_cell_fwd(const float* gx, int64_t gx_stride, const float* gh, int64_t batch, int32_t hidden,
                     float* h_out, int64_t h_stride, void* stream);
int arl_rnn_cell_bwd(const float* dh_or_null, int64_t dh_stride, const float* dh_rec_or_null,
                     const float* h_out, int64_t h_stride, int64_t batch, int32_t hidden, float* dpre,
                     int64_t dpre_stride, void* stream);


int arl_seq_handover(const float* h_prev, int64_t h_stride, const float* c_prev_or_null, int64_t c_stride,
                     const uint8_t* reset, const int32_t* idx_or_null, int64_t flag_row0, int64_t flag_row_step,
                     int64_t batch, int32_t hidden, float* hp, float* hprev_out, int64_t hprev_stride,
                     float* cprev_out_or_null, int64_t cprev_out_stride, void* stream);

int arl_lstm_cell_bwd_reset(const float* dh_or_null, int64_t dh_stride, const float* dh_rec_or_null,
                            const float* dc_next_or_null, const float* gates, int64_t gates_stride,
                            const float* c_prev, int64_t cprev_stride, const float* c_out, int64_t c_stride,
                            int64_t batch, int32_t hidden, float* dgates, int64_t dgates_stride, float* dc_prev,
                            const uint8_t* reset_or_null, const int32_t* idx_or_null, int64_t flag_row0,
                            int64_t flag_row_step, void* stream);
int arl_gru_cell_bwd_reset(const float* dh_or_null, int64_t dh_stride, const float* dh_rec_or_null,
                           const float* dh_dir_or_null, const float* saved, int64_t saved_stride,
                           const float* h_prev, int64_t hprev_stride, int64_t batch, int32_t hidden,
                           float* dgx, int64_t dgx_stride, float* dgh, int64_t dgh_stride, float* dh_prev,
                           const uint8_t* reset_or_null, const int32_t* idx_or_null, int64_t flag_row0,
                           int64_t flag_row_step, void* stream);
int arl_rnn_cell_bwd_reset(const float* dh_or_null, int64_t dh_stride, const float* dh_rec_or_null,
                           const float* h_out, int64_t h_stride, int64_t batch, int32_t hidden, float* dpre,
                           int64_t dpre_stride, const uint8_t* reset_or_null, const int32_t* idx_or_null,
                           int64_t flag_row0, int64_t flag_row_step, void* stream);

typedef struct arl_opt_state {
    int64_t n_params;
    float*  params;
    float*  grads;
    float*  slot0;
    float*  slot1;
    float*  step_count;
    float*  lr_mult;
    double* partials;
    float*  grad_norm_log;
    int32_t norm_log_len;
} arl_opt_state;

#define ARL_OPT_PARTIALS 1024
#define ARL_OPT_ADAM     0
#define ARL_OPT_RMSPROP  1

int arl_opt_step(const arl_opt_state* opt, int32_t method, float learning_rate,
                 float avg_factor, float clip, float beta1_or_rho, float beta2,
                 float epsilon, void* stream);

#define ARL_OPT_NORM_SLOTS  64
#define ARL_OPT_NORM_BLOCKS 2048
int arl_opt_step_noclip(const arl_opt_state* opt, int32_t method, float learning_rate, float avg_factor,
                        float beta1_or_rho, float beta2, float epsilon, int32_t k, float* step_pp,
                        double* norm_parts, void* stream);
int arl_opt_finish(const arl_opt_state* opt, int32_t n_updates, float avg_factor, float* step_pp,
                   const double* norm_parts, void* stream);

int arl_opt_step_noclip_split(const arl_opt_state* opt, int32_t method, float learning_rate, float avg_factor,
                              float beta1_or_rho, float beta2, float epsilon, int32_t k, float* step_pp,
                              double* norm_parts, int64_t hole_first, int64_t hole_count, int32_t part, void* stream);
int arl_opt_finish_split(const arl_opt_state* opt, int32_t n_updates, float avg_factor, float* step_pp,
                         const double* norm_parts, int64_t hole_count, void* stream);
typedef struct arl_corun_job { int64_t opaque[40]; } arl_corun_job;
int arl_corun_job_init(arl_corun_job* job, const arl_opt_state* opt, int32_t method, float learning_rate,
                       float avg_factor, float beta1_or_rho, float beta2, float epsilon, int32_t k, float* step_pp,
                       double* norm_parts, int64_t hole_first, int64_t hole_count);
int arl_corun_job_run(const arl_corun_job* job, void* stream);


int arl_noisy_normals(int64_t seed, int64_t counter, int32_t layer, int32_t which, int64_t rows, int32_t width,
                      int32_t rows_per_draw, float* e_or_null, float* f_or_null, uint32_t* words_or_null,
                      void* stream);

typedef struct arl_noisy_layer {
    float* fein;
    float* feout;
    const float* x;
    float* xs;
    int32_t fan_in;
    int32_t units;
    int32_t out_stride;
    int32_t layer;
} arl_noisy_layer;
#define ARL_NOISY_MAX_LAYERS 8

int arl_noisy_noise(const int64_t* state, const arl_noisy_layer* layers, int32_t n_layers, int64_t rows,
                    int32_t rows_per_draw, void* stream);

int arl_noisy_dense_combine(const arl_fold_item* w_prod, const float* bias_or_null, const arl_fold_item* sigma_prod,
                            const float* b_sigma_or_null, const float* feout, int64_t rows, int32_t units, int32_t relu,
                            float* y, const float* fein_next_or_null, float* xs_next_or_null, int64_t* state_or_null,
                            void* stream);

int arl_noisy_dense_bwd_prep(const float* g, const float* feout, int64_t rows, int32_t units, float* g2, float* db,
                             float* db_sigma, void* stream);

int arl_noisy_dense_bwd_dx(const float* dx_w, const float* dx_sigma, const float* fein, int64_t rows, int32_t fan_in,
                           float* dx, void* stream);


typedef struct arl_noisy_draw {
    float* f;
    const float* x;
    float* xs;
    int32_t width;
    int32_t pitch;
    int32_t layer;
    int32_t which;
} arl_noisy_draw;
#define ARL_NOISY_MAX_DRAWS 16

int arl_noisy_draws(const int64_t* state, const arl_noisy_draw* draws, int32_t n_draws, int64_t rows,
                    int32_t rows_per_draw, void* stream);

int arl_noisy_duel_combine(const arl_fold_item* w_prod, const float* bias_or_null, const arl_fold_item* sigma_lo,
                           const arl_fold_item* sigma_hi, const float* b_sigma_or_null, const float* feout, int64_t rows,
                           int32_t units, int32_t split, int32_t relu, float* y, const float* fein_next_or_null,
                           float* xs_next_or_null, int64_t* state_or_null, void* stream);

int arl_noisy_duel_bwd_prep(const float* g, const float* feout, int64_t rows, int32_t units, int32_t split,
                            float* g2_lo, float* g2_hi, float* db, float* db_sigma, void* stream);

int arl_noisy_duel_bwd_dx(const float* dx_w, const float* dx_sigma_lo, const float* fein_lo, const float* dx_sigma_hi,
                          const float* fein_hi, int64_t rows, int32_t fan_in, float* dx, void* stream);

typedef struct arl_noisy_logit_src {
    const float* w_part;
    const float* bias_or_null;
    const float* s_part;
    const float* b_sigma_or_null;
    const float* feout;
    int64_t w_split_stride;
    int64_t s_split_stride;
    int32_t w_splits;
    int32_t s_splits;
} arl_noisy_logit_src;
#define ARL_NOISY_CATDQN_MAX_SPLITS 128

int arl_noisy_catdqn_loss_limits(int32_t* max_splits, int32_t* max_actions, int32_t* max_atoms);

int arl_noisy_catdqn_loss_parts(const arl_noisy_logit_src* pred, const arl_noisy_logit_src* tgt_next,
                                const arl_noisy_logit_src* pol_next_or_null, const float* z, const uint8_t* actions,
                                const float* returns, const uint8_t* terminals, const float* is_weights_or_null,
                                int64_t batch, int32_t n_actions, int32_t n_atoms, int32_t atom_stride, int32_t dueling,
                                float v_min, float v_max, float gamma_n, float* dlogits, float* loss_rows, float* kl,
                                const struct arl_dgrad_wt* wt_items_or_null, int32_t n_wt, void* stream);


int arl_acer_retrace_scan(const float* prob, const float* prob_last, const float* q, const float* q_last,
                          int32_t q_stride, const float* old_prob, const uint8_t* actions, const float* rewards,
// ... 17 lines not shown
```

Measured before the change: 389,600 env-steps/s.

## Split co-run optimizer blocks across multiple backward kernels including wgrad group

Lets the optimizer co-run job be spread in shares across several host kernels: each dgrad layer and the grouped weight-gradient kernel can take a slice of the optimizer blocks, with unused shares carried forward. A leftover standalone launch runs whatever was not taken. The aim is to hide optimizer update work inside idle slots of several backward launches instead of one. The default host spec is 'dgrad', which splits the blocks over the dgrad layers. This adds bookkeeping and changes the grid sizes of the host kernels.

```diff
diff --git a/accel_rl_amd/_lib.py b/accel_rl_amd/_lib.py
--- a/accel_rl_amd/_lib.py
+++ b/accel_rl_amd/_lib.py
@@ -206,6 +206,7 @@
                                         C.POINTER(ArlFoldItem), _vp, C.POINTER(ArlFoldItem), C.POINTER(ArlCorunJob),
                                         C.POINTER(_i32), C.POINTER(ArlWgradPlan), _vp]),
     "arl_conv2d_bwd_weight_group": (_i32, [C.POINTER(ArlWgradPlan), _i32, _vp]),
+    "arl_conv2d_bwd_weight_group_job": (_i32, [C.POINTER(ArlWgradPlan), _i32, C.POINTER(ArlCorunJob), C.POINTER(_i32), _vp]),
     "arl_relu_bwd_bias_parts": (_i32, [_vp, _vp, _i64, _i32, _vp, _vp, C.POINTER(ArlFoldItem), _vp]),
     "arl_replay_append": (_i32, [C.POINTER(ArlReplay), _vp, _vp, _vp, _vp, _i32, _i32, _f64, _i32, _vp]),
     "arl_replay_extract": (_i32, [C.POINTER(ArlReplay), _vp, _vp, _i64, _vp, _vp, _vp, _vp, _vp, _vp]),
@@ -290,6 +291,7 @@
     "arl_opt_finish_split": (_i32, [C.POINTER(ArlOptState), _i32, _f32, _vp, _vp, _i64, _vp]),
     "arl_corun_job_init": (_i32, [C.POINTER(ArlCorunJob), C.POINTER(ArlOptState), _i32, _f32, _f32, _f32, _f32, _f32,
                                   _i32, _vp, _vp, _i64, _i64]),
+    "arl_corun_job_share": (_i32, [C.POINTER(ArlCorunJob), _i32]),
     "arl_corun_job_run": (_i32, [C.POINTER(ArlCorunJob), _vp]),
     "arl_noisy_normals": (_i32, [_i64, _i64, _i32, _i32, _i64, _i32, _i32, _vp, _vp, _vp, _vp]),
     "arl_noisy_noise": (_i32, [_vp, C.POINTER(ArlNoisyLayer), _i32, _i64, _i32, _vp]),
@@ -609,6 +611,10 @@
 
 def corun_job_run(job, stream=None):
     _check(load().arl_corun_job_run(C.byref(job), stream_ptr(stream)), "arl_corun_job_run")
+
+
+def corun_job_share(job, n_blocks=-1):
+    return int(load().arl_corun_job_share(C.byref(job), int(n_blocks)))
 
 
 
@@ -859,10 +865,16 @@
         self._n_plans += 1
         return C.byref(self._plans[self._n_plans - 1])
 
-    def run_wgrads(self, stream=None):
+    def run_wgrads(self, stream=None, corun=None):
         n, self._n_plans = self._n_plans, 0
-        if n:
+        taken = _i32(0)
+        if n and corun is not None:
+            _check(load().arl_conv2d_bwd_weight_group_job(self._plans, n, C.byref(corun), C.byref(taken),
+                                                          stream_ptr(stream)), "arl_conv2d_bwd_weight_group_job")
+        elif n:
             _check(load().arl_conv2d_bwd_weight_group(self._plans, n, stream_ptr(stream)), "arl_conv2d_bwd_weight_group")
+        if corun is not None:
+            self.corun_taken = bool(taken.value)
 
     def conv2d_bwd_weight(self, dy, x, dw, geom, workspace, dbias=None, stream=None, defer=False):
         ho, wo = conv_out_hw(geom)
diff --git a/accel_rl_amd/csrc/arl_optim_dev.h b/accel_rl_amd/csrc/arl_optim_dev.h
--- a/accel_rl_amd/csrc/arl_optim_dev.h
+++ b/accel_rl_amd/csrc/arl_optim_dev.h
@@ -63,6 +63,7 @@
     int block0, finish;
     int slots;
     int co_blocks;
+    int co_first, co_total;
 };
 
 template <int METHOD>
@@ -122,6 +123,11 @@
             c.norm_parts[(long long)c.k * ARL_OPT_NORM_BLOCKS + c.block0 + i] = 0.0;
 }
 
+__device__ __forceinline__ void opt_corun_block(const OptSeg& c, int i, double* lds) {
+    if (c.method == ARL_OPT_ADAM) opt_update_block<ARL_OPT_ADAM>(c, c.co_first + i, c.co_total, lds);
+    else opt_update_block<ARL_OPT_RMSPROP>(c, c.co_first + i, c.co_total, lds);
+}
+
 inline void opt_split_plan(long long n_params, long long hole_count, int* rest, int* hole) {
     const long long n4 = n_params >> 2, h4 = hole_count >> 2;
     *rest = (int)stream_grid(n4 - h4, 256);
diff --git a/accel_rl_amd/csrc/mfma_conv.hip b/accel_rl_amd/csrc/mfma_conv.hip
--- a/accel_rl_amd/csrc/mfma_conv.hip
+++ b/accel_rl_amd/csrc/mfma_conv.hip
@@ -147,13 +147,27 @@
     if (rc) return rc;
     j->host_blocks = 256;
     if (const char* e = getenv("ARL_CORUN_BLOCKS")) j->host_blocks = atoi(e) > 0 ? atoi(e) : 256;
+    j->given = 0; j->share = 0;
     return 0;
 }
 
-extern "C" int arl_corun_job_run(const arl_corun_job* job, void* stream) {
+extern "C" int32_t arl_corun_job_share(arl_corun_job* job, int32_t n_blocks) {
+    if (!job) return 0;
+    CorunJob* j = reinterpret_cast<CorunJob*>(job);
+    if (n_blocks >= 0) j->share = n_blocks;
+    return j->left();
+}
+
+extern "C" int arl_corun_job_run(arl_corun_job* job, void* stream) {
     ARL_REQUIRE(job, ARL_E_ARG, "null pointer");
-    const CorunJob* j = reinterpret_cast<const CorunJob*>(job);
-    return arl::launch_opt_seg(j->seg, j->blocks, (hipStream_t)stream);
+    CorunJob* j = reinterpret_cast<CorunJob*>(job);
+    if (j->given == 0) return arl::launch_opt_seg(j->seg, j->blocks, (hipStream_t)stream);
+    if (j->left() <= 0) return 0;
+    arl::OptSeg c = j->seg;
+    c.co_first = j->given; c.co_total = j->co_total();
+    const int blocks = j->left();
+    j->given += blocks;
+    return arl::launch_opt_seg(c, blocks, (hipStream_t)stream);
 }
 
 namespace {
@@ -496,7 +510,7 @@
 }
 
 extern "C" int arl_conv2d_bwd_data(const float* dy, const float* w, const float* wt_or_null, const float* mask_or_null,
-                                   float* dx, const arl_conv_geom* geom, const arl_corun_job* job_or_null,
+                                   float* dx, const arl_conv_geom* geom, arl_corun_job* job_or_null,
                                    int32_t* job_taken_or_null, void* stream) {
     ARL_ROUTE_SCOPE(geom, job_or_null);
     const int rc = dgrad_impl(dy, w, mask_or_null, dx, geom, nullptr, stream, nullptr, 0, wt_or_null);
@@ -706,7 +720,7 @@
 namespace {
 int pair_impl(const float* dy, const float* w, const float* wt_or_null, const float* mask_or_null, float* dx, const float* x,
               float* dw, const arl_conv_geom* geom, void* workspace, int64_t workspace_bytes, arl_fold_item* item,
-              float* dbias_or_null, arl_fold_item* bias_item_or_null, const arl_corun_job* job_or_null,
+              float* dbias_or_null, arl_fold_item* bias_item_or_null, arl_corun_job* job_or_null,
               int32_t* job_taken_or_null, WgradPlan* defer, void* stream) {
     ARL_REQUIRE(item && geom && (!dbias_or_null || bias_item_or_null), ARL_E_ARG, "null pointer");
     if (job_taken_or_null) *job_taken_or_null = 0;
@@ -748,7 +762,7 @@
 extern "C" int arl_conv2d_bwd_pair(const float* dy, const float* w, const float* wt_or_null, const float* mask_or_null,
                                    float* dx, const float* x, float* dw, const arl_conv_geom* geom, void* workspace,
                                    int64_t workspace_bytes, arl_fold_item* item, float* dbias_or_null,
-                                   arl_fold_item* bias_item_or_null, const arl_corun_job* job_or_null,
+                                   arl_fold_item* bias_item_or_null, arl_corun_job* job_or_null,
                                    int32_t* job_taken_or_null, void* stream) {
     return pair_impl(dy, w, wt_or_null, mask_or_null, dx, x, dw, geom, workspace, workspace_bytes, item, dbias_or_null,
                      bias_item_or_null, job_or_null, job_taken_or_null, nullptr, stream);
@@ -757,7 +771,7 @@
 extern "C" int arl_conv2d_bwd_pair_plan(const float* dy, const float* w, const float* wt_or_null, const float* mask_or_null,
                                         float* dx, const float* x, float* dw, const arl_conv_geom* geom, void* workspace,
                                         int64_t workspace_bytes, arl_fold_item* item, float* dbias_or_null,
-                                        arl_fold_item* bias_item_or_null, const arl_corun_job* job_or_null,
+                                        arl_fold_item* bias_item_or_null, arl_corun_job* job_or_null,
                                         int32_t* job_taken_or_null, arl_wgrad_plan* plan, void* stream) {
     ARL_REQUIRE(plan, ARL_E_ARG, "null pointer");
     *plan = arl_wgrad_plan{};
@@ -766,7 +780,13 @@
 }
 
 extern "C" int arl_conv2d_bwd_weight_group(const arl_wgrad_plan* plans, int32_t n, void* stream) {
+    return arl_conv2d_bwd_weight_group_job(plans, n, nullptr, nullptr, stream);
+}
+
+extern "C" int arl_conv2d_bwd_weight_group_job(const arl_wgrad_plan* plans, int32_t n, arl_corun_job* job_or_null,
+                                               int32_t* job_taken_or_null, void* stream) {
     launch_log_clear();
+    if (job_taken_or_null) *job_taken_or_null = 0;
     ARL_REQUIRE(plans || n == 0, ARL_E_ARG, "null pointer");
     ARL_REQUIRE(n >= 0 && n <= ARL_WGRAD_GROUP_MAX, ARL_E_RANGE, "0 .. ARL_WGRAD_GROUP_MAX plans");
     hipStream_t s = (hipStream_t)stream;
@@ -812,8 +832,10 @@
         groups += (g.blocks[k] + 7) / 8;
     }
     g.group_start[n_el] = groups; g.n = n_el;
-    const CallScope scope(route, nullptr, true);
-    return launch_wgrad_group(g, groups, lds, s);
+    const CallScope scope(route, job_or_null, true);
+    const int rc = launch_wgrad_group(g, groups, lds, s);
+    if (job_taken_or_null) *job_taken_or_null = t_ctx.corun_taken ? 1 : 0;
+    return rc;
 }
 
 namespace {
diff --git a/accel_rl_amd/csrc/mfma_dispatch.h b/accel_rl_amd/csrc/mfma_dispatch.h
--- a/accel_rl_amd/csrc/mfma_dispatch.h
+++ b/accel_rl_amd/csrc/mfma_dispatch.h
@@ -80,14 +80,18 @@
     return rc ? rc : arl::check_launch("igemm_kernel");
 }
 
-struct CorunJob { arl::OptSeg seg; int blocks, host_blocks; };
+struct CorunJob {
+    arl::OptSeg seg; int blocks, host_blocks, given, share;
+    int co_total() const { return blocks < host_blocks ? blocks : host_blocks; }
+    int left() const { return co_total() - given; }
+};
 static_assert(sizeof(CorunJob) <= sizeof(arl_corun_job), "arl_corun_job too small");
-struct CallCtx { int split; const CorunJob* corun; bool corun_taken; };
+struct CallCtx { int split; CorunJob* corun; bool corun_taken; };
 extern thread_local CallCtx t_ctx;
 #define g_split (t_ctx.split)
 struct CallScope {
-    explicit CallScope(int split, const arl_corun_job* job = nullptr, bool keep_log = false) {
-        t_ctx.split = split; t_ctx.corun = reinterpret_cast<const CorunJob*>(job); t_ctx.corun_taken = false;
+    explicit CallScope(int split, arl_corun_job* job = nullptr, bool keep_log = false) {
+        t_ctx.split = split; t_ctx.corun = reinterpret_cast<CorunJob*>(job); t_ctx.corun_taken = false;
         t_launch_split = split;
         if (!keep_log) launch_log_clear();
     }
@@ -101,12 +105,19 @@
 #define ARL_ROUTE_SCOPE(geom, job)                                                                         \
     ARL_REQUIRE(split_of(geom) >= 0, ARL_E_ARG, "conv route: ARL_CONV_ROUTE_SPLIT9, _FP32, _SPLIT6 or _BF16");    \
     const CallScope call_scope_(split_of(geom), job)
+inline bool corun_take(arl::OptSeg* c) {
+    CorunJob* j = t_ctx.corun;
+    if (!j || t_ctx.corun_taken || j->left() <= 0) return false;
+    *c = j->seg;
+    c->co_blocks = j->share > 0 && j->share < j->left() ? j->share : j->left();
+    c->co_first = j->given; c->co_total = j->co_total();
+    j->given += c->co_blocks;
+    t_ctx.corun_taken = true;
+    return true;
+}
 inline bool corun_take(arl::OptSeg* c, dim3* grid) {
-    if (!t_ctx.corun || t_ctx.corun_taken) return false;
-    *c = t_ctx.corun->seg;
-    c->co_blocks = t_ctx.corun->blocks < t_ctx.corun->host_blocks ? t_ctx.corun->blocks : t_ctx.corun->host_blocks;
+    if (!corun_take(c)) return false;
     grid->x += (unsigned)c->co_blocks;
-    t_ctx.corun_taken = true;
     return true;
 }
 
@@ -389,15 +400,18 @@
 #if ARL_CONV_PART == 8
 int launch_wgrad_group(const WgradGroupArgs& g, int groups, size_t lds, hipStream_t s) {
     int rc = 0;
+    arl::OptSeg c = {};
+    const bool co = corun_take(&c);
+    const dim3 grid((unsigned)groups * 8 + (unsigned)((c.co_blocks + 7) & ~7));
 #define ARL_WGROUP(SPL)                                                                                    \
     do {                                                                                                   \
         auto k = wgrad_group_kernel<SPL>;                                                                  \
         rc = allow_big_lds(k, lds + 4096);                                                                 \
-        if (!rc) hipLaunchKernelGGL(k, dim3((unsigned)groups * 8), dim3(256), lds, s, g);                  \
+        if (!rc) hipLaunchKernelGGL(k, grid, dim3(256), lds, s, g, c);                                     \
     } while (0)
     ARL_BY_MODE(ARL_WGROUP(1), ARL_WGROUP(6), ARL_WGROUP(9));
 #undef ARL_WGROUP
-    if (!rc) log_launch(ARL_DEV_K_WGRAD_GROUP, {0, 0, 0, 0, 32, 0}, 0, g.n, dim3((unsigned)groups * 8), lds);
+    if (!rc) log_launch(ARL_DEV_K_WGRAD_GROUP, {0, 0, 0, 0, 32, 0}, co ? ARL_DEV_F_CORUN : 0, g.n, grid, lds);
     return rc ? rc : arl::check_launch("wgrad_group_kernel");
 }
 #endif
diff --git a/accel_rl_amd/csrc/mfma_igemm.h b/accel_rl_amd/csrc/mfma_igemm.h
--- a/accel_rl_amd/csrc/mfma_igemm.h
+++ b/accel_rl_amd/csrc/mfma_igemm.h
@@ -647,8 +647,7 @@
         if (bx < c.co_blocks) {
             __shared__ double lds[8];
             if (blockIdx.y || blockIdx.z) return;
-            if (c.method == ARL_OPT_ADAM) arl::opt_update_block<ARL_OPT_ADAM>(c, bx, c.co_blocks, lds);
-            else arl::opt_update_block<ARL_OPT_RMSPROP>(c, bx, c.co_blocks, lds);
+            arl::opt_corun_block(c, bx, lds);
             return;
         }
         bx -= c.co_blocks;
@@ -672,8 +671,7 @@
         if ((int)blockIdx.x < c.co_blocks) {
             __shared__ double lds[8];
             if (blockIdx.y || blockIdx.z) return;
-            if (c.method == ARL_OPT_ADAM) arl::opt_update_block<ARL_OPT_ADAM>(c, (int)blockIdx.x, c.co_blocks, lds);
-            else arl::opt_update_block<ARL_OPT_RMSPROP>(c, (int)blockIdx.x, c.co_blocks, lds);
+            arl::opt_corun_block(c, (int)blockIdx.x, lds);
             return;
         }
         igemm_body<WGM, WGN, TM, TN, BK, B_KC, MULTI_TAP, HAS_PAD, N16, U8>(a, blockIdx.x - c.co_blocks, blockIdx.y, blockIdx.z, smem);
diff --git a/accel_rl_amd/csrc/mfma_wgrad.h b/accel_rl_amd/csrc/mfma_wgrad.h
--- a/accel_rl_amd/csrc/mfma_wgrad.h
+++ b/accel_rl_amd/csrc/mfma_wgrad.h
@@ -513,12 +513,18 @@
 };
 
 template <int SPLIT>
-__global__ __launch_bounds__(256, 2) void wgrad_group_kernel(const WgradGroupArgs g) {
+__global__ __launch_bounds__(256, 2) void wgrad_group_kernel(const WgradGroupArgs g, const arl::OptSeg c) {
     extern __shared__ __attribute__((aligned(16))) float smem[];
-    const int grp = (int)blockIdx.x >> 3;
+    int blk = (int)blockIdx.x;
+    if (c.co_blocks) {
+        if (blk < c.co_blocks) arl::opt_corun_block(c, blk, reinterpret_cast<double*>(smem));
+        if (blk < ((c.co_blocks + 7) & ~7)) return;
+        blk -= (c.co_blocks + 7) & ~7;
+    }
+    const int grp = blk >> 3;
     int it = 0;
     while (it + 1 < g.n && grp >= g.group_start[it + 1]) ++it;
-    const int id = ((grp - g.group_start[it]) << 3) | ((int)blockIdx.x & 7);
+    const int id = ((grp - g.group_start[it]) << 3) | (blk & 7);
     const int blocks = g.blocks[it];
     if (id >= blocks) return;
     const int gx = g.gx[it], gy = g.gy[it];
diff --git a/accel_rl_amd/csrc/optim.hip b/accel_rl_amd/csrc/optim.hip
--- a/accel_rl_amd/csrc/optim.hip
+++ b/accel_rl_amd/csrc/optim.hip
@@ -84,7 +84,7 @@
 template <int METHOD>
 __global__ __launch_bounds__(256) void update_noclip_kernel(const arl::OptSeg c) {
     __shared__ double lds[8];
-    arl::opt_update_block<METHOD>(c, (int)blockIdx.x, (int)gridDim.x, lds);
+    arl::opt_update_block<METHOD>(c, c.co_first + (int)blockIdx.x, c.co_total ? c.co_total : (int)gridDim.x, lds);
 }
 
 __global__ __launch_bounds__(256) void opt_finish_kernel(arl_opt_state o, int n_updates, int n_blocks, float avg,
diff --git a/accel_rl_amd/policies/atari_cnn_policy.py b/accel_rl_amd/policies/atari_cnn_policy.py
--- a/accel_rl_amd/policies/atari_cnn_policy.py
+++ b/accel_rl_amd/policies/atari_cnn_policy.py
@@ -564,20 +564,64 @@
             if items:
                 _lib.conv2d_dgrad_weights(items)
         group = os.environ.get("ARL_WGRAD_GROUP", "1") != "0"
+        shares = self._corun_shares(corun) if corun is not None else {}
+        carry, used = [0], set()
+
+        def offer(host):
+            key = host if host in shares else "dgrad" if host != "wgroup" and "dgrad" in shares else None
+            if key is None or key in used or _lib.corun_job_share(corun) == 0:
+                return None
+            _lib.corun_job_share(corun, 0 if key == shares["last"] else shares[key] + carry[0])
+            return key
+
+        def offered(key, last_chance=True):
+            if key is None:
+                return
+            if self._folds.corun_taken:
+                carry[0] = 0
+                used.add(key)
+            elif last_chance:
+                carry[0] += shares[key]
+                used.add(key)
+
         for i in range(self._n_conv - 1, -1, -1):
             nf, ci, sz, st, pad, ho, wo = self._conv_geom[i]
             d_in = self._buffer(("dx_conv", i, b), tuple(acts[i - 1].shape)) if i > 0 else None
             d_act, masked = self._through_activation(i, d_act, masked, acts[i])
+            key = offer("dgrad%d" % (i + 1)) if i > 0 else None
             self._layer_grads(d_act, masked, acts[i], b * ho * wo, nf, 2 * i, conv_g[i], acts[i - 1] if i > 0 else x, d_in,
-                              corun=corun if i > 0 else None,
+                              corun=corun if key is not None else None,
                               wt=self._wt.get(i) if _lib.default_route != _lib.ROUTE_FP32 else None, defer=group)
-            if corun is not None and i > 0 and self._folds.corun_taken:
-                corun = None
+            offered(key, last_chance=key != "dgrad" or i == 1)
             d_act, masked = d_in, True
-        self._folds.run_wgrads()
-        if corun is not None:
+        key = offer("wgroup")
+        self._folds.run_wgrads(corun=corun if key is not None else None)
+        offered(key)
+        if corun is not None and _lib.corun_job_share(corun):
             _lib.corun_job_run(corun)
         self._folds.run()
+
+    CORUN_HOSTS = "dgrad"
+
+    def _corun_shares(self, job):
+        spec = os.environ.get("ARL_CORUN_HOSTS", self.CORUN_HOSTS).strip()
+        if spec == "none":
+            return {}
+        names = [h.split(":") for h in spec.split("+")]
+        assert all(len(h) <= 2 and (h[0] in ("wgroup", "dgrad") or (h[0].startswith("dgrad") and h[0][5:].isdigit()))
+                   for h in names), "ARL_CORUN_HOSTS: dgrad[K][:fraction] and wgroup[:fraction] joined by '+', or none"
+        total = _lib.corun_job_share(job)
+
+        def whole(n):
+            return max(8, int(n) // 8 * 8) if total >= 16 else max(1, int(n))
+
+        fixed = {h[0]: whole(round(float(h[1]) * total)) for h in names if len(h) == 2}
+        free = [h[0] for h in names if len(h) == 1]
+        rest = max(0, total - sum(fixed.values()))
+        shares = {h: whole(rest // len(free)) for h in free}
+        shares.update(fixed)
+        shares["last"] = max(shares, key=lambda h: float("inf") if h == "wgroup" else -int(h[5:] or 0))
+        return shares
 
     def _layer_grads(self, d, masked, y, rows, channels, k, geom, inp, d_in, corun=None, wt=None, defer=False):
         folds, g = self._folds, self.grads
diff --git a/include/accel_rl_hip.h b/include/accel_rl_hip.h
--- a/include/accel_rl_hip.h
+++ b/include/accel_rl_hip.h
@@ -281,7 +281,7 @@
 
 struct arl_corun_job;
 int arl_conv2d_bwd_data(const float* dy, const float* w, const float* wt_or_null, const float* mask_or_null, float* dx,
-                        const arl_conv_geom* geom, const struct arl_corun_job* job_or_null,
+                        const arl_conv_geom* geom, struct arl_corun_job* job_or_null,
                         int32_t* job_taken_or_null, void* stream);
 
 typedef struct arl_dgrad_wt {
@@ -337,7 +337,7 @@
 int arl_conv2d_bwd_pair(const float* dy, const float* w, const float* wt_or_null, const float* mask_or_null, float* dx,
                         const float* x, float* dw, const arl_conv_geom* geom, void* workspace,
                         int64_t workspace_bytes, arl_fold_item* item, float* dbias_or_null,
-                        arl_fold_item* bias_item_or_null, const struct arl_corun_job* job_or_null,
+                        arl_fold_item* bias_item_or_null, struct arl_corun_job* job_or_null,
                         int32_t* job_taken_or_null, void* stream);
 
 int arl_conv2d_u8_fwd(const uint8_t* obs, int64_t obs_rows, const int32_t* idx_or_null, float scale,
@@ -362,9 +362,11 @@
 int arl_conv2d_bwd_pair_plan(const float* dy, const float* w, const float* wt_or_null, const float* mask_or_null,
                              float* dx, const float* x, float* dw, const arl_conv_geom* geom, void* workspace,
                              int64_t workspace_bytes, arl_fold_item* item, float* dbias_or_null,
-                             arl_fold_item* bias_item_or_null, const struct arl_corun_job* job_or_null,
+                             arl_fold_item* bias_item_or_null, struct arl_corun_job* job_or_null,
                              int32_t* job_taken_or_null, arl_wgrad_plan* plan, void* stream);
 int arl_conv2d_bwd_weight_group(const arl_wgrad_plan* plans, int32_t n, void* stream);
+int arl_conv2d_bwd_weight_group_job(const arl_wgrad_plan* plans, int32_t n, struct arl_corun_job* job_or_null,
+                                    int32_t* job_taken_or_null, void* stream);
 
 
 #define ARL_REPLAY_MAX_HORIZON 16
@@ -671,7 +673,8 @@
 int arl_corun_job_init(arl_corun_job* job, const arl_opt_state* opt, int32_t method, float learning_rate,
                        float avg_factor, float beta1_or_rho, float beta2, float epsilon, int32_t k, float* step_pp,
                        double* norm_parts, int64_t hole_first, int64_t hole_count);
-int arl_corun_job_run(const arl_corun_job* job, void* stream);
+int32_t arl_corun_job_share(arl_corun_job* job, int32_t n_blocks);
+int arl_corun_job_run(arl_corun_job* job, void* stream);
 
 
 int arl_noisy_normals(int64_t seed, int64_t counter, int32_t layer, int32_t which, int64_t rows, int32_t width,
```

Result: no change. 388,500 env-steps/s (-0.3%).
